# rsutormin/KmerGutsJava

Measured on AMD Instinct MI355X. Metric: amino-acid residues/sec scanned (and hits/sec) on 1 Gbp synthetic, 1/2/4/8 MI355X, higher is better.
Workload: dtype int64; 1 GPU; 1 Gbp contig mix (0.5 kbp..1.024 Mbp, uniform ACGT) on 1 GPU, 6-frame translate + 8-mer lookup vs 1400303159-slot signature table (33.6 GB, load 0.50), -m 5 -g 200; total_bp_rank0=1000000000, contigs_rank0=6351, total_bp_all_ranks=1000000000, num_sigs=1400303159, residues_rank0=1999974596, residues_all_ranks=1999974596, hits_rank0=36744843, hits_all_ranks=36744843, calls_rank0=4, parallelism=contig shards x1, table replicated

## Files before the change

### kmergutsjava_amd/csrc/kg_aggregate.hpp

```cpp
#pragma once

#include <hip/hip_runtime.h>
#include <stdint.h>

#include "../../include/kmerguts_hip.h"

namespace kg {

struct AggParams { int32_t min_hits, min_weighted_hits, max_gap, order_constraint; };

struct AggState {
    uint32_t lo, last, prev;
    int32_t last_pos, last_fI, last_avg, prev_fI;
    int32_t cnt;
    int32_t currentFI;
    uint32_t ncalls;
};

__device__ __forceinline__ int32_t rl(int32_t v, int k) { return __builtin_amdgcn_readlane(v, k); }
__device__ __forceinline__ int32_t uni(int32_t v) { return __builtin_amdgcn_readfirstlane(v); }

struct ChunkRegs {
    uint32_t base;
    uint64_t mask;
    int32_t fI, pos;
    float wt;
};

__device__ __forceinline__ uint32_t process_set(const kg_hit *__restrict__ h, const uint8_t *__restrict__ acc, uint8_t *__restrict__ vote,
                                            uint32_t begin, const AggParams &p, AggState &s, const ChunkRegs &cur, const ChunkRegs &prv,
                                            bool &cur_vote, uint32_t container, kg_call *calls, bool allow_carry)
{
    const int lane = threadIdx.x & 63;
    int32_t fICount = 0;
    float weighted = 0.f;
    uint32_t lastHit = s.lo;
    const uint32_t c0 = begin + ((s.lo - begin) & ~63u);
    for (uint32_t b = c0; b <= s.last; b += 64) {
        const uint32_t i = b + lane;
        const bool in = i >= s.lo && i <= s.last;
        int32_t fI = 0;
        float wt = 0.f;
        bool mem = false;
        if (b == cur.base) {
            fI = cur.fI;
            wt = cur.wt;
            mem = in && ((cur.mask >> lane) & 1ull) != 0;
        } else if (b == prv.base) {
            fI = prv.fI;
            wt = prv.wt;
            mem = in && ((prv.mask >> lane) & 1ull) != 0;
        } else if (in) {
            fI = h[i].fI;
            wt = h[i].functionWt;
            mem = (acc[i] & KG_EV_ACCEPTED) != 0;
        }
        uint64_t m = __ballot(in && mem && fI == s.currentFI);
        if (m) {
            fICount += (int32_t)__popcll(m);
            lastHit = b + 63u - (uint32_t)__builtin_clzll(m);
            const int32_t wbits = __float_as_int(wt);
            while (m) {
                const int k = __builtin_ctzll(m);
                m &= m - 1;
                weighted += __int_as_float(rl(wbits, k));
            }
        }
    }
    uint32_t what = 0;
    if (fICount >= p.min_hits && weighted >= (float)p.min_weighted_hits) {
        what = 1;
        auto pos_of = [&](uint32_t i) -> int32_t {
            if (i - cur.base < 64u) return rl(cur.pos, (int)(i - cur.base));
            if (i - prv.base < 64u) return rl(prv.pos, (int)(i - prv.base));
            return h[i].from0InProt;
        };
        const int32_t pos_lo = pos_of(s.lo), pos_last = pos_of(lastHit);
        if (lane == 0) {
            kg_call c;
            c.container = container;
            c.start = pos_lo;
            c.end = pos_last + (KG_K - 1);
            c.count = fICount; c.fI = s.currentFI; c.weightedHits = weighted;
            calls[s.ncalls] = c;
        }
        s.ncalls++;
        for (uint32_t b = c0; b <= s.last; b += 64) {
            const uint32_t i = b + lane;
            const bool in = i >= s.lo && i <= s.last;
            if (b == cur.base) {
                cur_vote = cur_vote || (in && ((cur.mask >> lane) & 1ull) != 0 && cur.fI == s.currentFI);
            } else if (b == prv.base) {
                if (in && ((prv.mask >> lane) & 1ull) != 0 && prv.fI == s.currentFI) vote[i] = 1;
            } else if (in && (acc[i] & KG_EV_ACCEPTED) != 0 && h[i].fI == s.currentFI) {
                vote[i] = 1;
            }
        }
    }
    if (allow_carry && s.cnt >= 2 && s.prev_fI != s.currentFI && s.prev_fI == s.last_fI) {
        s.currentFI = s.last_fI;
        s.lo = s.prev;
        s.cnt = 2;
        what |= 2;
    } else {
        s.cnt = 0;
    }
    return what;
}

struct EvBits {
    uint32_t e;
    __device__ __forceinline__ void before(int k, uint32_t what)
    {
        const uint32_t bits = KG_EV_RESET_BEFORE | ((what & 1u) ? KG_EV_CALL_BEFORE : 0u) | ((what & 2u) ? KG_EV_KEEP2_BEFORE : 0u);
        if ((int)(threadIdx.x & 63) == k) e |= bits;
    }
    __device__ __forceinline__ void after(int k, uint32_t what)
    {
        const uint32_t bits = KG_EV_RESET_AFTER | ((what & 1u) ? KG_EV_CALL_AFTER : 0u) | ((what & 2u) ? KG_EV_KEEP2_AFTER : 0u);
        if ((int)(threadIdx.x & 63) == k) e |= bits;
    }
};

constexpr uint32_t kNoPiece = 0xFFFFFFFFu;

constexpr uint32_t kPairWindow = 256;
constexpr uint32_t kPairMaxContainer = 39000;

__global__ __launch_bounds__(256) void piece_starts_kernel(const kg_hit *__restrict__ hits, const int64_t *__restrict__ chs,
                                                           uint32_t n_hits, uint32_t pshift, int32_t max_gap,
                                                           uint32_t *__restrict__ piece_start, uint8_t *__restrict__ piece_pair ,
                                                           uint32_t n_blocks, uint32_t pairs_ok)
{
    const int lane = threadIdx.x & 63;
    const uint32_t u = (uint32_t)uni((int32_t)(blockIdx.x * 4 + (threadIdx.x >> 6)));
    if (u >= n_blocks) return;
    uint32_t found = kNoPiece;
    const uint32_t blk = 1u << pshift, i0 = u << pshift;
    if (u > 0 && i0 < n_hits) {
        const uint32_t c0 = hits[i0].container;
        const uint32_t lo0 = (uint32_t)chs[c0], hi0 = (uint32_t)chs[c0 + 1];
        const bool long_enough = hi0 - lo0 >= 2u * blk || hi0 < i0 + blk;
        for (uint32_t j = 0; j < 256u && j < blk && found == kNoPiece && long_enough; j += 64) {
            const uint32_t i = i0 + j + (uint32_t)lane;
            bool gap = false;
            if (i < n_hits && j + (uint32_t)lane < blk) {
                const kg_hit a = hits[i - 1], b = hits[i];
                gap = a.container == b.container && (int32_t)((uint32_t)a.from0InProt + (uint32_t)max_gap) < b.from0InProt;
            }
            const uint64_t m = __ballot(gap);
            if (m) found = i0 + j + (uint32_t)__builtin_ctzll(m);
        }
    }
    if (found != kNoPiece) {
        const uint32_t c = hits[found].container;
        const uint32_t lo = (uint32_t)chs[c], hi = (uint32_t)chs[c + 1];
        if (found - lo < blk / 2 || hi - found < blk / 2) found = kNoPiece;
    }
    uint32_t pair = 0;
    if (found == kNoPiece && pairs_ok && u > 0 && i0 < n_hits) {
        const uint32_t c0 = hits[i0].container;
        const uint32_t lo0 = (uint32_t)chs[c0], hi0 = (uint32_t)chs[c0 + 1];
        if (hi0 - lo0 >= 2u * blk && hi0 - lo0 < kPairMaxContainer) {
            const uint32_t w0 = i0 - lo0 > kPairWindow ? i0 - kPairWindow : lo0;
            const uint32_t span = min(256u, blk);
            const uint32_t wend = min(min(i0 + span + 1u, hi0), n_hits);
            int32_t afi = 0;
            bool have = false, carry_eq = false, carry_start = false;
            for (uint32_t b = w0; b < wend && found == kNoPiece; b += 64) {
                const uint32_t i = b + (uint32_t)lane;
                const bool in = i < wend;
                int32_t fI = 0;
                bool cstart = false, gapf = false, eqf = false;
                if (in) {
                    const kg_hit cur = hits[i];
                    fI = cur.fI;
                    cstart = i == lo0;
                    if (!cstart) {
                        const kg_hit prv = hits[i - 1];
                        gapf = (int32_t)((uint32_t)prv.from0InProt + (uint32_t)max_gap) < cur.from0InProt;
                        eqf = !gapf && prv.fI == cur.fI;
                    }
                }
                const uint64_t am = __ballot(in && (cstart || gapf || eqf)), eqm = __ballot(eqf), stm = __ballot(cstart || gapf);
                const uint64_t below = am & ((1ull << lane) - 1ull);
                const int al = below ? 63 - __builtin_clzll(below) : 0;
                const int32_t lfi = __shfl(fI, al);
                const bool phave = below ? true : have;
                const int32_t pfi = below ? lfi : afi;
                const bool prev_eq = lane ? ((eqm >> (lane - 1)) & 1ull) != 0 : carry_eq;
                const bool prev_start = lane ? ((stm >> (lane - 1)) & 1ull) != 0 : carry_start;
                const bool cand = eqf && !prev_eq && !prev_start && phave && pfi != fI && i >= i0 + 1u && i - 1u < i0 + span &&
                                  i - 1u - lo0 >= blk / 2 && hi0 - (i - 1u) >= blk / 2;
                const uint64_t cm = __ballot(cand);
                if (cm) { found = b + (uint32_t)__builtin_ctzll(cm) - 1u; pair = 1; }
                if (am) { const int last = 63 - __builtin_clzll(am); afi = rl(fI, last); have = true; }
                carry_eq = (eqm >> 63) & 1ull;
                carry_start = (stm >> 63) & 1ull;
            }
        }
    }
    if (lane == 0) { piece_start[u] = found; piece_pair[u] = (uint8_t)pair; }
}

__global__ void merge_before_kernel(const uint32_t *__restrict__ piece_start, const uint8_t *__restrict__ piece_pair,
                                    const uint8_t *__restrict__ before_ev, uint32_t n_blocks, uint8_t *ev, unsigned long long *n_pieces)
{
    const uint32_t u = blockIdx.x * blockDim.x + threadIdx.x;
    const uint32_t ps = u < n_blocks ? piece_start[u] : kNoPiece;
    if (ps != kNoPiece && before_ev[u]) ev[ps + (piece_pair[u] ? 1u : 0u)] |= before_ev[u];
    const unsigned long long m = __ballot(ps != kNoPiece);
    if (m && (threadIdx.x & 63) == 0) atomicAdd(n_pieces, (unsigned long long)__popcll(m));
}

struct CallsCold {
    kg_call *staged;
    uint8_t *tail_ev;
    uint32_t *call_cnt, *first_cnt, *piece_cnt;
    uint8_t *before_ev;
    const uint8_t *piece_pair;
};

__device__ __forceinline__ uint32_t walk_unit(const kg_hit *__restrict__ hits, const AggParams &p, uint8_t *acc, uint8_t *vote,
                                              const uint32_t begin, const uint32_t end, const uint32_t c, kg_call *calls,
                                              const uint32_t *__restrict__ piece_start, const uint32_t pshift,
                                              const CallsCold *__restrict__ cold, uint32_t *tail_out, bool *reached_end)
{
    const int lane = threadIdx.x & 63;
    uint32_t stopped_at = kNoPiece;
    AggState s;
    s.lo = s.last = s.prev = begin;
    s.last_pos = s.last_fI = s.last_avg = s.prev_fI = 0;
    s.cnt = 0; s.currentFI = 0; s.ncalls = 0;
    int32_t carry_pos = 0, carry_fI = 0;
    ChunkRegs pv, ppv;
    pv.base = ppv.base = 0xFFFFFF00u; pv.mask = ppv.mask = 0; pv.fI = ppv.fI = pv.pos = ppv.pos = 0; pv.wt = ppv.wt = 0.f;

    int32_t n_pos = 0, n_fI = 0, n_avg = 0, m_pos = 0, m_fI = 0, m_avg = 0;
    float n_wt = 0.f, m_wt = 0.f;
    if (begin + (uint32_t)lane < end) {
        const kg_hit &h0 = hits[begin + lane];
        n_pos = h0.from0InProt; n_fI = h0.fI; n_avg = h0.avgOffFromEnd; n_wt = h0.functionWt;
    }
    if (begin + 64u + (uint32_t)lane < end) {
        const kg_hit &h1 = hits[begin + 64u + lane];
        m_pos = h1.from0InProt; m_fI = h1.fI; m_avg = h1.avgOffFromEnd; m_wt = h1.functionWt;
    }
    for (uint32_t base = begin; base < end; base += 64) {
        int n = (int)min(64u, end - base);
        if (piece_start) {
            const uint32_t u1 = base >> pshift, u2 = (base + (uint32_t)n - 1u) >> pshift;
            const uint32_t s1 = piece_start[u1];
            if (s1 > begin && s1 >= base && s1 < base + (uint32_t)n) stopped_at = s1;
            if (u2 != u1) {
                const uint32_t s2 = piece_start[u2];
                if (s2 > begin && s2 < base + (uint32_t)n && s2 < stopped_at) stopped_at = s2;
            }
            if (stopped_at != kNoPiece) n = (int)(stopped_at - base);
            if (n == 0) break;
        }
        const uint32_t i = base + lane;
        int32_t pos = n_pos, fI = n_fI, avg = n_avg;
        float wt = n_wt;
        if (lane >= n) { pos = 0; fI = 0; avg = 0; wt = 0.f; }
        n_pos = m_pos; n_fI = m_fI; n_avg = m_avg; n_wt = m_wt;
        m_pos = 0; m_fI = 0; m_avg = 0; m_wt = 0.f;
        if (base + 128u + (uint32_t)lane < end) {
            const kg_hit &h2 = hits[base + 128u + lane];
            m_pos = h2.from0InProt; m_fI = h2.fI; m_avg = h2.avgOffFromEnd; m_wt = h2.functionWt;
        }
        uint64_t accmask;
        bool votes = false;
        EvBits em = {0};
        ChunkRegs cu;
        cu.base = base; cu.mask = 0; cu.fI = fI; cu.pos = pos; cu.wt = wt;

        const bool fast = !p.order_constraint && s.cnt + n < KG_MAX_HITS_PER_SEQ - 2 &&
                          (s.cnt == 0 || s.last + 1 == base);
        if (fast) {
            accmask = n == 64 ? ~0ull : ((1ull << n) - 1ull);
            int32_t ppos = __shfl_up(pos, 1), pfI = __shfl_up(fI, 1);
            if (lane == 0) { ppos = carry_pos; pfI = carry_fI; }
            const bool first = i == begin;
            const bool gapf = !first && (int32_t)((uint32_t)ppos + (uint32_t)p.max_gap) < pos;
            const bool eqf = !first && fI == pfI;
            const uint64_t gapm = __ballot(gapf), eqm = __ballot(eqf);
            const uint64_t inm = n == 64 ? ~0ull : ((1ull << n) - 1ull);
            int k0 = 0;
            for (;;) {
                if (k0 >= n) break;
                const int32_t cfi = s.cnt > 0 ? s.currentFI : rl(fI, k0);
                const uint64_t neqm = __ballot(fI != cfi);
                const uint64_t ev = (gapm | (eqm & neqm)) & inm & ~((1ull << k0) - 1ull);
                if (!ev) break;
                const int k = __builtin_ctzll(ev);
                if (k > k0) {
                    if (s.cnt == 0) { s.currentFI = rl(fI, k0); s.lo = base + k0; }
                    s.cnt += k - k0;
                }
                const int32_t fk = rl(fI, k);
                const uint32_t ik = base + (uint32_t)k;
                if (s.cnt > 0 && ((gapm >> k) & 1)) {
                    uint32_t what = 0;
                    if (s.cnt >= p.min_hits) {
                        s.last = ik - 1;
                        what = (cu.mask = accmask, process_set(hits, acc, vote, begin, p, s, cu, pv, votes, c, calls, false));
                    } else {
                        s.cnt = 0;
                    }
                    em.before(k, what);
                }
                if (s.cnt == 0) { s.currentFI = fk; s.lo = ik; }
                s.cnt++;
                if (s.cnt > 1 && s.currentFI != fk && ((eqm >> k) & 1)) {
                    s.last = ik; s.prev = ik - 1; s.last_fI = fk; s.prev_fI = fk;
                    em.after(k, (cu.mask = accmask, process_set(hits, acc, vote, begin, p, s, cu, pv, votes, c, calls, true)));
                }
                k0 = k + 1;
            }
            if (n > k0) {
                if (s.cnt == 0) { s.currentFI = rl(fI, k0); s.lo = base + k0; }
                s.cnt += n - k0;
            }
            if (s.cnt > 0) {
                s.last = base + n - 1;
                s.last_pos = rl(pos, n - 1); s.last_fI = rl(fI, n - 1); s.last_avg = rl(avg, n - 1);
                if (s.cnt > 1) { s.prev = s.last - 1; s.prev_fI = n >= 2 ? rl(fI, n - 2) : carry_fI; }
            }
        } else {
            accmask = 0;
            for (int k = 0; k < n; k++) {
                const int32_t pk = rl(pos, k), fk = rl(fI, k), ak = rl(avg, k);
                const uint32_t ik = base + (uint32_t)k;
                if (s.cnt > 0 && (int32_t)((uint32_t)s.last_pos + (uint32_t)p.max_gap) < pk) {
                    uint32_t what = 0;
                    if (s.cnt >= p.min_hits)
                        what = (cu.mask = accmask, process_set(hits, acc, vote, begin, p, s, cu, pv, votes, c, calls, true));
                    else
                        s.cnt = 0;
                    em.before(k, what);
                }
                if (s.cnt == 0) s.currentFI = fk;
                bool ok = !p.order_constraint || s.cnt == 0;
                if (!ok) {
                    const int32_t d = (int32_t)((uint32_t)(pk - s.last_pos) - (uint32_t)(s.last_avg - ak));
                    const int32_t ad = d < 0 ? (int32_t)(0u - (uint32_t)d) : d;
                    ok = fk == s.last_fI && ad <= 20;
                }
                if (ok) {
                    if (s.cnt < KG_MAX_HITS_PER_SEQ - 2) {
                        if (s.cnt == 0) { s.lo = ik; s.prev = ik; s.prev_fI = fk; }
                        else { s.prev = s.last; s.prev_fI = s.last_fI; }
                        s.last = ik; s.last_pos = pk; s.last_fI = fk; s.last_avg = ak;
                        s.cnt++;
                        accmask |= 1ull << k;
                    }
                    if (s.cnt > 1 && s.currentFI != fk && s.prev_fI == s.last_fI)
                        em.after(k, (cu.mask = accmask, process_set(hits, acc, vote, begin, p, s, cu, pv, votes, c, calls, true)));
                }
            }
        }
        if (lane < n) {
            acc[i] = (uint8_t)(em.e | (uint32_t)((accmask >> lane) & 1ull) * KG_EV_ACCEPTED);
            vote[i] = votes ? 1 : 0;
        }
        carry_pos = rl(pos, n - 1);
        carry_fI = rl(fI, n - 1);
        ppv = pv;
        cu.mask = accmask;
        pv = cu;
        if (stopped_at != kNoPiece) break;
    }
    uint32_t tail = 0;
    if (stopped_at != kNoPiece && cold->piece_pair[stopped_at >> pshift]) {
        uint32_t bits = 0;
        if (s.cnt > 0) {
            bits = KG_EV_RESET_AFTER | KG_EV_KEEP2_AFTER;
            bool tail_votes = false;
            if (process_set(hits, acc, vote, begin, p, s, pv, ppv, tail_votes, c, calls, false) & 1u) bits |= KG_EV_CALL_AFTER;
            if (tail_votes) vote[pv.base + lane] = 1;
        }
        if (lane == 0) cold->before_ev[stopped_at >> pshift] = (uint8_t)bits;
    } else if (stopped_at != kNoPiece) {
        uint32_t bits = 0;
        if (s.cnt > 0) {
            bits = KG_EV_RESET_BEFORE;
            if (s.cnt >= p.min_hits) {
                bool tail_votes = false;
                if (process_set(hits, acc, vote, begin, p, s, pv, ppv, tail_votes, c, calls, false) & 1u) bits |= KG_EV_CALL_BEFORE;
                if (tail_votes) vote[pv.base + lane] = 1;
            }
        }
        if (lane == 0) cold->before_ev[stopped_at >> pshift] = (uint8_t)bits;
    } else if (s.cnt >= p.min_hits) {
        bool tail_votes = false;
        tail = process_set(hits, acc, vote, begin, p, s, pv, ppv, tail_votes, c, calls, true) & 1u;
        if (tail_votes) vote[pv.base + lane] = 1;
    }
    *tail_out = tail;
    *reached_end = stopped_at == kNoPiece;
    return s.ncalls;
}

__global__ __launch_bounds__(256) void calls_wave_kernel(const kg_hit *__restrict__ hits, const int64_t *__restrict__ chs,
                                                         uint32_t n_cont, AggParams p, uint8_t *acc, uint8_t *vote,
                                                         uint32_t per_wave, uint32_t n_cwaves,
                                                         const uint32_t *__restrict__ piece_start, uint32_t pshift, uint32_t n_pblocks,
                                                         const CallsCold *__restrict__ cold)
{
    const int lane = threadIdx.x & 63;
    const uint32_t w = (uint32_t)uni((int32_t)(blockIdx.x * 4 + (threadIdx.x >> 6)));
    if (w >= n_cwaves) {
        const uint32_t u = w - n_cwaves;
        if (u >= n_pblocks) return;
        const uint32_t begin = piece_start[u];
        if (begin == kNoPiece) return;
        const uint32_t c = hits[begin].container;
        const uint32_t end = (uint32_t)chs[c + 1];
        uint32_t tail;
        bool reached_end;
        const uint32_t ncalls = walk_unit(hits, p, acc, vote, begin, end, c, cold->staged + begin / (uint32_t)p.min_hits, piece_start, pshift,
                                          cold, &tail, &reached_end);
        if (lane == 0) {
            cold->piece_cnt[u] = ncalls;
            if (ncalls) atomicAdd(&cold->call_cnt[c], ncalls);
            if (reached_end) cold->tail_ev[c] = (uint8_t)tail;
        }
        return;
    }
    const uint32_t c_first = w * per_wave;
    uint32_t my_begin = 0, my_end = 0;
    const bool mine = (uint32_t)lane < per_wave && c_first + (uint32_t)lane < n_cont;
    if (mine) { my_begin = (uint32_t)chs[c_first + lane]; my_end = (uint32_t)chs[c_first + lane + 1]; }
    if (mine && my_end - my_begin < 2) {
        cold->first_cnt[c_first + lane] = 0;
        cold->tail_ev[c_first + lane] = 0;
        if (my_end != my_begin) { acc[my_begin] = (uint8_t)KG_EV_ACCEPTED; vote[my_begin] = 0; }
    }
    uint64_t todo = __ballot(mine && my_end - my_begin >= 2);
    while (todo) {
        const int ci = __builtin_ctzll(todo);
        todo &= todo - 1;
        const uint32_t c = c_first + (uint32_t)ci;
        const uint32_t begin = (uint32_t)rl((int32_t)my_begin, ci), end = (uint32_t)rl((int32_t)my_end, ci);
        uint32_t tail;
        bool reached_end;
        const uint32_t ncalls = walk_unit(hits, p, acc, vote, begin, end, c, cold->staged + begin / (uint32_t)p.min_hits, piece_start, pshift,
                                          cold, &tail, &reached_end);
        if (lane == 0) {
            cold->first_cnt[c] = ncalls;
            if (ncalls) atomicAdd(&cold->call_cnt[c], ncalls);
            if (reached_end) cold->tail_ev[c] = (uint8_t)tail;
        }
    }
}

template <int W>
__global__ __launch_bounds__(256) void compact_calls_kernel(const kg_call *__restrict__ staged, const int64_t *__restrict__ chs,
                                                            const uint32_t *__restrict__ first_cnt, const uint32_t *__restrict__ call_off,
                                                            uint32_t n_cont, uint32_t min_hits, kg_call *__restrict__ calls,
                                                            const uint32_t *__restrict__ piece_start, const uint32_t *__restrict__ piece_cnt,
                                                            uint32_t pshift)
{
    const uint64_t t = (uint64_t)blockIdx.x * blockDim.x + threadIdx.x;
    const uint64_t c = t / W;
    if (c >= n_cont) return;
    const uint32_t begin = (uint32_t)chs[c], end = (uint32_t)chs[c + 1];
    kg_call *dst = calls + call_off[c];
    {
        const uint32_t n = first_cnt[c];
        const kg_call *src = staged + begin / min_hits;
        for (uint32_t k = (uint32_t)(t % W); k < n; k += W) dst[k] = src[k];
        dst += n;
    }
    if (piece_start && end > begin) {
        if (W == 64) {
            const int lane = threadIdx.x & 63;
            const uint32_t last = (end - 1u) >> pshift;
            for (uint32_t u0 = begin >> pshift; u0 <= last; u0 += 64) {
                const uint32_t u = u0 + (uint32_t)lane;
                const uint32_t ps = u <= last ? piece_start[u] : kNoPiece;
                const bool mine = ps > begin && ps < end;
                const uint32_t n = mine ? piece_cnt[u] : 0u;
                uint32_t incl = n;
#pragma unroll
                for (int off = 1; off < 64; off <<= 1) {
                    const uint32_t v = (uint32_t)__shfl_up((int)incl, off);
                    if (lane >= off) incl += v;
                }
                const kg_call *src = staged + (mine ? ps / min_hits : 0u);
                for (uint32_t k = 0; k < n; k++) dst[incl - n + k] = src[k];
                dst += (uint32_t)__shfl((int)incl, 63);
            }
        } else {
            for (uint32_t u = begin >> pshift; u <= (end - 1u) >> pshift; u++) {
                const uint32_t ps = piece_start[u];
                if (ps <= begin || ps >= end) continue;
                const uint32_t n = piece_cnt[u];
                const kg_call *src = staged + ps / min_hits;
                for (uint32_t k = (uint32_t)(t % W); k < n; k += W) dst[k] = src[k];
                dst += n;
            }
        }
    }
}

__global__ void call_starts_kernel(const uint32_t *call_off, uint64_t n_cont, const uint64_t *total, int64_t *ccs)
{
    uint64_t c = (uint64_t)blockIdx.x * blockDim.x + threadIdx.x;
    if (c > n_cont) return;
    ccs[c] = c == n_cont ? (int64_t)*total : (int64_t)call_off[c];
}

__global__ __launch_bounds__(256) void voter_count_kernel(const uint8_t *__restrict__ vote, uint32_t n_hits, uint32_t *__restrict__ cnt)
{
    const uint32_t i = blockIdx.x * blockDim.x + threadIdx.x;
    const uint64_t m = __ballot(i < n_hits && vote[i] != 0);
    if ((threadIdx.x & 63) == 0 && (i & ~63u) < n_hits) cnt[i >> 6] = (uint32_t)__popcll(m);
    if (i == 0) cnt[(n_hits + 63u) >> 6] = 0;
}

__global__ __launch_bounds__(256) void voter_scatter_kernel(const kg_hit *__restrict__ hits, const uint8_t *__restrict__ vote,
                                                            uint32_t n_hits, const uint32_t *__restrict__ voff, int32_t *__restrict__ vlist)
{
    const uint32_t i = blockIdx.x * blockDim.x + threadIdx.x;
    const int lane = threadIdx.x & 63;
    const bool v = i < n_hits && vote[i] != 0;
    const uint64_t m = __ballot(v);
    if (v) vlist[voff[i >> 6] + (uint32_t)__popcll(m & ((1ull << lane) - 1ull))] = hits[i].oI;
}

__global__ __launch_bounds__(256) void otu_wave_kernel(const int32_t *__restrict__ vlist, const uint32_t *__restrict__ voff,
                                                       const uint8_t *__restrict__ vote, const int64_t *__restrict__ chs,
                                                       uint32_t n_hits, uint32_t n_seqs, uint32_t per, kg_otu *otu, uint32_t per_wave,
                                                       const kg_otu *__restrict__ otu_init)
{
    const int lane = threadIdx.x & 63;
    const uint32_t s_first = (uint32_t)uni((int32_t)(blockIdx.x * 4 + (threadIdx.x >> 6))) * per_wave;
    auto voter_index = [&](uint32_t i) -> uint32_t {
        const uint32_t c0 = i & ~63u;
        const uint64_t m = __ballot(c0 + (uint32_t)lane < n_hits && c0 + (uint32_t)lane < i && vote[c0 + lane] != 0);
        return (c0 < n_hits ? voff[c0 >> 6] : voff[(n_hits + 63u) >> 6]) + (uint32_t)__popcll(m);
    };
    for (uint32_t s = s_first; s < s_first + per_wave && s < n_seqs; s++) {
        int32_t n = 0;
        uint32_t nmask = 0;
        int32_t cnt = 0, oi = 0;
        if (otu_init) {
            const kg_otu *r0 = otu_init + s;
            n = uni(min(max(r0->n, 0), KG_OI_BUFSZ));
            nmask = (1u << n) - 1u;
            if (lane < KG_OI_BUFSZ) { cnt = r0->count[lane]; oi = r0->oI[lane]; }
        }
        const uint32_t vb = voter_index((uint32_t)chs[(uint64_t)s * per]), ve = voter_index((uint32_t)chs[(uint64_t)(s + 1) * per]);
        int32_t n_o = vb + (uint32_t)lane < ve ? vlist[vb + lane] : 0;
        for (uint32_t b = vb; b < ve; b += 64) {
            const int32_t o = n_o;
            n_o = b + 64u + (uint32_t)lane < ve ? vlist[b + 64u + lane] : 0;
            const int nv = (int)min(64u, ve - b);
            const int32_t before = __shfl_up(o, 1);
            uint64_t heads = __ballot(lane < nv && (lane == 0 || o != before));
            const uint64_t above = lane < 63 ? heads >> (lane + 1) : 0ull;
            const int32_t rlen = above ? __builtin_ctzll(above) + 1 : nv - lane;
            while (heads) {
                const int k = __builtin_ctzll(heads);
                heads &= heads - 1;
                const int32_t ok = rl(o, k), r = rl(rlen, k);
                const uint64_t at = __ballot(oi == ok) & nmask;
                int j;
                if (at) {
                    j = __builtin_ctzll(at);
                    cnt += lane == j ? r : 0;
                } else {
                    if (n == KG_OI_BUFSZ) j = KG_OI_BUFSZ - 1; else { j = n++; nmask = nmask * 2u + 1u; }
                    if (lane == j) { oi = ok; cnt = r; }
                }
                if (j == 0) continue;
                const int32_t cj = rl(cnt, j);
                const uint32_t more = (uint32_t)__ballot(cnt > cj);
                if ((more >> (j - 1)) & 1u) continue;
                const uint32_t gt = more & ((1u << j) - 1u);
                const int p = gt ? 32 - __builtin_clz(gt) : 0;
                const int32_t oj = rl(oi, j);
                const int32_t pc = __builtin_amdgcn_update_dpp(0, cnt, 0x111, 0xF, 0xF, false);
                const int32_t po = __builtin_amdgcn_update_dpp(0, oi, 0x111, 0xF, 0xF, false);
                if (lane > p && lane <= j) { cnt = pc; oi = po; }
                else if (lane == p) { cnt = cj; oi = oj; }
            }
        }
        if (lane < KG_OI_BUFSZ) {
            otu[s].count[lane] = lane < n ? cnt : 0;
            otu[s].oI[lane] = lane < n ? oi : 0;
        }
        if (lane == 0) otu[s].n = n;
    }
}

__global__ void process_set_single_kernel(const kg_hit *__restrict__ hits, int32_t n, int32_t current_fi, AggParams p,
                                          kg_otu *otu, kg_call *call, int32_t *out)
{
    if (threadIdx.x != 0 || blockIdx.x != 0) return;
    int32_t count = 0, last = 0;
    float wt = 0.f;
    for (int32_t i = 0; i < n; i++)
        if (hits[i].fI == current_fi) { last = i; count++; wt += hits[i].functionWt; }
    int32_t called = 0;
    kg_otu o = *otu;
    if (count >= p.min_hits && wt >= (float)p.min_weighted_hits) {
        called = 1;
        kg_call c;
        c.container = hits[0].container; c.start = hits[0].from0InProt; c.end = hits[last].from0InProt + (KG_K - 1);
        c.count = count; c.fI = current_fi; c.weightedHits = wt;
        *call = c;
        for (int32_t i = 0; i <= last; i++) {
            if (hits[i].fI != current_fi) continue;
            int32_t j = 0;
            while (j < o.n && o.oI[j] != hits[i].oI) j++;
            if (j == o.n) {
                if (o.n == KG_OI_BUFSZ) j--; else o.n++;
                o.oI[j] = hits[i].oI; o.count[j] = 1;
            } else o.count[j]++;
            while (j > 0 && o.count[j - 1] <= o.count[j]) {
                const int32_t tc = o.count[j - 1], to = o.oI[j - 1];
                o.count[j - 1] = o.count[j]; o.oI[j - 1] = o.oI[j];
                o.count[j] = tc; o.oI[j] = to;
                j--;
            }
        }
    }
    *otu = o;
    const bool keep2 = hits[n - 2].fI != current_fi && hits[n - 2].fI == hits[n - 1].fI;
    out[0] = called; out[1] = keep2 ? hits[n - 1].fI : current_fi; out[2] = keep2 ? 1 : 0;
}

}
```

### kmergutsjava_amd/csrc/kg_device.hpp

```cpp
#pragma once

#include <hip/hip_runtime.h>
#include <stdint.h>

#include "../../include/kmerguts_hip.h"

namespace kg {

constexpr int kWave = 64;
constexpr int kWavesPerWG = 4;
constexpr int kDnaPosPerBlock = 192;
constexpr int kAaWinPerBlock = 64;
constexpr uint32_t kInvalid = 0xFFFFFFFFu;
constexpr uint32_t kTagEmpty = 0xFFu;
constexpr uint64_t kNotFound = ~0ull;
constexpr int kTagPad = 64;

struct BlockDesc {
    uint64_t soff;
    uint32_t len;
    uint32_t j;
    uint32_t nk;
    uint32_t ibase;
    uint32_t seq;
// ... 623 lines not shown
            }
#pragma unroll
            for (int q = 0; q < N; q++) {
                if (r == q) {
                    cand[q] = s;
                    if (done) {
                        if (COUNTERS) stop[q] = s;
                        if (hit) { ent[q].oI = e.oI; ent[q].avg = e.avg; ent[q].fI = e.fI; ent[q].wt = e.wt; foundm |= 1u << q; }
                    }
                }
            }
            if (done) pend &= pend - 1;
        }
    }
    if (COUNTERS) {
#pragma unroll
        for (int q = 0; q < N; q++) {
            if (valid[q]) {
                uint64_t last = stop[q] < tab.limit ? stop[q] + 1 : tab.limit;
                ctr_slots += last - home[q];
                if (prog) progress_note_walk(prog, home[q], stop[q], tab.limit);
                if (found_slot) found_slot[q] = (uint32_t)stop[q];
            }
        }
    }
    return foundm;
}

__device__ __forceinline__ void flush_ran_off(bool ran_off, unsigned long long *ctr, int lane)
{
    if (__ballot(ran_off) && lane == 0) atomicOr(&ctr[3], 1ull);
}

__device__ __forceinline__ void flush_counters(unsigned long long ctr_valid, unsigned long long ctr_slots,
                                               unsigned long long *ctr, int lane)
{
    for (int off = 32; off > 0; off >>= 1) {
        ctr_valid += __shfl_down(ctr_valid, off);
        ctr_slots += __shfl_down(ctr_slots, off);
    }
    if (lane == 0) {
        atomicAdd(&ctr[0], ctr_valid);
        atomicAdd(&ctr[1], ctr_slots);
    }
}

template <bool AA, bool COUNTERS, int RPG>
__global__ __launch_bounds__(kWave *kWavesPerWG) void scan_kernel(
    const uint8_t *__restrict__ entries, const uint8_t *__restrict__ tags, uint64_t limit, uint64_t num_sigs, uint64_t magic,
    uint32_t m35, const uint8_t *__restrict__ seq, const BlockDesc *__restrict__ blocks, uint32_t n_blocks,
    uint32_t *__restrict__ counts,
    uint32_t *__restrict__ block_stage_base, kg_hit *__restrict__ stage, unsigned long long *cursor, uint64_t stage_cap,
    uint32_t stage_chunk, unsigned long long *ctr,
    Progress *prog , uint32_t *__restrict__ stage_slot ,
    const uint32_t *__restrict__ hbits , uint64_t tail_start)
{
    constexpr int ROWS = AA ? 1 : 6;
    constexpr int NG = ROWS / RPG;
    static_assert(ROWS % RPG == 0, "RPG must divide the row count");
    __shared__ typename WaveLds<AA>::type lds[kWavesPerWG];
    __shared__ typename WaveLds<AA>::tables enc_tables;
    const int lane = threadIdx.x & 63;
    const int wave = threadIdx.x >> 6;
    const uint32_t wave_global = __builtin_amdgcn_readfirstlane(blockIdx.x * kWavesPerWG + wave);
    const uint32_t n_waves = gridDim.x * kWavesPerWG;
    TableView tab;
    tab.entries = entries; tab.tags = tags; tab.limit = limit; tab.num_sigs = num_sigs; tab.magic = magic; tab.m35 = m35;

    typename WaveLds<AA>::type &l = lds[wave];
    encode_init<AA>(enc_tables, threadIdx.x, blockDim.x);
    __syncthreads();

    unsigned long long ctr_valid = 0, ctr_slots = 0;
    bool ran_off = false;
    unsigned long long res_at = 0, res_end = 0;

    for (uint32_t it_v = wave_global; it_v < n_blocks; it_v += n_waves) {
        const uint32_t it = __builtin_amdgcn_readfirstlane(it_v);
        const BlockDesc bd = blocks[it];
        encode_block<AA>(l, enc_tables, seq, bd, lane);

        for (int g = 0; g < NG; g++) {
            uint64_t val[RPG], home[RPG];
            uint32_t fp[RPG];
            bool valid[RPG];
#pragma unroll
            for (int q = 0; q < RPG; q++) {
                uint32_t hi, lo;
                uint64_t quo;
                valid[q] = row_halves<AA>(l, g * RPG + q, lane, bd, &hi, &lo);
                home[q] = split_halves(hi, lo, tab, &quo);
                fp[q] = tag_qs(quo, home[q]);
                val[q] = (uint64_t)hi * 160000ull + lo;
            }

            if (!COUNTERS && hbits) {
                uint32_t w[RPG];
#pragma unroll
                for (int q = 0; q < RPG; q++) w[q] = valid[q] && home[q] < limit ? hbits[home[q] >> 5] : ~0u;
#pragma unroll
                for (int q = 0; q < RPG; q++)
                    if (valid[q] && home[q] < limit && !((w[q] >> ((uint32_t)home[q] & 31u)) & 1u)) {
                        valid[q] = false;
                        if (home[q] >= tail_start) ran_off = true;
                    }
            }
            Payload ent[RPG];
            uint32_t fslot[RPG];
#pragma unroll
            for (int q = 0; q < RPG; q++) fslot[q] = 0;
            const uint32_t foundm = probe_n<RPG, COUNTERS>(tab, val, home, fp, valid, ent, ctr_valid, ctr_slots, ran_off,
                                                           COUNTERS ? prog : nullptr, COUNTERS && stage_slot ? fslot : nullptr);

            uint32_t cnt[RPG], rank[RPG];
            uint32_t total = 0;
#pragma unroll
            for (int q = 0; q < RPG; q++) {
                const int r = g * RPG + q;
                unsigned long long m = __ballot((foundm >> q) & 1u);
                cnt[q] = (uint32_t)__popcll(m);
                unsigned long long below = m & ((1ull << lane) - 1ull);
                unsigned long long above = lane == 63 ? 0ull : (m >> (lane + 1));
                rank[q] = (!AA && r >= 3) ? (uint32_t)__popcll(above) : (uint32_t)__popcll(below);
                total += cnt[q];
                if (lane == 0) counts[row_index<AA>(bd, it, r)] = cnt[q];
            }
            if (total > res_end - res_at) {
                unsigned long long chunk = total > stage_chunk ? total : stage_chunk;
                unsigned long long b = 0;
                if (lane == 0) b = atomicAdd(cursor, chunk);
                b = ((unsigned long long)__builtin_amdgcn_readfirstlane((uint32_t)(b >> 32)) << 32) |
                    (unsigned long long)__builtin_amdgcn_readfirstlane((uint32_t)b);
                res_at = b; res_end = b + chunk;
            }
            const unsigned long long base = res_at;
            res_at += total;
            if (lane == 0) block_stage_base[(uint64_t)it * NG + g] = (uint32_t)base;
            if (total && base + total <= stage_cap) {
                uint32_t rowbase = 0;
#pragma unroll
                for (int q = 0; q < RPG; q++) {
                    if ((foundm >> q) & 1u) {
                        kg_hit h;
                        row_record_key<AA>(bd, g * RPG + q, lane, &h.container, &h.from0InProt);
                        h.oI = ent[q].oI; h.avgOffFromEnd = ent[q].avg; h.fI = ent[q].fI; h.functionWt = ent[q].wt;
                        stage[base + rowbase + rank[q]] = h;
                        if (COUNTERS && stage_slot) stage_slot[base + rowbase + rank[q]] = fslot[q];
                    }
                    rowbase += cnt[q];
                }
            }
        }
        wave_sync();
    }

    if (COUNTERS) flush_counters(ctr_valid, ctr_slots, ctr, lane);
    flush_ran_off(ran_off, ctr, lane);
}

__global__ void build_blocks_kernel(const int64_t *seq_off, const uint32_t *ibase, uint32_t n_seqs,
                                    uint32_t n_blocks, BlockDesc *out)
{
    uint32_t i = blockIdx.x * blockDim.x + threadIdx.x;
    if (i >= n_blocks) return;
    uint32_t lo = 0, hi = n_seqs;
    while (hi - lo > 1) {
        uint32_t mid = lo + (hi - lo) / 2;
        if (ibase[mid] <= i) lo = mid; else hi = mid;
    }
    BlockDesc d;
    d.soff = (uint64_t)seq_off[lo];
    d.len = (uint32_t)(seq_off[lo + 1] - seq_off[lo]);
    d.j = i - ibase[lo];
    d.nk = ibase[lo + 1] - ibase[lo];
    d.ibase = ibase[lo];
    d.seq = lo;
    d.pad = 0;
    out[i] = d;
}

constexpr int kScanThreads = 256;
constexpr int kScanPerThread = 8;
constexpr int kScanChunk = kScanThreads * kScanPerThread;

__device__ __forceinline__ uint32_t wg_exclusive_scan(uint32_t x, uint32_t *total, uint32_t *lds )
{
    const int lane = threadIdx.x & 63, wave = threadIdx.x >> 6;
    uint32_t incl = x;
    for (int off = 1; off < 64; off <<= 1) {
        uint32_t y = __shfl_up(incl, off);
        if (lane >= off) incl += y;
    }
    if (lane == 63) lds[wave] = incl;
    __syncthreads();
    uint32_t wbase = 0, all = 0;
    for (int w = 0; w < kScanThreads / 64; w++) {
        uint32_t s = lds[w];
        if (w < wave) wbase += s;
        all += s;
    }
    __syncthreads();
    *total = all;
    return wbase + incl - x;
}

__global__ __launch_bounds__(kScanThreads) void scan_partials_kernel(const uint32_t *in, uint64_t n, uint64_t *partial)
{
    __shared__ uint64_t wsum[kScanThreads / 64];
    uint64_t base = (uint64_t)blockIdx.x * kScanChunk + (uint64_t)threadIdx.x * kScanPerThread;
    uint64_t s = 0;
    for (int k = 0; k < kScanPerThread; k++)
        if (base + k < n) s += in[base + k];
    for (int d = 32; d > 0; d >>= 1) s += __shfl_xor(s, d);
    if ((threadIdx.x & 63) == 0) wsum[threadIdx.x >> 6] = s;
    __syncthreads();
    if (threadIdx.x == 0) {
        uint64_t all = 0;
        for (int w = 0; w < kScanThreads / 64; w++) all += wsum[w];
        partial[blockIdx.x] = all;
    }
}

__global__ __launch_bounds__(kScanThreads) void scan_top_kernel(uint64_t *partial, uint32_t n_partials, uint64_t *total_out)
{
    __shared__ uint64_t carry;
    __shared__ uint64_t wsum[kScanThreads / 64];
    if (threadIdx.x == 0) carry = 0;
    __syncthreads();
    const int lane = threadIdx.x & 63, wave = threadIdx.x >> 6;
    for (uint32_t b = 0; b < n_partials; b += kScanThreads) {
        uint32_t i = b + threadIdx.x;
        uint64_t x = i < n_partials ? partial[i] : 0;
        uint64_t incl = x;
        for (int off = 1; off < 64; off <<= 1) {
            uint64_t y = __shfl_up(incl, off);
            if (lane >= off) incl += y;
        }
        if (lane == 63) wsum[wave] = incl;
        __syncthreads();
        uint64_t wbase = 0, all = 0;
        for (int w = 0; w < kScanThreads / 64; w++) {
            uint64_t s = wsum[w];
            if (w < wave) wbase += s;
            all += s;
        }
        uint64_t c = carry;
        if (i < n_partials) partial[i] = c + wbase + incl - x;
        __syncthreads();
        if (threadIdx.x == 0) carry = c + all;
        __syncthreads();
    }
    if (threadIdx.x == 0) *total_out = carry;
}

__global__ __launch_bounds__(kScanThreads) void scan_final_kernel(const uint32_t *in, uint64_t n, const uint64_t *partial,
                                                                  uint32_t *out)
{
    __shared__ uint32_t lds[8];
    uint64_t base = (uint64_t)blockIdx.x * kScanChunk + (uint64_t)threadIdx.x * kScanPerThread;
    uint32_t v[kScanPerThread];
    uint32_t s = 0;
    for (int k = 0; k < kScanPerThread; k++) {
        v[k] = base + k < n ? in[base + k] : 0;
        s += v[k];
    }
    uint32_t total;
    uint32_t excl = wg_exclusive_scan(s, &total, lds);
    uint32_t run = (uint32_t)partial[blockIdx.x] + excl;
    for (int k = 0; k < kScanPerThread; k++) {
        if (base + k < n) out[base + k] = run;
        run += v[k];
    }
}

template <bool AA>
__global__ __launch_bounds__(kWave *kWavesPerWG) void place_kernel(const BlockDesc *__restrict__ blocks, uint32_t n_blocks,
                                                                  const uint32_t *__restrict__ counts,
                                                                  const uint32_t *__restrict__ offs,
                                                                  const uint32_t *__restrict__ block_stage_base, uint32_t rpg,
                                                                  const kg_hit *__restrict__ stage, kg_hit *__restrict__ hits,
                                                                  const uint32_t *__restrict__ stage_slot, uint32_t *__restrict__ hit_slots)
{
    constexpr int ROWS = AA ? 1 : 6;
    const int lane = threadIdx.x & 63;
    const uint32_t it = __builtin_amdgcn_readfirstlane(blockIdx.x * kWavesPerWG + (threadIdx.x >> 6));
    if (it >= n_blocks) return;
    const BlockDesc bd = blocks[it];
    const uint32_t ng = (uint32_t)ROWS / rpg;
    uint32_t src = 0;
#pragma unroll
    for (int r = 0; r < ROWS; r++) {
        if ((uint32_t)r % rpg == 0) src = block_stage_base[(uint64_t)it * ng + (uint32_t)r / rpg];
        const uint32_t vrow = row_index<AA>(bd, it, r);
        uint32_t n = counts[vrow];
        if ((uint32_t)lane < n) {
            hits[(uint64_t)offs[vrow] + lane] = stage[(uint64_t)src + lane];
            if (hit_slots) hit_slots[(uint64_t)offs[vrow] + lane] = stage_slot[(uint64_t)src + lane];
        }
        src += n;
    }
}

template <bool AA>
__global__ void container_starts_kernel(const uint32_t *ibase, uint32_t n_seqs, const uint32_t *offs, uint64_t n_rows,
                                        const uint64_t *total, int64_t *chs)
{
    constexpr uint32_t PER = AA ? 1 : 6;
    uint64_t c = (uint64_t)blockIdx.x * blockDim.x + threadIdx.x;
    uint64_t n_cont = (uint64_t)n_seqs * PER;
    if (c > n_cont) return;
    if (c == n_cont) { chs[c] = (int64_t)*total; return; }
    uint32_t k = (uint32_t)(c / PER), cc = (uint32_t)(c % PER);
    uint32_t nk = ibase[k + 1] - ibase[k];
    uint64_t row = (uint64_t)PER * ibase[k] + (uint64_t)cc * nk;
    chs[c] = row < n_rows ? (int64_t)offs[row] : (int64_t)*total;
}

struct ClearList { uint32_t *p[8]; uint64_t words[8]; int n; };

__global__ __launch_bounds__(256) void clear_many_kernel(ClearList l)
{
    const uint64_t tid = (uint64_t)blockIdx.x * blockDim.x + threadIdx.x, stride = (uint64_t)gridDim.x * blockDim.x;
    for (int k = 0; k < l.n; k++) {
        uint32_t *p = l.p[k];
        const uint64_t w = l.words[k];
        const uint64_t head = min(w, (uint64_t)((16u - ((uintptr_t)p & 15u)) & 15u) / 4u);
        const uint64_t quads = (w - head) / 4;
        uint4 *q = reinterpret_cast<uint4 *>(p + head);
        for (uint64_t i = tid; i < quads; i += stride) q[i] = make_uint4(0, 0, 0, 0);
        for (uint64_t i = tid; i < head; i += stride) p[i] = 0;
        for (uint64_t i = head + quads * 4 + tid; i < w; i += stride) p[i] = 0;
    }
}

__global__ void build_tags_kernel(const uint8_t *entries, uint64_t limit, uint64_t n_tags, uint64_t num_sigs, uint64_t magic,
                                  uint8_t *tags, unsigned long long *occupied)
{
    TableView tab;
    tab.entries = entries; tab.tags = tags; tab.limit = limit; tab.num_sigs = num_sigs; tab.magic = magic; tab.m35 = 0;
    uint64_t i = (uint64_t)blockIdx.x * blockDim.x + threadIdx.x;
    uint64_t stride = (uint64_t)gridDim.x * blockDim.x;
    unsigned long long occ = 0, tail = 0;
    for (; i < n_tags; i += stride) {
        uint32_t t = kTagEmpty;
        if (i < limit) {
            const uint2 *p = reinterpret_cast<const uint2 *>(entries + i * 24);
            uint2 a = p[0];
            int64_t key = (int64_t)(((uint64_t)a.y << 32) | a.x);
            if (key <= KG_MAX_ENCODED) {
                uint64_t q;
                const uint64_t slot = split_value((uint64_t)key, tab, &q);
                t = tag_qs(q, slot);
                occ++;
            }
        }
        tags[i] = (uint8_t)t;
        if (t == kTagEmpty && i < limit) tail = i + 1;
    }
    for (int off = 32; off > 0; off >>= 1) {
        occ += __shfl_down(occ, off);
        const unsigned long long o = __shfl_down(tail, off);
        tail = o > tail ? o : tail;
    }
    if ((threadIdx.x & 63) == 0) {
        if (occ) atomicAdd(occupied, occ);
        if (tail) atomicMax(occupied + 1, tail);
    }
}

constexpr uint32_t kHomeWalkMax = 1024;
constexpr uint32_t kBidxClasses = 19, kBidxPair0 = 20, kBidxHash0 = 191, kBidxMore = 255;
constexpr uint32_t kBidxInexact = 0x80000000u;

__host__ __device__ constexpr uint32_t bidx_pair_code(uint32_t c1, uint32_t c2)
{
    return kBidxPair0 + c1 * 19u - c1 * (c1 + 1u) / 2u + (c2 - c1 - 1u);
}
static_assert(bidx_pair_code(0, 1) == 20 && bidx_pair_code(0, 18) == 37 && bidx_pair_code(1, 2) == 38 && bidx_pair_code(17, 18) == 190,
              "pair codes must fill 20..190");

__device__ __forceinline__ uint32_t bidx_decode(uint32_t code)
{
    if (code == 0) return 0u;
    if (code < kBidxPair0) return 1u << (code - 1u);
    if (code < kBidxHash0) {
        uint32_t c1 = 0;
        while (code >= bidx_pair_code(c1, c1 + 1u) + (18u - c1)) c1++;
        const uint32_t c2 = c1 + 1u + (code - bidx_pair_code(c1, c1 + 1u));
        return (1u << c1) | (1u << c2);
    }
    if (code == kBidxMore) return 0x7FFFFu | kBidxInexact;
    const uint32_t m6 = code - kBidxHash0;
    uint32_t m = 0;
    for (uint32_t c = 0; c < kBidxClasses; c++) m |= ((m6 >> (c % 6u)) & 1u) << c;
    return m | kBidxInexact;
}

__device__ __forceinline__ uint32_t bidx_encode(uint32_t class_mask, bool complete)
{
    if (!complete) return kBidxMore;
    const uint32_t n = (uint32_t)__popc(class_mask);
    if (n == 0) return 0u;
    const uint32_t c1 = (uint32_t)__builtin_ctz(class_mask);
    if (n == 1) return 1u + c1;
    if (n == 2) return bidx_pair_code(c1, 31u - (uint32_t)__builtin_clz(class_mask));
    const uint32_t m6 = (class_mask | (class_mask >> 6) | (class_mask >> 12) | (class_mask >> 18)) & 63u;
    return kBidxHash0 + m6;
}

__global__ void build_bidx_kernel(const uint8_t *entries, const uint8_t *tags, uint64_t limit, uint64_t n_idx, uint64_t num_sigs,
                                  uint64_t magic, uint8_t *idx)
{
    TableView tab;
    tab.entries = entries; tab.tags = tags; tab.limit = limit; tab.num_sigs = num_sigs; tab.magic = magic; tab.m35 = 0;
    const uint64_t stride = (uint64_t)gridDim.x * blockDim.x;
    for (uint64_t h = (uint64_t)blockIdx.x * blockDim.x + threadIdx.x; h < n_idx; h += stride) {
        uint32_t mask = 0;
        bool complete = true;
        if (h < limit && tags[h] != kTagEmpty) {
            uint64_t j = h;
            for (; j < limit && j - h < kHomeWalkMax; j++) {
                if (tags[j] == kTagEmpty) break;
                const uint2 a = *reinterpret_cast<const uint2 *>(entries + j * 24);
                const int64_t key = (int64_t)(((uint64_t)a.y << 32) | a.x);
                if (key < 0) continue;
                uint64_t q;
                if (split_value((uint64_t)key, tab, &q) != h) continue;
                mask |= 1u << (uint32_t)(q % kBidxClasses);
            }
            if (j < limit && j - h >= kHomeWalkMax) complete = false;
        }
        idx[h] = (uint8_t)bidx_encode(mask, complete);
    }
}

__global__ void build_hbits_kernel(const uint8_t *__restrict__ idx, uint64_t n_idx, uint32_t *__restrict__ bits, uint64_t n_words)
{
    const uint64_t stride = (uint64_t)gridDim.x * blockDim.x;
    for (uint64_t w = (uint64_t)blockIdx.x * blockDim.x + threadIdx.x; w < n_words; w += stride) {
        uint32_t out = 0;
        const uint64_t s0 = w * 32;
        if (s0 + 32 <= n_idx) {
            const uint4 a = *reinterpret_cast<const uint4 *>(idx + s0), b = *reinterpret_cast<const uint4 *>(idx + s0 + 16);
            const uint32_t v[8] = {a.x, a.y, a.z, a.w, b.x, b.y, b.z, b.w};
#pragma unroll
            for (int k = 0; k < 8; k++)
#pragma unroll
                for (int j = 0; j < 4; j++) out |= (((v[k] >> (8 * j)) & 0xFFu) != 0u ? 1u : 0u) << (4 * k + j);
        } else {
            for (uint32_t j = 0; j < 32 && s0 + j < n_idx; j++) out |= (idx[s0 + j] != 0 ? 1u : 0u) << j;
        }
        bits[w] = out;
    }
}

}
```

### kmergutsjava_amd/csrc/kg_host.hpp

```cpp
#pragma once

#include <algorithm>
#include <atomic>
#include <cstdio>
#include <cstdlib>
#include <cstring>
#include <map>
#include <memory>
#include <mutex>
#include <new>
#include <string>
#include <thread>
#include <unordered_map>
#include <vector>

namespace {

thread_local std::string g_err;

int fail(int code, const std::string &msg)
{
    g_err = msg;
    return code;
}

#define HIP_TRY(expr)                                                                              \
    do {                                                                                           \
        hipError_t e_ = (expr);                                                                    \
        if (e_ != hipSuccess)                                                                      \
            return fail(KG_ERR_DEVICE, std::string(#expr) + ": " + hipGetErrorString(e_));         \
    } while (0)

struct DevCache {
    std::mutex mu;
    std::multimap<size_t, void *> free_;
    std::unordered_map<void *, size_t> live;

    static size_t round_up(size_t b)
    {
        if (b < 256) return 256;
        size_t g = b >= (8u << 20) ? (2u << 20) : 256;
        return (b + g - 1) / g * g;
    }
    hipError_t get(void **p, size_t bytes)
    {
        bytes = round_up(bytes);
        std::lock_guard<std::mutex> lk(mu);
        auto it = free_.lower_bound(bytes);
        if (it != free_.end() && it->first <= bytes + bytes / 2 + (1u << 20)) {
            *p = it->second;
            live[*p] = it->first;
            free_.erase(it);
            return hipSuccess;
        }
        hipError_t e = hipMalloc(p, bytes);
        if (e != hipSuccess) {
            for (auto &kv : free_) (void)hipFree(kv.second);
            free_.clear();
            e = hipMalloc(p, bytes);
            if (e != hipSuccess) return e;
        }
        live[*p] = bytes;
        return hipSuccess;
    }
    void put(void *p)
    {
        std::lock_guard<std::mutex> lk(mu);
        auto it = live.find(p);
        if (it == live.end()) return;
        free_.emplace(it->second, p);
        live.erase(it);
    }
    void detach(void *p)
    {
        std::lock_guard<std::mutex> lk(mu);
        live.erase(p);
    }
    size_t live_bytes()
    {
        std::lock_guard<std::mutex> lk(mu);
        size_t n = 0;
        for (auto &kv : live) n += kv.second;
        return n;
    }
    void release_all()
    {
        std::lock_guard<std::mutex> lk(mu);
        for (auto &kv : free_) (void)hipFree(kv.second);
        for (auto &kv : live) (void)hipFree(kv.first);
        free_.clear();
        live.clear();
    }
    void release_free()
    {
        std::lock_guard<std::mutex> lk(mu);
        for (auto &kv : free_) (void)hipFree(kv.second);
        free_.clear();
    }
};

struct PinCache {
    std::mutex mu;
    std::multimap<size_t, void *> free_;
    std::unordered_map<void *, size_t> live;
    size_t kept = 0;
    static constexpr size_t kKeepTotal = 6ull << 30;

    hipError_t get(void **p, size_t bytes)
    {
        bytes = bytes < 4096 ? 4096 : (bytes + 4095) / 4096 * 4096;
        {
            std::lock_guard<std::mutex> lk(mu);
            auto it = free_.lower_bound(bytes);
            if (it != free_.end() && it->first <= 2 * bytes + (1u << 16)) {
                *p = it->second;
                live[*p] = it->first;
                kept -= it->first;
                free_.erase(it);
                return hipSuccess;
            }
        }
        hipError_t e = hipHostMalloc(p, bytes);
        if (e != hipSuccess) return e;
        std::lock_guard<std::mutex> lk(mu);
        live[*p] = bytes;
        return hipSuccess;
    }
    void put(void *p)
    {
        std::vector<void *> drop;
        {
            std::lock_guard<std::mutex> lk(mu);
            auto it = live.find(p);
            if (it == live.end()) return;
            const size_t bytes = it->second;
            live.erase(it);
            free_.emplace(bytes, p);
            kept += bytes;
            while (kept > kKeepTotal && !free_.empty()) {
                auto big = std::prev(free_.end());
                kept -= big->first;
                drop.push_back(big->second);
                free_.erase(big);
            }
        }
        for (void *d : drop) (void)hipHostFree(d);
    }
    void release_all()
    {
        std::lock_guard<std::mutex> lk(mu);
        for (auto &kv : free_) (void)hipHostFree(kv.second);
        for (auto &kv : live) (void)hipHostFree(kv.first);
        free_.clear();
        live.clear();
        kept = 0;
    }
};

}

constexpr uint64_t kHbitsMaxSlots = 1ull << 26;

constexpr uint32_t kMaxChunks = 8;
constexpr uint32_t kMaxOrderStreams = 4;
enum : int {
    kPevChunk = 0,
    kPevFork = 16,
    kPevJoin2 = 17, kPevJoin3 = 18,
    kPevTotals = 19,
    kPevVerified = 20,
    kPevBase = 32,
    kPevOrdered = 40,
    kPevCount = 48
};
static_assert(kPevChunk + 2 * kMaxChunks <= kPevFork && kPevVerified + kMaxChunks <= kPevBase && kPevBase + kMaxChunks <= kPevOrdered &&
              kPevOrdered + kMaxOrderStreams <= kPevCount, "event slots overlap");
enum : int { kEvBegin = 0, kEvScanBegin = 1, kEvScanEnd = 2, kEvOrderEnd = 3, kEvAggEnd = 4, kEvScattered = 5 , kEvSpare = 6,
             kEvJoined = 7 , kEvCount = 8, kEvStageBegin = kEvBegin, kEvStageEnd = kEvScanBegin };
enum : int { kTotHits = 0, kTotCursor = 1 , kTotValid = 2, kTotSlots = 3 ,
             kTotCalls = 4, kTotRanOff = 5 , kTotPieces = 6, kTotVoters = 7, kTotWords = 8,
             kTotSent = 6  };
enum : int { kPcUcur = 0 , kPcCcur = 8 , kPcBase = 16 ,
             kPcCtot = 32 , kPcWords = 48 };
static_assert(kPcUcur + kMaxChunks <= kPcCcur && kPcCcur + kMaxChunks <= kPcBase && kPcBase + kMaxChunks + 1 <= kPcCtot &&
              kPcCtot + kMaxChunks <= kPcWords, "per-chunk words overlap");
enum : int { kOvfGroups = 0 , kOvfLowc = 1 , kOvfGuard = 2 ,
             kOvfWords = 8 };
enum : int { kPinPc = 0 , kPinOvf = 48 , kPinTotals = 80 , kPinCalls = 88 ,
             kPinPieces = 89, kPinWords = 96,
             kPinStage = 80, kPinStageWords = kPinWords - kPinStage,
             kPinAssign = 90  };
static_assert(kPinPc + kPcWords <= kPinOvf && kOvfWords * kMaxChunks * 4 <= (kPinTotals - kPinOvf) * 8 && kPinTotals + kTotSent <= kPinCalls,
              "counters must fit their pinned words");
static_assert(kPinAssign >= kPinStage && kPinAssign + 2 + 3 <= kPinWords, "stage words must fit their pinned words");

struct kg_table {
    int device = 0;
    hipStream_t stream = nullptr;
    hipStream_t stream2 = nullptr;
    hipStream_t stream3 = nullptr;
    hipStream_t ostream[kMaxOrderStreams] = {};
    hipEvent_t pev[kPevCount] = {};
    bool own_entries = false;
    uint8_t *d_entries = nullptr;
    uint8_t *d_tags = nullptr;
    uint8_t *d_bidx = nullptr;
    bool bidx_exact = false;
    uint32_t *d_hbits = nullptr;
    uint64_t tail_start = 0;
    int64_t num_sigs = 0, entry_size = 0, version = 0;
    uint64_t limit = 0;
    uint64_t magic = 0;
    uint32_t m35 = 0;
    uint64_t occupied = 0;
    double stage_ratio = 1.0 / 16;
    size_t scatter_lds[2][3] = {};
    kg::ScatterCold *d_cold = nullptr;
    kg::ScatterCold h_cold[kMaxChunks] = {};
    kg::CallsCold *d_calls_cold = nullptr;
    kg::CallsCold h_calls_cold = {};
    size_t hist_lds = 48 * 1024;
    size_t place_lds[2] = {48 * 1024, 48 * 1024};
    hipEvent_t ev[kEvCount] = {};
    uint64_t *h_pin = nullptr;
    std::atomic<int> busy{0};
    uint32_t fail_alloc_at = 0, alloc_count = 0;
    DevCache cache;
    PinCache pins;
};

struct kg_result {
    kg_table *tab = nullptr;
    bool own_tab = false;
    kg_stats st = {};
    uint32_t per = 6;
    kg_hit *d_hits = nullptr;
    int64_t *d_chs = nullptr;
    kg_call *d_calls = nullptr;
    int64_t *d_ccs = nullptr;
    kg_otu *d_otu = nullptr;
    uint8_t *d_ev = nullptr, *d_tail_ev = nullptr;
    uint32_t *d_hit_slots = nullptr;
    bool has_progress = false;
    kg_progress progress = {};
    void *h_hits = nullptr, *h_chs = nullptr, *h_ccs = nullptr, *h_calls = nullptr, *h_otu = nullptr, *h_ev = nullptr,
         *h_tail_ev = nullptr, *h_hit_slots = nullptr;
};

namespace {

uint32_t env_u32(const char *name, uint32_t dflt)
{
    const char *v = getenv(name);
    if (!v || !*v) return dflt;
    char *end = nullptr;
    long x = strtol(v, &end, 10);
    return (end != v && x >= 0) ? (uint32_t)x : dflt;
}

constexpr uint32_t kMaxGrid = 256u * 32u;

uint32_t env_knob(const char *name, uint32_t dflt, uint32_t lo, uint32_t hi, uint32_t mult = 1)
{
    uint32_t x = dflt;
    if (const char *v = getenv(name); v && *v) {
        char *end = nullptr;
        const long long y = strtoll(v, &end, 10);
        if (end != v && y >= 0) x = y > (long long)hi ? hi : (uint32_t)y;
    }
    x = std::min(hi, std::max(lo, x));
    return (x + mult - 1) / mult * mult;
}

uint32_t test_hook(const char *name)
{
    static const bool enabled = env_u32("KG_ENABLE_TEST_HOOKS", 0u) != 0;
    return enabled ? env_u32(name, 0u) : 0u;
}

int dalloc(kg_table *t, void **p, size_t bytes)
{
    if (t->fail_alloc_at && ++t->alloc_count == t->fail_alloc_at)
        return fail(KG_ERR_NOMEM, "device allocation failed: KG_TEST_FAIL_ALLOC test hook");
    hipError_t e = t->cache.get(p, bytes);
    if (e != hipSuccess) return fail(KG_ERR_NOMEM, std::string("device allocation failed: ") + hipGetErrorString(e));
    return KG_OK;
}

void dfree(kg_table *t, void *p)
{
    if (p) t->cache.put(p);
}

int dalloc_detached(kg_table *t, uint8_t **p, size_t bytes)
{
    const int rc = dalloc(t, (void **)p, bytes);
    if (rc == KG_OK) t->cache.detach(*p);
    return rc;
}

int table_new(int device, kg_table **out);

struct CallScope {
    kg_table *t = nullptr;
    const bool owned;
    int rc;
    CallScope(kg_table *tab, const char *busy_text) : owned(false), rc(tab->busy.exchange(1) != 0 ? fail(KG_ERR_BUSY, busy_text) : KG_OK)
    {
        if (rc == KG_OK) { t = tab; rc = arm(true); }
    }
    explicit CallScope(int device, bool hook = true) : owned(true), rc(table_new(device, &t))
    {
        if (rc == KG_OK) arm(hook);
    }
    ~CallScope()
    {
        if (!t) return;
        t->fail_alloc_at = 0;
        if (owned) kg_table_close(t);
        else t->busy.store(0);
    }
    int arm(bool hook)
    {
        t->fail_alloc_at = hook ? test_hook("KG_TEST_FAIL_ALLOC") : 0u;
        t->alloc_count = 0;
        if (!owned) HIP_TRY(hipSetDevice(t->device));
        return KG_OK;
    }
    kg_table *disown() { kg_table *out = t; t = nullptr; out->fail_alloc_at = 0; return out; }
};

int prefix_sum(kg_table *t, const uint32_t *d_in, uint64_t n, uint32_t *d_out, uint64_t *d_partial, uint64_t *d_total,
               hipStream_t stream = nullptr)
{
    if (!stream) stream = t->stream;
    uint32_t nb = (uint32_t)((n + kg::kScanChunk - 1) / kg::kScanChunk);
    if (nb == 0) nb = 1;
    hipLaunchKernelGGL(kg::scan_partials_kernel, dim3(nb), dim3(kg::kScanThreads), 0, stream, d_in, n, d_partial);
    hipLaunchKernelGGL(kg::scan_top_kernel, dim3(1), dim3(kg::kScanThreads), 0, stream, d_partial, nb, d_total);
    hipLaunchKernelGGL(kg::scan_final_kernel, dim3(nb), dim3(kg::kScanThreads), 0, stream, d_in, n, d_partial, d_out);
    HIP_TRY(hipGetLastError());
    return KG_OK;
}

struct ClearItem { void *p; uint64_t words; };

template <typename G>
int clear_words(hipStream_t stream, G grid, std::initializer_list<ClearItem> items)
{
    kg::ClearList cl = {};
    uint64_t most = 0;
    for (const ClearItem &it : items) {
        if (!it.words) continue;
        if (cl.n == (int)std::size(cl.p)) return fail(KG_ERR_DEVICE, "more than eight arrays in one clear (internal error)");
        cl.p[cl.n] = (uint32_t *)it.p; cl.words[cl.n++] = it.words;
        most = std::max(most, it.words);
    }
    if (cl.n) hipLaunchKernelGGL(kg::clear_many_kernel, dim3(grid(most)), dim3(256), 0, stream, cl);
    return KG_OK;
}

struct Scratch {
    kg_table *t;
    std::vector<void *> ptrs;
    explicit Scratch(kg_table *tt) : t(tt) {}
    ~Scratch()
    {
        (void)hipStreamSynchronize(t->stream);
        if (t->stream2) (void)hipStreamSynchronize(t->stream2);
        if (t->stream3) (void)hipStreamSynchronize(t->stream3);
        for (auto &os : t->ostream) if (os) (void)hipStreamSynchronize(os);
        for (void *p : ptrs) dfree(t, p);
    }
    void adopt(void *p) { ptrs.push_back(p); }
    void release(void *p) { ptrs.erase(std::find(ptrs.begin(), ptrs.end(), p)); }
    template <typename T> int get(T **p, size_t count)
    {
        void *v = nullptr;
        int rc = dalloc(t, &v, count * sizeof(T));
        if (rc) return rc;
        ptrs.push_back(v);
        *p = (T *)v;
        return KG_OK;
    }
};

struct SetBase {
    kg_table *tab = nullptr;
    bool own_tab = false;
    std::vector<void *> blocks;
    SetBase() = default;
    SetBase(const SetBase &) = delete;
    SetBase &operator=(const SetBase &) = delete;
    ~SetBase()
    {
        if (!tab) return;
        (void)hipSetDevice(tab->device);
        for (void *p : blocks) dfree(tab, p);
        if (own_tab) kg_table_close(tab);
    }
    template <typename T> T *keep(Scratch &sc, T *p)
    {
        if (p) { blocks.push_back(p); sc.release(p); }
        return p;
    }
};

template <typename S>
int make_set(const CallScope &cs, std::unique_ptr<S> &set)
{
    set.reset(new (std::nothrow) S());
    if (!set) return fail(KG_ERR_NOMEM, "out of host memory");
    set->tab = cs.t;
    return KG_OK;
}

template <typename S>
int hand_out(CallScope &cs, std::unique_ptr<S> &set, S **out)
{
    if (cs.owned) {
        cs.t->cache.release_free();
        set->own_tab = true;
        cs.disown();
    }
    *out = set.release();
    return KG_OK;
}

int device_of(const SetBase *s) { return s ? s->tab->device : 0; }

template <typename T>
int copy_records(const void *s, int device, const T *src, size_t per, int64_t have, int64_t first, int64_t count, T *dst, const char *what,
                 const char *of = "the set")
{
    if (!s || (count > 0 && !dst)) return fail(KG_ERR_ARG, "null argument");
    if (first < 0 || count < 0 || first + count > have) return fail(KG_ERR_ARG, std::string(what) + ": range outside " + of);
    if (count == 0) return KG_OK;
    HIP_TRY(hipSetDevice(device));
    HIP_TRY(hipMemcpy(dst, src + (size_t)first * per, (size_t)count * per * sizeof(T), hipMemcpyDefault));
    return KG_OK;
}

int copy_starts(const void *s, int device, const int64_t *src, int64_t n, int64_t *dst)
{
    if (!s || !dst) return fail(KG_ERR_ARG, "null argument");
    HIP_TRY(hipSetDevice(device));
    HIP_TRY(hipMemcpy(dst, src, ((size_t)n + 1) * 8, hipMemcpyDefault));
    return KG_OK;
}

template <typename St>
int copy_stats(const void *s, const St *st, St *out)
{
    if (!s || !out) return fail(KG_ERR_ARG, "null argument");
    *out = *st;
    return KG_OK;
}

uint32_t grid_of(uint64_t n, uint32_t threads = 256)
{
    return (uint32_t)std::max<uint64_t>(1, (n + threads - 1) / threads);
}

uint64_t magic_of(uint64_t d)
{
    return d == 1 ? ~0ull : (uint64_t)(((unsigned __int128)1 << 64) / d);
}

std::string kmer_text(int64_t v)
{
    char b[32];
    snprintf(b, sizeof b, "%lld", (long long)v);
    return b;
}

int fail_and_free(kg_result *r, int rc) { std::string keep = g_err; kg_result_free(r); g_err = keep; return rc; }

uint32_t bit_width(uint64_t v) { return v ? 64u - (uint32_t)__builtin_clzll(v) : 0u; }

uint32_t bits_for(uint64_t n) { return n > 1 ? bit_width(n - 1) : 0; }

template <int N>
struct Events {
    hipEvent_t e[N] = {};
    ~Events() { for (auto x : e) if (x) (void)hipEventDestroy(x); }
    int create() { for (auto &x : e) HIP_TRY(hipEventCreate(&x)); return KG_OK; }
    hipEvent_t operator[](int i) const { return e[i]; }
    float ms(int i, int j) const { float m = 0; (void)hipEventElapsedTime(&m, e[i], e[j]); return m; }
};

struct ErrWord { int word, code; const char *prefix, *suffix; };
constexpr uint64_t kNoErr = 0x7F7F7F7F7F7F7F7Full;
static_assert(kNoErr == kg::kAssignNoErr && kNoErr == kg::kRegionNoErr, "the stages' kernels share the error words' \"none\"");

int read_error_words(kg_table *t, const void *d_words, size_t n_words, int pin, std::initializer_list<ErrWord> table)
{
    HIP_TRY(hipMemcpyAsync(t->h_pin + pin, d_words, n_words * 8, hipMemcpyDeviceToHost, t->stream));
    HIP_TRY(hipStreamSynchronize(t->stream));
    for (const ErrWord &w : table)
        if (const uint64_t at = t->h_pin[pin + w.word]; at != kNoErr) return fail(w.code, w.prefix + kmer_text((int64_t)at) + w.suffix);
    return KG_OK;
}

int read_record_errors(kg_table *t, const void *d_words, size_t n_words, int n_err, const char *const *what)
{
    int rc;
    if ((rc = read_error_words(t, d_words, n_words, kPinStage, {}))) return rc;
    const uint64_t *h = t->h_pin + kPinStage;
    const int first = (int)(std::min_element(h, h + n_err) - h);
    if (h[first] != kNoErr) return fail(KG_ERR_ARG, "record " + kmer_text((int64_t)h[first]) + what[first]);
    return KG_OK;
}

int upload_pinned(kg_table *t, const uint8_t *src, size_t bytes, uint8_t *d_dst)
{
    const size_t CH = 32u << 20;
    const size_t n_pieces = (bytes + CH - 1) / CH;
    const unsigned hw = std::thread::hardware_concurrency();
    const size_t n_thr = std::max<size_t>(1, std::min<size_t>({(size_t)8, (size_t)(hw ? hw : 4), n_pieces}));
    std::atomic<size_t> next{0};
    std::atomic<bool> ok{true};
    auto worker = [&]() {
        if (hipSetDevice(t->device) != hipSuccess) { ok = false; return; }
        hipStream_t s = nullptr;
        uint8_t *pin[2] = {nullptr, nullptr};
        hipEvent_t done[2] = {nullptr, nullptr};
        bool good = hipStreamCreateWithFlags(&s, hipStreamNonBlocking) == hipSuccess &&
                    hipHostMalloc((void **)&pin[0], CH) == hipSuccess && hipHostMalloc((void **)&pin[1], CH) == hipSuccess &&
                    hipEventCreate(&done[0]) == hipSuccess && hipEventCreate(&done[1]) == hipSuccess;
        bool used[2] = {false, false};
        int which = 0;
        while (good && ok.load()) {
            const size_t k = next.fetch_add(1);
            if (k >= n_pieces) break;
            const size_t at = k * CH, n = std::min(CH, bytes - at);
            if (used[which]) good = hipEventSynchronize(done[which]) == hipSuccess;
            if (!good) break;
            memcpy(pin[which], src + at, n);
            good = hipMemcpyAsync(d_dst + at, pin[which], n, hipMemcpyHostToDevice, s) == hipSuccess &&
                   hipEventRecord(done[which], s) == hipSuccess;
            used[which] = true;
            which ^= 1;
        }
        if (s && hipStreamSynchronize(s) != hipSuccess) good = false;
        if (!good) ok = false;
        for (int i = 0; i < 2; i++) { if (pin[i]) (void)hipHostFree(pin[i]); if (done[i]) (void)hipEventDestroy(done[i]); }
        if (s) (void)hipStreamDestroy(s);
    };
    {
        std::vector<std::thread> pool;
        for (size_t i = 1; i < n_thr; i++) pool.emplace_back(worker);
        worker();
        for (auto &th : pool) th.join();
    }
    return ok.load() ? KG_OK : fail(KG_ERR_DEVICE, "uploading to the device failed (pinned staging or host-to-device copy)");
}

struct SortPairs {
    uint64_t *k[2] = {nullptr, nullptr};
    uint32_t *v[2] = {nullptr, nullptr};
    int cur = 0;
    int alloc(Scratch &sc, uint64_t n) { int rc = sc.get(&k[0], n); return rc ? rc : sc.get(&v[0], n); }
    uint64_t *keys() const { return k[cur]; }
    uint32_t *vals() const { return v[cur]; }
    SortPairs next() const { SortPairs s; s.k[0] = k[cur ^ 1]; s.v[0] = v[cur]; return s; }
    int sort(kg_table *t, Scratch &sc, uint64_t n, uint32_t key_bits);
};

int SortPairs::sort(kg_table *t, Scratch &sc, uint64_t n, uint32_t key_bits)
{
    if (n <= 1 || key_bits == 0) return KG_OK;
    const uint32_t n_tiles = (uint32_t)((n + kg::kBuildTile - 1) / kg::kBuildTile);
    const uint32_t passes = (key_bits + 7) / 8, bits = passes ? (key_bits + passes - 1) / passes : 1, radix = 1u << bits;
    const uint64_t n_hist = (uint64_t)radix * n_tiles;
    const uint64_t nb = (n_hist + kg::kScanChunk - 1) / kg::kScanChunk;
    uint32_t *hist = nullptr, *offs = nullptr;
    uint64_t *partial = nullptr;
    int rc;
    if ((rc = sc.get(&k[cur ^ 1], n)) || (rc = sc.get(&v[cur ^ 1], n)) || (rc = sc.get(&hist, n_hist)) ||
        (rc = sc.get(&offs, n_hist)) || (rc = sc.get(&partial, nb + 2)))
        return rc;
    for (uint32_t p = 0; p < passes; p++) {
        const uint32_t shift = p * bits;
        hipLaunchKernelGGL(kg::build_hist_kernel, dim3(n_tiles), dim3(kg::kBuildThreads), 0, t->stream, k[cur], n, shift, radix,
                           n_tiles, hist);
        HIP_TRY(hipGetLastError());
        if ((rc = prefix_sum(t, hist, n_hist, offs, partial, partial + nb + 1))) return rc;
        hipLaunchKernelGGL(kg::build_scatter_kernel, dim3(n_tiles), dim3(kg::kBuildThreads), 0, t->stream, k[cur], v[cur], n,
                           shift, bits, n_tiles, offs, k[cur ^ 1], v[cur ^ 1]);
        HIP_TRY(hipGetLastError());
        cur ^= 1;
    }
    return KG_OK;
}

}
```

### kmergutsjava_amd/csrc/kg_host_aggregate.hpp

```cpp
#pragma once

namespace {

int aggregate_stage(kg_table *t, const kg_params *p, kg_result *res, Scratch &sc, int64_t n_seqs, uint64_t n_cont, uint64_t n_hits,
                    uint32_t PER, uint64_t *d_partial, uint64_t *d_totals, const kg_otu *d_otu_init, bool allow_pieces, const AggPlan &ag)
{
    int rc;
    kg::AggParams ap;
    ap.min_hits = p->min_hits; ap.min_weighted_hits = p->min_weighted_hits;
    ap.max_gap = p->max_gap; ap.order_constraint = p->order_constraint ? 1 : 0;
    uint32_t *d_ccnt = nullptr, *d_coff = nullptr, *d_first = nullptr;
    kg_call *d_staged = nullptr;
    uint8_t *d_vote = nullptr;
    if ((rc = dalloc(t, (void **)&res->d_ev, n_hits))) return rc;
    if ((rc = dalloc(t, (void **)&res->d_tail_ev, n_cont))) return rc;
    uint8_t *d_acc = res->d_ev;
    if ((rc = sc.get(&d_ccnt, n_cont))) return rc;
    if ((rc = sc.get(&d_first, n_cont))) return rc;
    if ((rc = sc.get(&d_coff, n_cont))) return rc;
    if ((rc = sc.get(&d_vote, n_hits))) return rc;
    if ((rc = sc.get(&d_staged, (size_t)(n_hits / (uint64_t)p->min_hits + 1)))) return rc;
    if ((rc = dalloc(t, (void **)&res->d_ccs, (n_cont + 1) * 8))) return rc;
    if ((rc = dalloc(t, (void **)&res->d_otu, (size_t)(n_seqs ? n_seqs : 1) * sizeof(kg_otu)))) return rc;
    const bool pieces = allow_pieces && !p->order_constraint && p->max_gap >= 0 && p->max_gap < (1 << 30) && n_cont &&
                        n_hits > (2ull << ag.pshift) && ag.pieces_on;
    const uint32_t n_pblocks = pieces ? (uint32_t)((n_hits + (1ull << ag.pshift) - 1) >> ag.pshift) : 0u;
    uint32_t *d_pstart = nullptr, *d_pcnt = nullptr;
    uint8_t *d_before = nullptr, *d_ppair = nullptr;
    t->h_pin[kPinCalls] = 0;
    t->h_pin[kPinPieces] = 0;
    if (pieces) {
        if ((rc = sc.get(&d_pstart, (size_t)n_pblocks + 1))) return rc;
        if ((rc = sc.get(&d_pcnt, (size_t)n_pblocks + 1))) return rc;
        if ((rc = sc.get(&d_before, ((size_t)n_pblocks + 4) & ~(size_t)3))) return rc;
        if ((rc = sc.get(&d_ppair, ((size_t)n_pblocks + 4) & ~(size_t)3))) return rc;
    }
    if ((rc = clear_words(t->stream, [](uint64_t most) { return (uint32_t)std::min<uint64_t>(1024, most / 1024 + 1); },
                          {{d_ccnt, n_cont}, {d_pcnt, pieces ? (uint64_t)n_pblocks + 1 : 0}, {d_before, pieces ? ((uint64_t)n_pblocks + 4) / 4 : 0}})))
        return rc;
    if (pieces)
        hipLaunchKernelGGL(kg::piece_starts_kernel, dim3((n_pblocks + 3) / 4), dim3(256), 0, t->stream, res->d_hits, res->d_chs,
                           (uint32_t)n_hits, ag.pshift, ap.max_gap, d_pstart, d_ppair, n_pblocks, ag.agg_pairs);
    const uint32_t cpw = (uint32_t)std::min<uint64_t>(16, std::max<uint64_t>(1, n_cont / (1u << 17)));
    const uint32_t n_cwaves = (uint32_t)((n_cont + cpw - 1) / cpw);
    if (n_cont) {
        const kg::CallsCold cold = {d_staged, res->d_tail_ev, d_ccnt, d_first, d_pcnt, d_before, d_ppair};
        if (!t->d_calls_cold || memcmp(&cold, &t->h_calls_cold, sizeof cold)) {
            if (!t->d_calls_cold) HIP_TRY(hipMalloc((void **)&t->d_calls_cold, sizeof cold));
            t->h_calls_cold = cold;
            HIP_TRY(hipMemcpyAsync(t->d_calls_cold, &t->h_calls_cold, sizeof cold, hipMemcpyHostToDevice, t->stream));
        }
        hipLaunchKernelGGL(kg::calls_wave_kernel, dim3((n_cwaves + n_pblocks + 3) / 4), dim3(256), 0, t->stream, res->d_hits, res->d_chs,
                           (uint32_t)n_cont, ap, d_acc, d_vote, cpw, n_cwaves, d_pstart, ag.pshift, n_pblocks, t->d_calls_cold);
        if (pieces)
            hipLaunchKernelGGL(kg::merge_before_kernel, dim3((n_pblocks + 255) / 256), dim3(256), 0, t->stream, d_pstart, d_ppair, d_before,
                               n_pblocks, res->d_ev, (unsigned long long *)(d_totals + kTotPieces));
        HIP_TRY(hipGetLastError());
    }
    if ((rc = prefix_sum(t, d_ccnt, n_cont, d_coff, d_partial, d_totals + kTotCalls))) return rc;
    if (n_cont) HIP_TRY(hipMemcpyAsync(t->h_pin + kPinCalls, d_totals + kTotCalls, 8, hipMemcpyDeviceToHost, t->stream));
    if (pieces) HIP_TRY(hipMemcpyAsync(t->h_pin + kPinPieces, d_totals + kTotPieces, 8, hipMemcpyDeviceToHost, t->stream));
    if (n_seqs) {
        const uint32_t n_vchunks = (uint32_t)((n_hits + 63) / 64);
        uint32_t *d_vcnt = nullptr, *d_voff = nullptr;
        int32_t *d_vlist = nullptr;
        uint64_t *d_vpartial = nullptr;
        if ((rc = sc.get(&d_vcnt, (size_t)n_vchunks + 1))) return rc;
        if ((rc = sc.get(&d_voff, (size_t)n_vchunks + 1))) return rc;
        if ((rc = sc.get(&d_vlist, (size_t)n_hits + 1))) return rc;
        if ((rc = sc.get(&d_vpartial, (size_t)((n_vchunks + 1) / kg::kScanChunk + 2)))) return rc;
        if (n_hits) {
            const uint32_t vgrid = (uint32_t)((n_hits + 255) / 256);
            hipLaunchKernelGGL(kg::voter_count_kernel, dim3(vgrid), dim3(256), 0, t->stream, d_vote, (uint32_t)n_hits, d_vcnt);
            if ((rc = prefix_sum(t, d_vcnt, (uint64_t)n_vchunks + 1, d_voff, d_vpartial, d_totals + kTotVoters))) return rc;
            hipLaunchKernelGGL(kg::voter_scatter_kernel, dim3(vgrid), dim3(256), 0, t->stream, res->d_hits, d_vote, (uint32_t)n_hits, d_voff,
                               d_vlist);
        } else {
            HIP_TRY(hipMemsetAsync(d_voff, 0, 4, t->stream));
        }
        const uint32_t spw = (uint32_t)std::min<uint64_t>(16, std::max<uint64_t>(1, (uint64_t)n_seqs / (1u << 17)));
        hipLaunchKernelGGL(kg::otu_wave_kernel, dim3((uint32_t)((((uint64_t)n_seqs + spw - 1) / spw + 3) / 4)), dim3(256), 0, t->stream,
                           d_vlist, d_voff, d_vote, res->d_chs, (uint32_t)n_hits, (uint32_t)n_seqs, PER, res->d_otu, spw, d_otu_init);
    }
    hipLaunchKernelGGL(kg::call_starts_kernel, dim3((uint32_t)((n_cont + 1 + 255) / 256)), dim3(256), 0, t->stream, d_coff,
                       n_cont, d_totals + kTotCalls, res->d_ccs);
    if ((rc = dalloc(t, (void **)&res->d_calls, (size_t)(n_hits / (uint64_t)p->min_hits + 1) * sizeof(kg_call)))) return rc;
    if (n_cont) {
        if (n_cont < (1u << 17))
            hipLaunchKernelGGL((kg::compact_calls_kernel<64>), dim3((uint32_t)((n_cont * 64 + 255) / 256)), dim3(256), 0, t->stream,
                               d_staged, res->d_chs, d_first, d_coff, (uint32_t)n_cont, (uint32_t)p->min_hits, res->d_calls,
                               d_pstart, d_pcnt, ag.pshift);
        else
            hipLaunchKernelGGL((kg::compact_calls_kernel<1>), dim3((uint32_t)((n_cont + 255) / 256)), dim3(256), 0, t->stream,
                               d_staged, res->d_chs, d_first, d_coff, (uint32_t)n_cont, (uint32_t)p->min_hits, res->d_calls,
                               d_pstart, d_pcnt, ag.pshift);
    }
    HIP_TRY(hipGetLastError());
    return KG_OK;
}

int aggregate_records(kg_table *t, const kg_params *p, const kg_hit *hits, const int64_t *container_hit_start, int64_t n_seqs,
                      const kg_otu *otu_init, kg_result *r)
{
    const uint64_t n_cont = (uint64_t)n_seqs * r->per, n_hits = (uint64_t)container_hit_start[n_cont];
    Scratch sc(t);
    int rc;
    uint64_t *d_partial = nullptr, *d_totals = nullptr;
    kg_otu *d_init = nullptr;
    if ((rc = dalloc(t, (void **)&r->d_hits, (n_hits ? n_hits : 1) * sizeof(kg_hit)))) return rc;
    if ((rc = dalloc(t, (void **)&r->d_chs, (n_cont + 1) * 8))) return rc;
    if ((rc = sc.get(&d_partial, (size_t)(n_cont / kg::kScanChunk + 2)))) return rc;
    if ((rc = sc.get(&d_totals, 8))) return rc;
    if (otu_init && n_seqs && (rc = sc.get(&d_init, (size_t)n_seqs))) return rc;
    HIP_TRY(hipMemsetAsync(d_totals, 0, 64, t->stream));
    if (n_hits) HIP_TRY(hipMemcpyAsync(r->d_hits, hits, n_hits * sizeof(kg_hit), hipMemcpyHostToDevice, t->stream));
    HIP_TRY(hipMemcpyAsync(r->d_chs, container_hit_start, (n_cont + 1) * 8, hipMemcpyHostToDevice, t->stream));
    if (d_init) HIP_TRY(hipMemcpyAsync(d_init, otu_init, (size_t)n_seqs * sizeof(kg_otu), hipMemcpyHostToDevice, t->stream));
    if ((rc = aggregate_stage(t, p, r, sc, n_seqs, n_cont, n_hits, r->per, d_partial, d_totals, d_init, false, plan_aggregate()))) return rc;
    HIP_TRY(hipStreamSynchronize(t->stream));
    r->st.n_seqs = n_seqs; r->st.n_containers = (int64_t)n_cont; r->st.n_hits = (int64_t)n_hits;
    r->st.n_calls = (int64_t)t->h_pin[kPinCalls];
    r->st.windows_valid = -1; r->st.slots_inspected = -1;
    return KG_OK;
}

}

extern "C" {

int kg_aggregate_hits(int device, const kg_params *p, const kg_hit *hits, const int64_t *container_hit_start, int64_t n_seqs,
                      const kg_otu *otu_init, kg_result **out)
{
    if (!p || !container_hit_start || !out || n_seqs < 0) return fail(KG_ERR_ARG, "null or negative argument");
    if (n_seqs > 0x7FFFFFF0ll / 6) return fail(KG_ERR_LIMIT, "too many sequences in one batch");
    if (p->min_hits < 2)
        return fail(KG_ERR_UNSUPPORTED, "minHits < 2: the reference throws in processSetOfHits (KGJ:442); refusing");
    const uint32_t PER = p->aa ? 1u : 6u;
    const uint64_t n_cont = (uint64_t)n_seqs * PER;
    if (container_hit_start[0] != 0) return fail(KG_ERR_ARG, "container_hit_start[0] must be 0");
    for (uint64_t c = 0; c < n_cont; c++)
        if (container_hit_start[c + 1] < container_hit_start[c]) return fail(KG_ERR_ARG, "container_hit_start must be non-decreasing");
    const uint64_t n_hits = (uint64_t)container_hit_start[n_cont];
    if (n_hits && !hits) return fail(KG_ERR_ARG, "null hit records");
    if (n_hits > 0xFFFFFF00ull) return fail(KG_ERR_LIMIT, "more than 2^32-256 hit records");
    CallScope cs(device,  false);
    if (cs.rc) return cs.rc;
    kg_result *r = new (std::nothrow) kg_result();
    if (!r) return fail(KG_ERR_NOMEM, "out of host memory");
    r->tab = cs.t; r->per = PER;
    if (const int rc = aggregate_records(cs.t, p, hits, container_hit_start, n_seqs, otu_init, r)) return fail_and_free(r, rc);
    r->own_tab = true;
    cs.disown();
    *out = r;
    return KG_OK;
}

int kg_process_set_of_hits(int device, const kg_params *p, const kg_hit *hits, int32_t n_hits, int32_t current_fi, kg_otu *otu,
                           kg_call *call, int32_t *called, int32_t *new_current_fi, int32_t *keeps_last_two)
{
    if (!p || !hits || !otu || !call || !called || !new_current_fi || !keeps_last_two) return fail(KG_ERR_ARG, "null argument");
    if (n_hits < 2)
        return fail(KG_ERR_UNSUPPORTED, "processSetOfHits on fewer than two hits: the reference throws (hits.get(numHits-2), KGJ:442); refusing");
    if (otu->n < 0 || otu->n > KG_OI_BUFSZ) return fail(KG_ERR_ARG, "oICounts holds more than OI_BUFSZ entries");
    int ndev = 0;
    if (hipGetDeviceCount(&ndev) != hipSuccess || ndev <= 0)
        return fail(KG_ERR_DEVICE, "no HIP device: libkmerguts_hip needs an MI355X (gfx950) GPU; there is no CPU path");
    if (device < 0 || device >= ndev) return fail(KG_ERR_ARG, "device index out of range");
    HIP_TRY(hipSetDevice(device));
    kg_hit *d_hits = nullptr;
    uint8_t *d_small = nullptr;
    const size_t small = sizeof(kg_otu) + sizeof(kg_call) + 16;
    HIP_TRY(hipMalloc((void **)&d_hits, (size_t)n_hits * sizeof(kg_hit)));
    hipError_t e = hipMalloc((void **)&d_small, small);
    if (e == hipSuccess) e = hipMemcpy(d_hits, hits, (size_t)n_hits * sizeof(kg_hit), hipMemcpyHostToDevice);
    if (e == hipSuccess) e = hipMemset(d_small, 0, small);
    if (e == hipSuccess) e = hipMemcpy(d_small, otu, sizeof(kg_otu), hipMemcpyHostToDevice);
    uint8_t h_small[sizeof(kg_otu) + sizeof(kg_call) + 16];
    if (e == hipSuccess) {
        kg::AggParams ap;
        ap.min_hits = p->min_hits; ap.min_weighted_hits = p->min_weighted_hits;
        ap.max_gap = p->max_gap; ap.order_constraint = p->order_constraint ? 1 : 0;
        hipLaunchKernelGGL(kg::process_set_single_kernel, dim3(1), dim3(64), 0, nullptr, d_hits, n_hits, current_fi, ap,
                           (kg_otu *)d_small, (kg_call *)(d_small + sizeof(kg_otu)), (int32_t *)(d_small + sizeof(kg_otu) + sizeof(kg_call)));
        e = hipGetLastError();
        if (e == hipSuccess) e = hipMemcpy(h_small, d_small, small, hipMemcpyDeviceToHost);
    }
    (void)hipFree(d_hits);
    if (d_small) (void)hipFree(d_small);
    if (e != hipSuccess) return fail(KG_ERR_DEVICE, std::string("processSetOfHits on the device failed: ") + hipGetErrorString(e));
    memcpy(otu, h_small, sizeof(kg_otu));
    memcpy(call, h_small + sizeof(kg_otu), sizeof(kg_call));
    int32_t o3[4];
    memcpy(o3, h_small + sizeof(kg_otu) + sizeof(kg_call), 16);
    *called = o3[0]; *new_current_fi = o3[1]; *keeps_last_two = o3[2];
    return KG_OK;
}

}
```

### kmergutsjava_amd/csrc/kg_host_plan.hpp

```cpp
#pragma once

namespace {


template <typename T, T V, T... Vs, typename F>
void dispatch(T x, F &&f)
{
    if constexpr (sizeof...(Vs) == 0) f(std::integral_constant<T, V>{});
    else if (x == V) f(std::integral_constant<T, V>{});
    else dispatch<T, Vs...>(x, f);
}

struct BatchPlan {
    std::vector<uint32_t> ibase;
    uint64_t nblocks = 0, windows = 0, residues = 0;
    uint64_t n_rows = 0, n_cont = 0;
    int64_t longest = 0;
};

template <bool AA>
int plan_batch(const int64_t *offsets, int64_t n_seqs, BatchPlan &b)
{
    constexpr uint32_t PER = AA ? 1 : 6;
    b.ibase.resize((size_t)n_seqs + 1);
    for (int64_t k = 0; k < n_seqs; k++) {
        int64_t L = offsets[k + 1] - offsets[k];
        if (L < 0) return fail(KG_ERR_ARG, "offsets must be non-decreasing");
        b.longest = std::max(b.longest, L);
        if (L > 0xFFFFFFF0ll) return fail(KG_ERR_LIMIT, "a single sequence longer than 2^32-16 characters");
        b.ibase[(size_t)k] = (uint32_t)b.nblocks;
        uint64_t nb;
        if (AA) {
            uint64_t nwin = L >= 9 ? (uint64_t)L - 8 : 0;
            b.windows += nwin;
            b.residues += (uint64_t)L;
            nb = (nwin + kg::kAaWinPerBlock - 1) / kg::kAaWinPerBlock;
        } else {
            uint64_t npos = L >= 24 ? (uint64_t)L - 23 : 0;
            b.windows += 2 * npos;
            for (int f = 0; f < 3; f++)
                if (L - f >= 3) b.residues += 2 * (uint64_t)((L - f) / 3);
            nb = (npos + kg::kDnaPosPerBlock - 1) / kg::kDnaPosPerBlock;
        }
        b.nblocks += nb;
        if (b.nblocks > 0x7FFFFFFFull / PER) return fail(KG_ERR_LIMIT, "batch too large: more than 2^31-1 window rows; split the batch");
    }
    b.ibase[(size_t)n_seqs] = (uint32_t)b.nblocks;
    if (b.windows > 0xFFFFFF00ull) return fail(KG_ERR_LIMIT, "batch too large: more than 2^32-256 windows; split the batch");
    b.n_rows = b.nblocks * PER;
    b.n_cont = (uint64_t)n_seqs * PER;
    return KG_OK;
}

uint64_t bucket_count(uint64_t limit, uint32_t shift) { return (limit + (1ull << shift) - 1) >> shift; }

struct PartPlan {
    bool applicable = false;
    uint32_t shift = 0, buckets = 0;
    uint32_t n_chunks = 0;
    std::vector<uint64_t> clo;
    std::vector<int64_t> cseq;
    uint64_t max_chunk = 0;
    uint32_t n_wg = 0, cap = 0;
    uint64_t n_regions = 0;
    uint32_t ovf_cap = 0;
    uint32_t gshift = 10, groups_stride = 0;
    size_t next_stride = 0;
    size_t scatter_lds = 0;
    bool use_bidx = false, part_counters = false, prog_index = false;
    uint32_t probe_grid = 0, index_grid = 0, verify_grid = 0, lowc_grid = 0, ovf_grid = 0, order_grid = 0;
    uint32_t scatter_prio = 0, index_prio = 0, verify_prio = 0, index_r = 1, probe_grab = 0;
    uint32_t flush_list = 0;
    uint64_t list_slack = 0, ucap = 0, ccap = 0;
    uint32_t n_os = 0;
    bool early_totals = false, place_staged = false, debug = false;
};

template <bool AA>
int plan_partition(const kg_table *t, const BatchPlan &b, bool progress, bool counters_req, PartPlan &pl)
{
    constexpr uint32_t PER = AA ? 1 : 6;
    const uint64_t nblocks = b.nblocks;
    uint32_t shift = env_knob("KG_PART_SHIFT", 21u, 4u, 31u);
    const uint64_t qmax = (uint64_t)KG_MAX_ENCODED / (uint64_t)t->num_sigs + 1;
    while (shift > 4 && qmax >= (1ull << (32 - shift))) shift--;
    while (bucket_count(t->limit, shift) > (uint64_t)kg::kMaxBuckets) shift++;
    while (kg::scatter_lds_bytes<AA>((uint32_t)bucket_count(t->limit, shift)) > 160u * 1024) shift++;
    const bool fits = shift < 32 && qmax < (1ull << (32 - shift)) && nblocks <= (1ull << 23) && t->m35 != 0 &&
                      t->limit < (1ull << 32) - 64;
    const uint32_t mode = env_u32("KG_PARTITION", 2u);
    const bool worth = t->limit >= (64ull << 20) && b.windows >= (1ull << 27);
    if (!(fits && nblocks > 0 && (mode == 1 || (mode == 2 && worth)))) return KG_OK;
    pl.shift = shift;
    pl.buckets = (uint32_t)bucket_count(t->limit, shift);

    constexpr uint32_t WIN = AA ? 64u : 384u;
    uint32_t want = env_u32("KG_PART_CHUNKS", 4u);
    if (want < 1) want = 1;
    if (want > kMaxChunks) want = kMaxChunks;
    if (getenv("KG_PART_MIN_CHUNK_BLOCKS")) {
        const uint64_t min_chunk = std::max(1u, env_u32("KG_PART_MIN_CHUNK_BLOCKS", 600000u));
        while (want > 1 && nblocks / want < min_chunk) want--;
    } else {
        const uint32_t by_size = nblocks < 450000 ? 1u : std::max(2u, (uint32_t)std::lround(std::sqrt((double)nblocks / 325000.0)));
        want = std::min(want, std::max(1u, by_size));
    }
    pl.clo.push_back(0); pl.cseq.push_back(0);
    std::vector<double> cum;
    if (const char *tp = getenv("KG_PART_TAPER")) {
        double acc = 0;
        for (const char *q = tp; *q;) {
            char *endp = nullptr;
            const double v = strtod(q, &endp);
            if (endp == q) break;
            acc += v; cum.push_back(acc);
            q = *endp == ',' ? endp + 1 : endp;
        }
        if (cum.size() >= 2 && cum.size() <= kMaxChunks && acc > 0) { for (auto &x : cum) x /= acc; want = (uint32_t)cum.size(); }
        else cum.clear();
    }
    for (uint32_t c = 1; c < want; c++) {
        const uint64_t target = cum.empty() ? nblocks * c / want : (uint64_t)((double)nblocks * cum[c - 1]);
        const auto it = std::lower_bound(b.ibase.begin(), b.ibase.end(), (uint32_t)target);
        const uint64_t cut = *it;
        if (cut > pl.clo.back() && cut < nblocks) { pl.clo.push_back(cut); pl.cseq.push_back((int64_t)(it - b.ibase.begin())); }
    }
    pl.clo.push_back(nblocks); pl.cseq.push_back((int64_t)b.ibase.size() - 1);
    pl.n_chunks = (uint32_t)pl.clo.size() - 1;
    for (uint32_t c = 0; c < pl.n_chunks; c++) pl.max_chunk = std::max(pl.max_chunk, pl.clo[c + 1] - pl.clo[c]);
    const uint64_t max_chunk = pl.max_chunk;
    const uint64_t chunk_blocks = (max_chunk + kg::kScatterWaves - 1) / kg::kScatterWaves * kg::kScatterWaves;
    const double max_frac = (double)max_chunk / (double)nblocks;
    uint32_t n_wg = env_knob("KG_PART_WGS", 256u, 1u, kMaxGrid);
    if ((uint64_t)n_wg * kg::kScatterWaves > chunk_blocks) n_wg = (uint32_t)((chunk_blocks + kg::kScatterWaves - 1) / kg::kScatterWaves);
    const uint64_t blocks_per_wg = ((chunk_blocks + (uint64_t)n_wg * kg::kScatterWaves - 1) / ((uint64_t)n_wg * kg::kScatterWaves)) * kg::kScatterWaves;
    const double mean = (double)blocks_per_wg * WIN / (double)pl.buckets * (env_u32("KG_PART_SLACK", 100u) / 100.0);
    const uint64_t cap64 = ((uint64_t)(mean + 6.0 * std::sqrt(mean) + 32.0) + 15) / 16 * 16;
    if (cap64 >= (1ull << 24) || (uint64_t)pl.buckets * n_wg >= (1ull << 24)) return KG_OK;
    pl.n_wg = n_wg;
    pl.cap = (uint32_t)cap64;
    pl.n_regions = (uint64_t)pl.buckets * n_wg;
    pl.ovf_cap = env_u32("KG_PART_OVF_GROUPS", (uint32_t)std::min<uint64_t>(1u << 23, std::max<uint64_t>(65536, pl.n_regions * pl.cap / 16 / 8)));
    while (pl.gshift < 12 && ((max_chunk * PER) >> pl.gshift) + 2 > 8192) pl.gshift++;
    pl.groups_stride = (uint32_t)(((max_chunk * PER) >> pl.gshift) + 2);
    if (pl.groups_stride > kg::kMaxGroups) return fail(KG_ERR_LIMIT, "a chunk of the batch holds more than 2^26 window rows");
    pl.next_stride = std::max<size_t>((size_t)pl.buckets + 8, 256);
    pl.use_bidx = t->d_bidx != nullptr && !counters_req && env_u32("KG_BIDX", 1u) != 0;
    pl.part_counters = (counters_req || progress) && !pl.use_bidx;
    pl.prog_index = progress && pl.use_bidx;
    pl.scatter_lds = kg::scatter_lds_bytes<AA>(pl.buckets);
    pl.flush_list = env_knob("KG_SCATTER_FLUSH_LIST", kg::scatter_flush_list_max<AA>(), 1u, kg::scatter_flush_list_max<AA>());
    pl.probe_grid = env_knob("KG_PROBE_GRID", 256u * 8u, 8u, kMaxGrid, 8u);
    pl.index_grid = env_knob("KG_INDEX_GRID", 256u * 4u, 8u, kMaxGrid, 8u);
    pl.scatter_prio = std::min(3u, env_u32("KG_SCATTER_PRIO", 1u));
    pl.index_prio = std::min(3u, env_u32("KG_INDEX_PRIO", 2u));
    pl.verify_prio = std::min(3u, env_u32("KG_VERIFY_PRIO", pl.n_chunks == 1 ? 2u : 0u));
    uint32_t index_r = env_u32("KG_INDEX_R", 0u);
    if (index_r == 0) index_r = mean * 0.7 >= 640.0 ? 1u : mean * 0.7 >= 320.0 ? 2u : 4u;
    if (index_r != 1 && index_r != 2) index_r = 4;
    while (index_r > 1 && (n_wg % index_r != 0 || kg::kIndexN % index_r != 0)) index_r /= 2;
    pl.index_r = index_r;
    pl.verify_grid = env_knob("KG_VERIFY_GRID", 256u * 2u, 1u, kMaxGrid);
    pl.lowc_grid = env_knob("KG_LOWC_GRID", 256u, 1u, kMaxGrid);
    pl.ovf_grid = env_knob("KG_OVF_GRID", 256u, 1u, kMaxGrid);
    pl.list_slack = (uint64_t)(std::max(std::max(pl.probe_grid, pl.index_grid), pl.verify_grid) + 64) * 4 * kg::kUChunk + 4096;
    pl.ucap = ((uint64_t)((double)b.windows * t->stage_ratio * max_frac) + pl.list_slack + kg::kUChunk - 1) / kg::kUChunk * kg::kUChunk;
    pl.ccap = ((uint64_t)((double)b.windows * (t->stage_ratio * 1.25 + 0.03) * max_frac) + pl.list_slack + kg::kUChunk - 1) /
              kg::kUChunk * kg::kUChunk;
    if (test_hook("KG_TEST_TINY_LISTS")) pl.ucap = pl.ccap = kg::kUChunk;
    const uint32_t grab_unit = 256u * (uint32_t)std::max(kg::kProbeN, kg::kIndexN);
    pl.probe_grab = env_knob("KG_PROBE_GRAB", pl.cap, grab_unit, 1u << 24, grab_unit);
    pl.n_os = pl.n_chunks < 2 ? 0u : std::min(env_u32("KG_ORDER_STREAMS", 0u), kMaxOrderStreams);
    pl.early_totals = pl.n_os == 0 && env_u32("KG_EARLY_TOTALS", 1u) != 0;
    pl.order_grid = env_knob("KG_ORDER_GRID", 256u * 3u, 1u, kMaxGrid);
    pl.place_staged = pl.gshift == 10 && env_u32("KG_PLACE_STAGED", 1u) != 0;
    pl.debug = getenv("KG_DEBUG") != nullptr;
    pl.applicable = true;
    return KG_OK;
}

struct DirectPlan {
    uint32_t scan_grid, stage_chunk;
    const uint32_t *d_hbits;
    uint32_t rpg;
    uint64_t stage_cap;
};

template <bool AA>
DirectPlan plan_direct(const kg_table *t, const BatchPlan &b, bool counters)
{
    DirectPlan pl;
    pl.scan_grid = env_knob("KG_SCAN_GRID", 256u * 8u, 1u, kMaxGrid);
    pl.stage_chunk = env_knob("KG_STAGE_CHUNK", 256u, 1u, 1u << 12);
    const uint32_t filter_mode = env_u32("KG_DIRECT_FILTER", 1u);
    pl.d_hbits = (counters || filter_mode == 0 || (filter_mode == 1 && t->limit <= (4ull << 20))) ? nullptr : t->d_hbits;
    pl.rpg = AA ? 1u : env_u32("KG_SCAN_RPG", pl.d_hbits ? 6u : 3u);
    if (pl.rpg != 1 && pl.rpg != 2 && pl.rpg != 3 && pl.rpg != 6) pl.rpg = 3;
    pl.stage_cap = (uint64_t)((double)b.windows * t->stage_ratio) + 4096 + (uint64_t)pl.scan_grid * kg::kWavesPerWG * pl.stage_chunk;
    if (pl.stage_cap > 0xFFFFFF00ull) pl.stage_cap = 0xFFFFFF00ull;
    if (test_hook("KG_TEST_TINY_LISTS")) pl.stage_cap = 256;
    return pl;
}

struct AggPlan {
    uint32_t pshift;
    bool pieces_on;
    uint32_t agg_pairs;
};

AggPlan plan_aggregate()
{
    AggPlan pl;
    pl.pshift = std::min(20u, std::max(6u, env_u32("KG_AGG_BLOCK_SHIFT", 9u)));
    pl.pieces_on = env_u32("KG_AGG_PIECES", 1u) != 0;
    pl.agg_pairs = env_u32("KG_AGG_PAIRS", 1u);
    return pl;
}

}
```

### kmergutsjava_amd/csrc/kg_host_scan.hpp

```cpp
#pragma once

namespace {

struct ScanCtx {
    kg_table *t;
    kg_result *res;
    Scratch &sc;
    const BatchPlan &b;
    const uint8_t *d_seq, *h_seq;
    const int64_t *offsets;
    int64_t n_seqs;
    bool progress, counters;
    bool seq_uploaded;
    uint64_t n_hits = 0;
    int64_t *d_off = nullptr;
    uint32_t *d_ibase = nullptr;
    kg::BlockDesc *d_blocks = nullptr;
    uint32_t *d_counts = nullptr, *d_offs = nullptr, *d_bsb = nullptr;
    uint64_t *d_partial = nullptr, *d_totals = nullptr;
    kg::Progress *d_prog = nullptr;
};

int upload_seq(const ScanCtx &cx, int64_t a, int64_t b)
{
    if (cx.h_seq && b > a)
        HIP_TRY(hipMemcpyAsync(const_cast<uint8_t *>(cx.d_seq) + a, cx.h_seq + a, (size_t)(b - a), hipMemcpyHostToDevice, cx.t->stream));
    return KG_OK;
}

template <int N>
struct BlockGuard {
    Scratch &sc;
    void **slot[N];
    void release() { for (void **q : slot) { dfree(sc.t, *q); *q = nullptr; } }
    ~BlockGuard() { for (void **q : slot) if (*q) { sc.adopt(*q); *q = nullptr; } }
};

void drop_hits(kg_table *t, kg_result *res)
{
    dfree(t, res->d_hits); dfree(t, res->d_hit_slots);
    res->d_hits = nullptr; res->d_hit_slots = nullptr;
}

int send_counters(kg_table *t, const uint64_t *d_pc, const uint32_t *d_ovfc, const uint64_t *d_totals, hipStream_t s)
{
    if (d_pc) {
        HIP_TRY(hipMemcpyAsync(t->h_pin + kPinPc, d_pc, kPcWords * 8, hipMemcpyDeviceToHost, s));
        HIP_TRY(hipMemcpyAsync(t->h_pin + kPinOvf, d_ovfc, kOvfWords * kMaxChunks * 4, hipMemcpyDeviceToHost, s));
    }
    HIP_TRY(hipMemcpyAsync(t->h_pin + kPinTotals, d_totals, kTotSent * 8, hipMemcpyDeviceToHost, s));
    return KG_OK;
}

void note_totals(ScanCtx &cx, uint64_t n_hits, bool counted)
{
    kg_table *t = cx.t;
    kg_stats &st = cx.res->st;
    const uint64_t *h_tot = t->h_pin + kPinTotals;
    st.windows_valid = counted ? (int64_t)h_tot[kTotValid] : -1;
    st.slots_inspected = counted ? (int64_t)h_tot[kTotSlots] : -1;
    st.lookup_ran_off = h_tot[kTotRanOff] ? 1 : 0;
    if (cx.b.windows) {
        double ratio = (double)n_hits / (double)cx.b.windows * 1.1 + 1e-3;
        if (ratio > t->stage_ratio) t->stage_ratio = ratio > 1.0 ? 1.0 : ratio;
    }
    cx.n_hits = n_hits;
    st.n_hits = (int64_t)n_hits;
}

int progress_begin(ScanCtx &cx)
{
    kg_table *t = cx.t;
    int rc;
    if (t->limit > 0xFFFFFFFFull) return fail(KG_ERR_UNSUPPORTED, "KG_F_PROGRESS: table streams of 2^32 records or more");
    if ((rc = cx.sc.get(&cx.d_prog, 1))) return rc;
    kg::Progress h;
    for (auto &x : h.first) x = ~0ull;
    h.last_plus1 = 0; h.first_beyond = ~0ull; h.walk_ran_off = 0;
    for (auto &x : h.found_upto) x = 0;
    h.kmers_found = 0;
    for (auto &x : h.miss_max1) x = 0;
    const double n = (double)t->num_sigs;
    auto tenth = [&](uint64_t s) { return (int)(10.0 * ((double)(s + 1) / n)); };
    for (int f = 0; f <= 10; f++) {
        const unsigned __int128 num = (unsigned __int128)(uint64_t)t->num_sigs * (unsigned)f;
        uint64_t s = (uint64_t)((num + 9) / 10);
        s = s > 3 ? s - 3 : 0;
        while (tenth(s) < f) s++;
        h.lo[f] = s;
    }
    HIP_TRY(hipMemcpyAsync(cx.d_prog, &h, sizeof h, hipMemcpyHostToDevice, t->stream));
    HIP_TRY(hipStreamSynchronize(t->stream));
    return KG_OK;
}

int progress_finish(ScanCtx &cx, bool index_walks)
{
    kg_table *t = cx.t;
    int rc;
    if (index_walks)
        hipLaunchKernelGGL(kg::progress_finish_kernel, dim3(1), dim3(256), 0, t->stream, cx.d_prog, t->d_tags, t->limit);
    uint32_t *d_bitmap = nullptr;
    const uint64_t n_words = (t->limit + 31) / 32 + 1;
    if ((rc = cx.sc.get(&d_bitmap, (size_t)n_words))) return rc;
    HIP_TRY(hipMemsetAsync(d_bitmap, 0, n_words * 4, t->stream));
    if (cx.n_hits)
        hipLaunchKernelGGL(kg::mark_found_kernel, dim3((uint32_t)std::min<uint64_t>(2048, (cx.n_hits + 255) / 256)), dim3(256), 0, t->stream,
                           cx.res->d_hit_slots, cx.n_hits, d_bitmap);
    hipLaunchKernelGGL(kg::count_found_kernel, dim3((uint32_t)std::min<uint64_t>(2048, (n_words + 255) / 256)), dim3(256), 0, t->stream,
                       d_bitmap, n_words, cx.d_prog);
    return KG_OK;
}

int progress_fetch(ScanCtx &cx)
{
    kg::Progress h;
    HIP_TRY(hipMemcpy(&h, cx.d_prog, sizeof h, hipMemcpyDeviceToHost));
    kg_progress &g = cx.res->progress;
    for (int f = 0; f <= 10; f++) g.first_visited[f] = h.first[f] == ~0ull ? -1 : (int64_t)h.first[f];
    g.last_visited = (int64_t)h.last_plus1 - 1;
    g.first_beyond = h.first_beyond == ~0ull ? -1 : (int64_t)h.first_beyond;
    g.walk_ran_off = h.walk_ran_off ? 1 : 0;
    g.stream_slots = (int64_t)cx.t->limit;
    for (int f = 0; f <= 10; f++) g.found_upto[f] = g.first_visited[f] < 0 ? 0 : (int64_t)h.found_upto[f];
    g.kmers_found = (int64_t)h.kmers_found;
    cx.res->has_progress = true;
    return KG_OK;
}

struct PartBuffers {
    uint64_t *d_ent = nullptr, *d_ovf_ent = nullptr;
    uint32_t *d_fill = nullptr, *d_ovf_bucket = nullptr, *d_next = nullptr;
    uint32_t *d_ovfc = nullptr;
    uint32_t *d_lowc = nullptr;
    kg::RowGeo *d_geo = nullptr;
    uint64_t *d_pc = nullptr;
    uint32_t *d_ghist = nullptr, *d_gbase = nullptr, *d_gcur1 = nullptr, *d_gcur2 = nullptr, *d_gtile = nullptr;
    uint64_t ucap = 0, ccap = 0;
    size_t cused_stride = 0, candused_stride = 0;
    kg_hit *d_ulist = nullptr, *d_sortA = nullptr, *d_sortB = nullptr;
    uint32_t *d_cused = nullptr, *d_candused = nullptr;
    kg::CandRec *d_cand = nullptr;
};

struct ChunkView {
    uint32_t c, lo, nb;
    uint64_t *ent, *ovf_ent;
    uint32_t *fill, *next, *ovfc, *ovf_bucket;
    kg_hit *ulist, *sortA, *sortB;
    uint32_t *cused, *candused;
    kg::CandRec *cand;
    unsigned long long *ucur, *ccur;
    uint64_t *base, *ctot;
    uint32_t *ghist, *gbase, *gcur1, *gcur2, *gtile;
};

ChunkView chunk_view(const PartPlan &pl, const PartBuffers &pb, uint32_t c)
{
    ChunkView v;
    v.c = c; v.lo = (uint32_t)pl.clo[c]; v.nb = (uint32_t)(pl.clo[c + 1] - pl.clo[c]);
    v.ent = pb.d_ent + (uint64_t)c * pl.n_regions * pl.cap;
    v.fill = pb.d_fill + (uint64_t)c * pl.n_regions;
    v.next = pb.d_next + (size_t)c * pl.next_stride;
    v.ovfc = pb.d_ovfc + kOvfWords * c; v.ovf_bucket = pb.d_ovf_bucket + (size_t)c * pl.ovf_cap;
    v.ovf_ent = pb.d_ovf_ent + (size_t)c * pl.ovf_cap * kg::kGroup;
    v.ulist = pb.d_ulist + (uint64_t)c * pb.ucap;
    v.cused = pb.d_cused + c * pb.cused_stride; v.candused = pb.d_candused + c * pb.candused_stride;
    v.cand = pb.d_cand + (uint64_t)c * pb.ccap;
    v.ucur = (unsigned long long *)(pb.d_pc + kPcUcur + c); v.ccur = (unsigned long long *)(pb.d_pc + kPcCcur + c);
    v.base = pb.d_pc + kPcBase + c; v.ctot = pb.d_pc + kPcCtot + c;
    v.ghist = pb.d_ghist + (size_t)c * pl.groups_stride; v.gbase = pb.d_gbase + (size_t)c * (pl.groups_stride + 1);
    v.gcur1 = pb.d_gcur1 + (size_t)c * (kg::kHDigits + 1); v.gcur2 = pb.d_gcur2 + (size_t)c * pl.groups_stride;
    v.gtile = pb.d_gtile + (size_t)c * (kg::kHDigits + 1);
    v.sortA = pb.d_sortA + (uint64_t)c * pb.ucap; v.sortB = pb.d_sortB + (uint64_t)c * pb.ucap;
    return v;
}

int scatter_variant_of(const ScanCtx &cx)
{
    return cx.t->limit >= (uint64_t)cx.t->num_sigs ? 0 : cx.d_prog ? 2 : 1;
}
template <typename F>
void scatter_variant(int variant, F &&f)
{
    if (variant == 0) f(std::false_type{}, std::false_type{});
    else if (variant == 1) f(std::true_type{}, std::false_type{});
    else f(std::true_type{}, std::true_type{});
}

int upload_scatter_cold(const ScanCtx &cx, const PartPlan &pl, const PartBuffers &pb)
{
    kg_table *t = cx.t;
    kg::ScatterCold h[kMaxChunks] = {};
    for (uint32_t c = 0; c < pl.n_chunks; c++) {
        uint32_t *ovfc = pb.d_ovfc + kOvfWords * c;
        h[c].ovf_cursor = ovfc; h[c].ovf_bucket = pb.d_ovf_bucket + (size_t)c * pl.ovf_cap;
        h[c].ovf_ent = pb.d_ovf_ent + (size_t)c * pl.ovf_cap * kg::kGroup;
        h[c].lowc_cursor = ovfc + kOvfLowc; h[c].lowc_blocks = pb.d_lowc + pl.clo[c];
        h[c].ctr = (unsigned long long *)(cx.d_totals + kTotValid); h[c].prog = cx.d_prog;
        h[c].ovf_cap = pl.ovf_cap;
    }
    if (!t->d_cold) HIP_TRY(hipMalloc((void **)&t->d_cold, sizeof h));
    else if (!memcmp(h, t->h_cold, sizeof h)) return KG_OK;
    memcpy(t->h_cold, h, sizeof h);
    HIP_TRY(hipMemcpyAsync(t->d_cold, t->h_cold, sizeof h, hipMemcpyHostToDevice, t->stream));
    return KG_OK;
}

template <bool AA>
int chunk_passes(const ScanCtx &cx, const PartPlan &pl, const PartBuffers &pb, const ChunkView &v)
{
    kg_table *t = cx.t;
    kg::Progress *d_prog = cx.d_prog;
    unsigned long long *d_ctr = (unsigned long long *)(cx.d_totals + kTotValid);
    const hipStream_t s2 = t->stream2, s3 = t->stream3;
    uint32_t *lowc_cursor = v.ovfc + kOvfLowc, *lowc = pb.d_lowc + v.lo;
    const uint32_t limit32 = (uint32_t)std::min<uint64_t>(t->limit, 0xFFFFFFFFull);
    scatter_variant(scatter_variant_of(cx), [&](auto is_short, auto prog) {
        constexpr bool SHORT = decltype(is_short)::value, PROG = decltype(prog)::value;
        hipLaunchKernelGGL((kg::part_scatter_kernel<AA, SHORT, PROG>), dim3(pl.n_wg), dim3(kg::kWave * kg::kScatterWaves), pl.scatter_lds,
                           t->stream, cx.d_seq, cx.d_blocks, v.lo, v.nb, limit32, (uint32_t)t->num_sigs, t->m35, pl.shift, pl.buckets, pl.cap,
                           v.ent, v.fill, t->d_cold + v.c, pl.scatter_prio, pl.flush_list);
    });
    HIP_TRY(hipEventRecord(t->pev[kPevChunk + 2 * v.c], t->stream));
    HIP_TRY(hipStreamWaitEvent(s2, t->pev[kPevChunk + 2 * v.c], 0));
    hipLaunchKernelGGL((kg::lowc_blocks_kernel<AA>), dim3(pl.lowc_grid), dim3(64 * kg::kLowcWaves), 0, s2, cx.d_seq, cx.d_blocks, lowc_cursor, lowc,
                       t->limit, (uint32_t)t->num_sigs, t->m35, pl.shift, pl.n_wg, pl.cap, v.ent, v.fill, v.ovfc, pl.ovf_cap,
                       v.ovf_bucket, v.ovf_ent, d_ctr, d_prog);
    if (pl.use_bidx) {
        const uint32_t tail_start = (uint32_t)std::min<uint64_t>(t->tail_start, 0xFFFFFFFFull);
        dispatch<int, 1, 2, 4>((int)pl.index_r, [&](auto r) {
            dispatch<bool, true, false>(t->bidx_exact, [&](auto exact) {
                dispatch<bool, true, false>(pl.prog_index, [&](auto prog) {
                    constexpr int R = decltype(r)::value;
                    constexpr bool EXACT = decltype(exact)::value, PROG = decltype(prog)::value;
                    hipLaunchKernelGGL((kg::bucket_index_kernel<kg::kIndexN, R, EXACT, PROG>), dim3(pl.index_grid), dim3(256), 0, s2,
                                       t->d_bidx, tail_start, v.ent, v.fill, pl.n_wg, pl.cap, pl.buckets, pl.shift, pl.probe_grab, v.next,
                                       v.cand, v.candused, v.ccur, pb.ccap, d_ctr, pl.index_prio, PROG ? d_prog : (kg::Progress *)nullptr);
                });
            });
        });
    } else {
        dispatch<bool, true, false>(pl.part_counters, [&](auto counters) {
            constexpr bool COUNTERS = decltype(counters)::value;
            hipLaunchKernelGGL((kg::bucket_tag_kernel<COUNTERS>), dim3(pl.probe_grid), dim3(256), 0, s2, t->d_tags, t->limit,
                               (uint64_t)t->num_sigs, v.ent, v.fill, pl.n_wg, pl.cap, pl.buckets, pl.shift, pl.probe_grab, v.next, v.cand,
                               v.candused, v.ccur, pb.ccap, d_ctr, COUNTERS ? d_prog : (kg::Progress *)nullptr);
        });
    }
    HIP_TRY(hipEventRecord(t->pev[kPevChunk + 2 * v.c + 1], s2));
    HIP_TRY(hipStreamWaitEvent(s3, t->pev[kPevChunk + 2 * v.c + 1], 0));
    dispatch<int, 1, 2, 0>(pl.part_counters ? 1 : pl.prog_index ? 2 : 0, [&](auto walks) {
        constexpr bool COUNTERS = decltype(walks)::value == 1, PROG = decltype(walks)::value == 2;
        hipLaunchKernelGGL((kg::verify_kernel<AA, COUNTERS, PROG>), dim3(pl.verify_grid), dim3(256), 0, s3, t->d_entries, t->d_tags, t->limit,
                           (uint64_t)t->num_sigs, t->magic, v.cand, v.candused, v.ccur, pb.ccap, v.ulist, v.cused, v.ucur, pb.ucap, d_ctr,
                           d_prog, pl.verify_prio);
        hipLaunchKernelGGL((kg::overflow_probe_kernel<AA, COUNTERS, PROG>), dim3(pl.ovf_grid), dim3(256), 0, s3, t->d_entries, t->d_tags,
                           t->limit, (uint64_t)t->num_sigs, t->magic, v.ovf_bucket, v.ovf_ent, v.ovfc, pl.ovf_cap, pl.shift, v.ulist,
                           v.cused, v.ucur, pb.ucap, d_ctr, d_prog);
    });
    HIP_TRY(hipEventRecord(t->pev[kPevVerified + v.c], s3));
    HIP_TRY(hipGetLastError());
    return KG_OK;
}

template <bool AA>
int chunk_order(const ScanCtx &cx, const PartPlan &pl, const PartBuffers &pb, const ChunkView &v, uint64_t hits_cap)
{
    constexpr uint32_t PER = AA ? 1 : 6;
    kg_table *t = cx.t;
    kg_result *res = cx.res;
    const uint32_t c = v.c, gshift = pl.gshift;
    const bool last = c + 1 == pl.n_chunks;
    hipStream_t s = t->stream;
    if (pl.n_os) {
        s = t->ostream[c % pl.n_os];
        HIP_TRY(hipStreamWaitEvent(s, t->ev[kEvScattered], 0));
    }
    HIP_TRY(hipStreamWaitEvent(s, t->pev[kPevVerified + c], 0));
    const uint64_t row_lo = (uint64_t)v.lo * PER, row_hi = row_lo + (uint64_t)v.nb * PER;
    const uint32_t g0 = (uint32_t)(row_lo >> gshift);
    const uint32_t n_groups = v.nb ? (uint32_t)(((row_hi - 1) >> gshift) - g0 + 1) : 1u;
    hipLaunchKernelGGL(kg::hit_hist_kernel, dim3(pl.order_grid), dim3(kg::kHThreads), (size_t)n_groups * 4, s, v.ulist, v.cused, v.ucur, pb.ucap,
                       g0, 6u + gshift, n_groups, v.ghist);
    hipLaunchKernelGGL(kg::group_scan_kernel, dim3(1), dim3(kg::kGsThreads), 0, s, v.ghist, n_groups, v.gbase, v.gcur1, v.gcur2, v.ctot, v.gtile);
    if (pl.n_os && c) HIP_TRY(hipStreamWaitEvent(s, t->pev[kPevBase + c - 1], 0));
    hipLaunchKernelGGL(kg::chunk_base_kernel, dim3(1), dim3(1), 0, s, v.ctot, v.base, last ? cx.d_totals : (uint64_t *)nullptr);
    if (pl.n_os) HIP_TRY(hipEventRecord(t->pev[kPevBase + c], s));
    if (pl.early_totals && last) {
        int rc;
        if ((rc = send_counters(t, pb.d_pc, pb.d_ovfc, cx.d_totals, s))) return rc;
        HIP_TRY(hipEventRecord(t->pev[kPevTotals], s));
    }
    hipLaunchKernelGGL((kg::hit_partition_kernel<true>), dim3(pl.order_grid), dim3(kg::kHThreads), 0, s, v.ulist, v.cused, v.ucur, pb.ucap,
                       v.gbase, n_groups, g0, 6u + gshift, v.gcur1, v.sortA, pb.ucap, v.gtile);
    hipLaunchKernelGGL((kg::hit_partition_kernel<false>), dim3(pl.order_grid), dim3(kg::kHThreads), 0, s, v.sortA, v.cused, v.ucur, pb.ucap,
                       v.gbase, n_groups, g0, 6u + gshift, v.gcur2, v.sortB, pb.ucap, v.gtile);
    hipLaunchKernelGGL((kg::group_place_kernel<AA>), dim3(std::min(n_groups, 256u * 8u)), dim3(kg::kHThreads),
                       kg::group_place_lds(gshift, pl.place_staged), s,
                       v.sortB, v.gbase, n_groups, g0, gshift, (uint32_t)row_lo, (uint32_t)row_hi, pb.d_geo, (uint64_t)cx.b.n_rows,
                       pl.place_staged ? 1u : 0u, v.base, res->d_hits, hits_cap, cx.d_offs, res->d_hit_slots);
    HIP_TRY(hipGetLastError());
    return KG_OK;
}

template <bool AA>
int part_allocate(ScanCtx &cx, const PartPlan &pl, PartBuffers &pb)
{
    kg_table *t = cx.t;
    Scratch &sc = cx.sc;
    const uint32_t n_chunks = pl.n_chunks, groups_stride = pl.groups_stride;
    int rc;
    if ((rc = sc.get(&pb.d_ent, (size_t)(pl.n_regions * pl.cap * n_chunks)))) return rc;
    if ((rc = sc.get(&pb.d_fill, (size_t)pl.n_regions * n_chunks))) return rc;
    if ((rc = sc.get(&pb.d_ovf_ent, (size_t)pl.ovf_cap * kg::kGroup * n_chunks))) return rc;
    if ((rc = sc.get(&pb.d_ovf_bucket, (size_t)pl.ovf_cap * n_chunks))) return rc;
    if ((rc = sc.get(&pb.d_next, pl.next_stride * n_chunks))) return rc;
    if ((rc = sc.get(&pb.d_ovfc, kOvfWords * kMaxChunks))) return rc;
    if ((rc = sc.get(&pb.d_lowc, (size_t)cx.b.nblocks + 1))) return rc;
    if ((rc = sc.get(&pb.d_geo, (size_t)cx.b.n_rows))) return rc;
    if ((rc = sc.get(&pb.d_ghist, (size_t)groups_stride * n_chunks))) return rc;
    if ((rc = sc.get(&pb.d_gbase, (size_t)(groups_stride + 1) * n_chunks))) return rc;
    if ((rc = sc.get(&pb.d_gcur1, (size_t)(kg::kHDigits + 1) * n_chunks))) return rc;
    if ((rc = sc.get(&pb.d_gcur2, (size_t)groups_stride * n_chunks))) return rc;
    if ((rc = sc.get(&pb.d_gtile, (size_t)(kg::kHDigits + 1) * n_chunks))) return rc;
    if (kg::group_place_lds(pl.gshift, pl.gshift == 10) > t->place_lds[AA ? 1 : 0]) {
        const size_t want_lds = kg::group_place_lds(pl.gshift, pl.gshift == 10);
        HIP_TRY(hipFuncSetAttribute((const void *)kg::group_place_kernel<AA>, hipFuncAttributeMaxDynamicSharedMemorySize, (int)want_lds));
        t->place_lds[AA ? 1 : 0] = want_lds;
    }
    if (groups_stride * 4u > t->hist_lds) {
        HIP_TRY(hipFuncSetAttribute((const void *)kg::hit_hist_kernel, hipFuncAttributeMaxDynamicSharedMemorySize, (int)(groups_stride * 4u)));
        t->hist_lds = groups_stride * 4u;
    }
    if ((rc = sc.get(&pb.d_pc, kPcWords))) return rc;
    const int sv = scatter_variant_of(cx);
    if (t->scatter_lds[AA ? 1 : 0][sv] < pl.scatter_lds) {
        hipError_t e = hipSuccess;
        scatter_variant(sv, [&](auto is_short, auto prog) {
            e = hipFuncSetAttribute((const void *)kg::part_scatter_kernel<AA, decltype(is_short)::value, decltype(prog)::value>,
                                    hipFuncAttributeMaxDynamicSharedMemorySize, (int)pl.scatter_lds);
        });
        HIP_TRY(e);
        t->scatter_lds[AA ? 1 : 0][sv] = pl.scatter_lds;
    }
    return KG_OK;
}

template <bool AA>
int scan_partitioned(ScanCtx &cx, const PartPlan &pl, bool &done)
{
    constexpr uint32_t PER = AA ? 1 : 6;
    kg_table *t = cx.t;
    kg_result *res = cx.res;
    kg_stats &st = res->st;
    const uint32_t n_chunks = pl.n_chunks;
    const uint64_t nblocks = cx.b.nblocks;
    int rc;
    PartBuffers pb;
    if ((rc = part_allocate<AA>(cx, pl, pb))) return rc;
    BlockGuard<6> lists{cx.sc, {(void **)&pb.d_ulist, (void **)&pb.d_cused, (void **)&pb.d_cand, (void **)&pb.d_candused,
                                (void **)&pb.d_sortA, (void **)&pb.d_sortB}};
    pb.ucap = pl.ucap; pb.ccap = pl.ccap;
    HIP_TRY(hipEventRecord(t->ev[kEvScanBegin], t->stream));
    for (int attempt = 0; attempt < 3; attempt++) {
        const uint64_t ucap = pb.ucap, ccap = pb.ccap;
        const uint64_t hits_cap = ucap * n_chunks;
        pb.cused_stride = (size_t)(ucap / kg::kUChunk + 1); pb.candused_stride = (size_t)(ccap / kg::kUChunk + 1);
        if ((rc = dalloc(t, (void **)&res->d_hits, hits_cap * sizeof(kg_hit)))) return rc;
        if (cx.progress && (rc = dalloc(t, (void **)&res->d_hit_slots, hits_cap * 4))) return rc;
        if ((rc = dalloc(t, (void **)&pb.d_ulist, ucap * n_chunks * sizeof(kg_hit)))) return rc;
        if ((rc = dalloc(t, (void **)&pb.d_cused, pb.cused_stride * n_chunks * 4))) return rc;
        if ((rc = dalloc(t, (void **)&pb.d_cand, ccap * n_chunks * sizeof(kg::CandRec)))) return rc;
        if ((rc = dalloc(t, (void **)&pb.d_candused, pb.candused_stride * n_chunks * 4))) return rc;
        if ((rc = dalloc(t, (void **)&pb.d_sortA, ucap * n_chunks * sizeof(kg_hit)))) return rc;
        if ((rc = dalloc(t, (void **)&pb.d_sortB, ucap * n_chunks * sizeof(kg_hit)))) return rc;
        if ((rc = clear_words(t->stream, [](uint64_t most) { return (uint32_t)std::min<uint64_t>(4096, (most / 4 + 255) / 256 + 1); },
                              {{pb.d_cused, (uint64_t)pb.cused_stride * n_chunks},
                               {pb.d_candused, (uint64_t)pb.candused_stride * n_chunks},
                               {pb.d_pc, kPcWords * 2},
                               {cx.d_totals, kTotWords * 2},
                               {pb.d_ovfc, kOvfWords * kMaxChunks},
                               {pb.d_next, (uint64_t)pl.next_stride * n_chunks},
                               {pb.d_ghist, (uint64_t)pl.groups_stride * n_chunks}})))
            return rc;
        if ((rc = upload_scatter_cold(cx, pl, pb))) return rc;
        HIP_TRY(hipEventRecord(t->pev[kPevFork], t->stream));
        HIP_TRY(hipStreamWaitEvent(t->stream2, t->pev[kPevFork], 0));
        HIP_TRY(hipStreamWaitEvent(t->stream3, t->pev[kPevFork], 0));
        hipLaunchKernelGGL((kg::row_geo_kernel<AA>), dim3((uint32_t)((nblocks * PER + 255) / 256)), dim3(256), 0, t->stream3, cx.d_blocks,
                           (uint32_t)nblocks, pb.d_geo);
        for (uint32_t c = 0; c < n_chunks; c++) {
            if (!cx.seq_uploaded && (rc = upload_seq(cx, cx.offsets[pl.cseq[c]], cx.offsets[pl.cseq[c + 1]]))) return rc;
            if ((rc = chunk_passes<AA>(cx, pl, pb, chunk_view(pl, pb, c)))) return rc;
        }
        HIP_TRY(hipEventRecord(t->ev[kEvScattered], t->stream));
        cx.seq_uploaded = true;
        for (uint32_t k = 0; k < pl.n_os; k++)
            if (!t->ostream[k]) {
                int pr_least = 0, pr_greatest = 0;
                HIP_TRY(hipDeviceGetStreamPriorityRange(&pr_least, &pr_greatest));
                HIP_TRY(hipStreamCreateWithPriority(&t->ostream[k], hipStreamNonBlocking, pr_least));
            }
        for (uint32_t c = 0; c < n_chunks; c++)
            if ((rc = chunk_order<AA>(cx, pl, pb, chunk_view(pl, pb, c), hits_cap))) return rc;

        for (uint32_t k = 0; k < pl.n_os; k++) {
            HIP_TRY(hipEventRecord(t->pev[kPevOrdered + k], t->ostream[k]));
            HIP_TRY(hipStreamWaitEvent(t->stream, t->pev[kPevOrdered + k], 0));
        }
        HIP_TRY(hipEventRecord(t->pev[kPevJoin2], t->stream2));
        HIP_TRY(hipStreamWaitEvent(t->stream, t->pev[kPevJoin2], 0));
        HIP_TRY(hipEventRecord(t->pev[kPevJoin3], t->stream3));
        HIP_TRY(hipStreamWaitEvent(t->stream, t->pev[kPevJoin3], 0));
        HIP_TRY(hipEventRecord(t->ev[kEvJoined], t->stream));
        st.scan_launches++;
        HIP_TRY(hipEventRecord(t->ev[kEvScanEnd], t->stream));
        if (pl.early_totals) {
            HIP_TRY(hipEventSynchronize(t->pev[kPevTotals]));
        } else {
            if ((rc = send_counters(t, pb.d_pc, pb.d_ovfc, cx.d_totals, t->stream))) return rc;
            HIP_TRY(hipStreamSynchronize(t->stream));
        }
        const uint64_t *h_pc = t->h_pin + kPinPc;
        const uint32_t *h_ovf = reinterpret_cast<const uint32_t *>(t->h_pin + kPinOvf);
        uint64_t need_u = 0, need_c = 0;
        uint32_t max_ovf = 0, guard = 0;
        for (uint32_t c = 0; c < n_chunks; c++) {
            need_u = std::max(need_u, h_pc[kPcUcur + c]); need_c = std::max(need_c, h_pc[kPcCcur + c]);
            max_ovf = std::max(max_ovf, h_ovf[kOvfWords * c + kOvfGroups]);
            guard |= h_ovf[kOvfWords * c + kOvfGuard];
        }
        const uint64_t n_hits = h_pc[kPcBase + n_chunks];
        if (pl.debug)
            fprintf(stderr, "[kg] partition attempt %d: %u chunks (largest %llu of %llu blocks), overflow groups <= %u (cap %u), hit list <= %llu "
                            "(cap %llu), candidates <= %llu (cap %llu), regions/chunk %llu x %u entries, %u buckets, shift %u, %u scatter "
                            "workgroups, hits %llu, %s\n",
                    attempt, n_chunks, (unsigned long long)pl.max_chunk, (unsigned long long)nblocks, max_ovf, pl.ovf_cap,
                    (unsigned long long)need_u, (unsigned long long)ucap, (unsigned long long)need_c, (unsigned long long)ccap,
                    (unsigned long long)pl.n_regions, pl.cap, pl.buckets, pl.shift, pl.n_wg, (unsigned long long)n_hits, pl.use_bidx ? "byte home index" : "tags");
        const bool redo = guard || max_ovf > pl.ovf_cap || need_u > ucap || need_c > ccap;
        if (redo && pl.early_totals) HIP_TRY(hipStreamSynchronize(t->stream));
        if (guard || max_ovf > pl.ovf_cap) {
            st.fallback = guard ? 2 : 1;
            lists.release();
            drop_hits(t, res);
            return KG_OK;
        }
        if (!redo) {
            note_totals(cx, n_hits, pl.part_counters);
            st.partitioned = 1;
            st.part_chunks = (int32_t)n_chunks; st.part_buckets = (int32_t)pl.buckets; st.part_shift = (int32_t)pl.shift;
            st.part_levels = pl.use_bidx ? 4 : 1;
            done = true;
            return KG_OK;
        }
        lists.release();
        drop_hits(t, res);
        if (attempt == 2) break;
        if (need_c > ccap) { pb.ccap = (need_c + pl.list_slack + kg::kUChunk - 1) / kg::kUChunk * kg::kUChunk; pb.ucap = std::max(ucap, pb.ccap); }
        else pb.ucap = (need_u + pl.list_slack + kg::kUChunk - 1) / kg::kUChunk * kg::kUChunk;
    }
    return fail(KG_ERR_DEVICE, "hit list overflow after resize (internal error)");
}

template <bool AA>
int scan_direct(ScanCtx &cx, const DirectPlan &pl)
{
    kg_table *t = cx.t;
    kg_result *res = cx.res;
    kg_stats &st = res->st;
    const uint64_t nblocks = cx.b.nblocks, n_rows = cx.b.n_rows;
    int rc;
    st.scan_launches = 0;
    if (!cx.seq_uploaded) { if ((rc = upload_seq(cx, cx.offsets[0], cx.offsets[cx.n_seqs]))) return rc; cx.seq_uploaded = true; }
    uint64_t stage_cap = pl.stage_cap;
    kg_hit *d_stage = nullptr;
    uint32_t *d_stage_slot = nullptr;
    BlockGuard<2> stage{cx.sc, {(void **)&d_stage, (void **)&d_stage_slot}};
    unsigned long long *d_cursor = (unsigned long long *)(cx.d_totals + kTotCursor);
    unsigned long long *d_ctr = (unsigned long long *)(cx.d_totals + kTotValid);
    for (int attempt = 0;; attempt++) {
        if ((rc = dalloc(t, (void **)&d_stage, stage_cap * sizeof(kg_hit)))) return rc;
        if (cx.progress && (rc = dalloc(t, (void **)&d_stage_slot, stage_cap * 4))) return rc;
        HIP_TRY(hipMemsetAsync(cx.d_totals, 0, kTotWords * 8, t->stream));
        HIP_TRY(hipEventRecord(t->ev[kEvScanBegin], t->stream));
        if (nblocks) {
            const uint64_t wgs = (nblocks + kg::kWavesPerWG - 1) / kg::kWavesPerWG;
            const uint32_t grid = (uint32_t)(wgs < pl.scan_grid ? wgs : pl.scan_grid);
            dispatch<bool, true, false>(cx.counters, [&](auto counters) {
                dispatch<int, 1, 2, 3, 6>((int)pl.rpg, [&](auto rpg) {
                    constexpr bool COUNTERS = decltype(counters)::value;
                    constexpr int RPG = AA ? 1 : decltype(rpg)::value;
                    hipLaunchKernelGGL((kg::scan_kernel<AA, COUNTERS, RPG>), dim3(grid), dim3(kg::kWave * kg::kWavesPerWG), 0, t->stream,
                                       t->d_entries, t->d_tags, t->limit, (uint64_t)t->num_sigs, t->magic, t->m35, cx.d_seq, cx.d_blocks,
                                       (uint32_t)nblocks, cx.d_counts, cx.d_bsb, d_stage, d_cursor, stage_cap, pl.stage_chunk, d_ctr, cx.d_prog,
                                       d_stage_slot, pl.d_hbits, t->tail_start);
                });
            });
            HIP_TRY(hipGetLastError());
        }
        HIP_TRY(hipEventRecord(t->ev[kEvScanEnd], t->stream));
        st.scan_launches++;
        if ((rc = prefix_sum(t, cx.d_counts, n_rows, cx.d_offs, cx.d_partial, cx.d_totals + kTotHits))) return rc;
        if ((rc = send_counters(t, nullptr, nullptr, cx.d_totals, t->stream))) return rc;
        HIP_TRY(hipStreamSynchronize(t->stream));
        const uint64_t need = t->h_pin[kPinTotals + kTotCursor];
        if (need <= stage_cap) break;
        stage.release();
        if (attempt == 1) return fail(KG_ERR_DEVICE, "staging overflow after resize (internal error)");
        stage_cap = need;
    }
    const uint64_t n_hits = n_rows ? t->h_pin[kPinTotals + kTotHits] : 0;
    note_totals(cx, n_hits, cx.counters);

    if ((rc = dalloc(t, (void **)&res->d_hits, n_hits * sizeof(kg_hit)))) return rc;
    if (cx.progress && (rc = dalloc(t, (void **)&res->d_hit_slots, (n_hits ? n_hits : 1) * 4))) return rc;
    if (nblocks) {
        const uint32_t grid = (uint32_t)((nblocks + kg::kWavesPerWG - 1) / kg::kWavesPerWG);
        hipLaunchKernelGGL((kg::place_kernel<AA>), dim3(grid), dim3(kg::kWave * kg::kWavesPerWG), 0, t->stream, cx.d_blocks,
                           (uint32_t)nblocks, cx.d_counts, cx.d_offs, cx.d_bsb, pl.rpg, d_stage, res->d_hits, d_stage_slot, res->d_hit_slots);
    }
    return KG_OK;
}

template <bool AA>
int scan_impl(kg_table *t, const kg_params *p, const uint8_t *d_seq, const uint8_t *h_seq ,
              const int64_t *offsets, int64_t n_seqs, kg_result *res)
{
    constexpr uint32_t PER = AA ? 1 : 6;
    const bool progress = (p->flags & KG_F_PROGRESS) != 0;
    const bool counters_req = (p->flags & KG_F_COUNTERS) != 0;
    const bool aggregate = !(p->flags & KG_F_SKIP_AGGREGATE);
    kg_stats &st = res->st;
    res->per = PER;
    int rc;

    BatchPlan b;
    if ((rc = plan_batch<AA>(offsets, n_seqs, b))) return rc;
    const uint64_t nblocks = b.nblocks, n_rows = b.n_rows, n_cont = b.n_cont;
    st.n_seqs = n_seqs; st.n_containers = (int64_t)n_cont; st.n_blocks = (int64_t)nblocks;
    st.residues = (int64_t)b.residues; st.windows = (int64_t)b.windows;
    st.table_bytes = t->num_sigs * (int64_t)KG_TABLE_ENTRY_SIZE;

    Scratch sc(t);
    ScanCtx cx{t, res, sc, b, d_seq, h_seq, offsets, n_seqs, progress, counters_req || progress, h_seq == nullptr};
    if ((rc = sc.get(&cx.d_off, (size_t)n_seqs + 1))) return rc;
    if ((rc = sc.get(&cx.d_ibase, (size_t)n_seqs + 1))) return rc;
    HIP_TRY(hipMemcpyAsync(cx.d_off, offsets, ((size_t)n_seqs + 1) * 8, hipMemcpyHostToDevice, t->stream));
    HIP_TRY(hipMemcpyAsync(cx.d_ibase, b.ibase.data(), ((size_t)n_seqs + 1) * 4, hipMemcpyHostToDevice, t->stream));
    if ((rc = sc.get(&cx.d_blocks, nblocks))) return rc;
    if ((rc = sc.get(&cx.d_counts, n_rows))) return rc;
    if ((rc = sc.get(&cx.d_offs, n_rows))) return rc;
    if ((rc = sc.get(&cx.d_bsb, nblocks * 6))) return rc;
    if ((rc = sc.get(&cx.d_partial, (size_t)(std::max(n_rows, n_cont) / kg::kScanChunk + 2)))) return rc;
    if ((rc = sc.get(&cx.d_totals, kTotWords))) return rc;
    HIP_TRY(hipMemsetAsync(cx.d_totals, 0, kTotWords * 8, t->stream));
    if ((rc = dalloc(t, (void **)&res->d_chs, (n_cont + 1) * 8))) return rc;
    if (progress && (rc = progress_begin(cx))) return rc;
    HIP_TRY(hipEventRecord(t->ev[kEvBegin], t->stream));
    if (nblocks) {
        hipLaunchKernelGGL(kg::build_blocks_kernel, dim3((uint32_t)((nblocks + 255) / 256)), dim3(256), 0, t->stream,
                           cx.d_off, cx.d_ibase, (uint32_t)n_seqs, (uint32_t)nblocks, cx.d_blocks);
        HIP_TRY(hipGetLastError());
    }

    st.scan_launches = 0;
    PartPlan part;
    if ((rc = plan_partition<AA>(t, b, progress, counters_req, part))) return rc;
    bool part_done = false;
    if (part.applicable && (rc = scan_partitioned<AA>(cx, part, part_done))) return rc;
    if (!part_done && (rc = scan_direct<AA>(cx, plan_direct<AA>(t, b, cx.counters)))) return rc;

    if (progress && (rc = progress_finish(cx, part_done && part.prog_index))) return rc;
    hipLaunchKernelGGL((kg::container_starts_kernel<AA>), dim3((uint32_t)((n_cont + 1 + 255) / 256)), dim3(256), 0, t->stream,
                       cx.d_ibase, (uint32_t)n_seqs, cx.d_offs, n_rows, cx.d_totals, res->d_chs);
    HIP_TRY(hipGetLastError());
    HIP_TRY(hipEventRecord(t->ev[kEvOrderEnd], t->stream));

    if (aggregate && (rc = aggregate_stage(t, p, res, sc, n_seqs, n_cont, cx.n_hits, PER, cx.d_partial, cx.d_totals, nullptr, b.longest < (1ll << 30),
                                         plan_aggregate())))
        return rc;
    HIP_TRY(hipEventRecord(t->ev[kEvAggEnd], t->stream));
    HIP_TRY(hipStreamSynchronize(t->stream));
    st.n_calls = aggregate ? (int64_t)t->h_pin[kPinCalls] : 0;
    if (progress && (rc = progress_fetch(cx))) return rc;
    st.agg_pieces = aggregate ? (int32_t)std::min<uint64_t>(t->h_pin[kPinPieces], 0x7FFFFFFF) : 0;
    float ms = 0;
    HIP_TRY(hipEventElapsedTime(&ms, t->ev[kEvScanBegin], t->ev[kEvScanEnd])); st.ms_scan = ms;
    HIP_TRY(hipEventElapsedTime(&ms, t->ev[kEvScanEnd], t->ev[kEvOrderEnd])); st.ms_order = ms;
    HIP_TRY(hipEventElapsedTime(&ms, t->ev[kEvOrderEnd], t->ev[kEvAggEnd])); st.ms_aggregate = ms;
    HIP_TRY(hipEventElapsedTime(&ms, t->ev[kEvBegin], t->ev[kEvAggEnd])); st.ms_total = ms;
    if (st.partitioned) {
        HIP_TRY(hipEventElapsedTime(&ms, t->ev[kEvScanBegin], t->ev[kEvScattered])); st.ms_part_scatter = ms;
        st.ms_part_tag = 0;
        HIP_TRY(hipEventElapsedTime(&ms, t->ev[kEvScattered], t->ev[kEvJoined])); st.ms_part_verify = ms;
    }
    return KG_OK;
}

int scan_entry(kg_table *t, const kg_params *p, const uint8_t *seq, bool on_device, const int64_t *offsets, int64_t n_seqs,
               kg_result **out)
{
    if (!t || !p || !offsets || !out || n_seqs < 0) return fail(KG_ERR_ARG, "null or negative argument");
    if (n_seqs > 0x7FFFFFF0ll / 6) return fail(KG_ERR_LIMIT, "too many sequences in one batch");
    if (p->min_hits < 2)
        return fail(KG_ERR_UNSUPPORTED, "minHits < 2: the reference throws in processSetOfHits (KGJ:442); refusing");
    CallScope cs(t, "another kg_scan* is in flight on this kg_table (one scan at a time per table; open a second table "
                    "object for concurrent scans)");
    if (cs.rc) return cs.rc;
    int64_t total = offsets[n_seqs] - offsets[0];
    if (total < 0) return fail(KG_ERR_ARG, "offsets must be non-decreasing");
    if (!seq && total > 0) return fail(KG_ERR_ARG, "null sequence buffer");
    kg_result *r = new (std::nothrow) kg_result();
    if (!r) return fail(KG_ERR_NOMEM, "out of host memory");
    r->tab = t;
    uint8_t *d_seq = nullptr;
    int rc = KG_OK;
    if (!on_device) {
        size_t end = (size_t)offsets[n_seqs];
        rc = dalloc(t, (void **)&d_seq, end + 16);
    }
    if (rc == KG_OK) {
        const uint8_t *s = on_device ? seq : d_seq;
        const uint8_t *h = on_device ? nullptr : seq;
        rc = p->aa ? scan_impl<true>(t, p, s, h, offsets, n_seqs, r) : scan_impl<false>(t, p, s, h, offsets, n_seqs, r);
    }
    (void)hipStreamSynchronize(t->stream);
    if (d_seq) dfree(t, d_seq);
    if (rc != KG_OK) return fail_and_free(r, rc);
    *out = r;
    return KG_OK;
}

}

extern "C" {

int kg_scan(kg_table *t, const kg_params *p, const uint8_t *seq, const int64_t *offsets, int64_t n_seqs, kg_result **out)
{
    return scan_entry(t, p, seq, false, offsets, n_seqs, out);
}

int kg_scan_device(kg_table *t, const kg_params *p, const uint8_t *d_seq, const int64_t *offsets, int64_t n_seqs,
                   kg_result **out)
{
    return scan_entry(t, p, d_seq, true, offsets, n_seqs, out);
}

}
```

### kmergutsjava_amd/csrc/kg_host_table.hpp

```cpp
#pragma once

namespace {

int table_finish(kg_table *t)
{
    HIP_TRY(hipSetDevice(t->device));
    HIP_TRY(hipDeviceSynchronize());
    unsigned __int128 one = 1;
    if (t->num_sigs == 1) t->magic = ~0ull;
    else t->magic = (uint64_t)((one << 64) / (unsigned __int128)(uint64_t)t->num_sigs);
    t->m35 = (t->num_sigs >= 64 && t->num_sigs < (1ll << 31)) ? (uint32_t)((1ull << 35) / (uint64_t)t->num_sigs) : 0u;
    uint64_t n_tags = t->limit + kg::kTagPad;
    HIP_TRY(hipMalloc((void **)&t->d_tags, n_tags));
    unsigned long long *d_occ = nullptr;
    HIP_TRY(hipMalloc((void **)&d_occ, 16));
    HIP_TRY(hipMemsetAsync(d_occ, 0, 16, t->stream));
    uint64_t want = (n_tags + 255) / 256;
    uint32_t grid = (uint32_t)(want < 256ull * 16 ? (want ? want : 1) : 256ull * 16);
    hipLaunchKernelGGL(kg::build_tags_kernel, dim3(grid), dim3(256), 0, t->stream, t->d_entries, t->limit, n_tags,
                       (uint64_t)t->num_sigs, t->magic, t->d_tags, d_occ);
    HIP_TRY(hipGetLastError());
    t->bidx_exact = (uint64_t)KG_MAX_ENCODED / (uint64_t)t->num_sigs + 1 <= kg::kBidxClasses;
    if (t->m35 != 0 && t->limit > 0) {
        const uint64_t n_bidx = t->limit + kg::kTagPad;
// ... 4 lines not shown
        HIP_TRY(hipGetLastError());
        if (n_bidx <= kHbitsMaxSlots) {
            const uint64_t n_words = (n_bidx + 31) / 32;
            HIP_TRY(hipMalloc((void **)&t->d_hbits, n_words * 4));
            hipLaunchKernelGGL(kg::build_hbits_kernel, dim3((uint32_t)std::min<uint64_t>((n_words + 255) / 256, 256ull * 32)), dim3(256), 0, t->stream,
                               t->d_bidx, n_bidx, t->d_hbits, n_words);
            HIP_TRY(hipGetLastError());
        }
    }
    unsigned long long occ[2] = {0, 0};
    HIP_TRY(hipMemcpyAsync(occ, d_occ, 16, hipMemcpyDeviceToHost, t->stream));
    HIP_TRY(hipStreamSynchronize(t->stream));
    HIP_TRY(hipFree(d_occ));
    t->occupied = occ[0];
    t->tail_start = occ[1];
    for (auto &e : t->pev) HIP_TRY(hipEventCreateWithFlags(&e, hipEventDisableTiming));
    HIP_TRY(hipStreamCreateWithFlags(&t->stream2, hipStreamNonBlocking));
    HIP_TRY(hipStreamCreateWithFlags(&t->stream3, hipStreamNonBlocking));
    return KG_OK;
}

int table_new(int device, kg_table **out)
{
    int ndev = 0;
    if (hipGetDeviceCount(&ndev) != hipSuccess || ndev <= 0)
        return fail(KG_ERR_DEVICE, "no HIP device: libkmerguts_hip needs an MI355X (gfx950) GPU; there is no CPU path");
    if (device < 0 || device >= ndev) return fail(KG_ERR_ARG, "device index out of range");
    HIP_TRY(hipSetDevice(device));
    kg_table *t = new (std::nothrow) kg_table();
    if (!t) return fail(KG_ERR_NOMEM, "out of host memory");
    t->device = device;
    hipError_t e = hipStreamCreateWithFlags(&t->stream, hipStreamNonBlocking);
    if (e == hipSuccess) e = hipHostMalloc((void **)&t->h_pin, kPinWords * 8);
    for (auto &ev : t->ev)
        if (e == hipSuccess) e = hipEventCreate(&ev);
    if (e != hipSuccess) { kg_table_close(t); return fail(KG_ERR_DEVICE, std::string("hipStreamCreate / hipEventCreate: ") + hipGetErrorString(e)); }
    *out = t;
    return KG_OK;
}

int64_t rd_i64le(const uint8_t *b)
{
    uint64_t v = 0;
    for (int i = 7; i >= 0; i--) v = (v << 8) | b[i];
    return (int64_t)v;
}

int parse_header(const uint8_t *hdr, kg_table *t)
{
    t->num_sigs = rd_i64le(hdr);
    t->entry_size = rd_i64le(hdr + 8);
    t->version = rd_i64le(hdr + 16);
    if (t->num_sigs <= 0) return fail(KG_ERR_FORMAT, "kmer table header: numSigs <= 0");
    if (t->entry_size != KG_TABLE_ENTRY_SIZE)
        return fail(KG_ERR_FORMAT, "kmer table header: entrySize != 24 (the reference reads 24-byte records, KGJ:995-999)");
    return KG_OK;
}

bool write_all(int fd, gzFile g, const uint8_t *p, size_t n)
{
    while (n) {
        const size_t piece = std::min<size_t>(n, 1u << 30);
        long got;
        if (g) got = gzwrite(g, p, (unsigned)piece);
        else got = (long)write(fd, p, piece);
        if (got <= 0) {
            if (!g && got < 0 && errno == EINTR) continue;
            return false;
        }
        p += got;
        n -= (size_t)got;
    }
    return true;
}

}

extern "C" {

const char *kg_last_error(void) { return g_err.c_str(); }
const char *kg_version(void) { return "libkmerguts_hip 0.1.0 gfx950"; }

int kg_table_from_memory(const void *image, size_t nbytes, int device, kg_table **out)
{
    if (!image || !out) return fail(KG_ERR_ARG, "null argument");
    if (nbytes < 24) return fail(KG_ERR_FORMAT, "kmer table image shorter than its 24-byte header");
    kg_table *t = nullptr;
    int rc = table_new(device, &t);
    if (rc) return rc;
    rc = parse_header((const uint8_t *)image, t);
    if (rc) { kg_table_close(t); return rc; }
    t->limit = (nbytes - 24) / KG_TABLE_ENTRY_SIZE;
    size_t bytes = (size_t)t->limit * KG_TABLE_ENTRY_SIZE;
    t->own_entries = true;
    hipError_t e = hipMalloc((void **)&t->d_entries, bytes ? bytes : 256);
    if (e != hipSuccess) { kg_table_close(t); return fail(KG_ERR_NOMEM, std::string("hipMalloc(table): ") + hipGetErrorString(e)); }
    if (bytes) {
        e = hipMemcpy(t->d_entries, (const uint8_t *)image + 24, bytes, hipMemcpyHostToDevice);
        if (e != hipSuccess) { kg_table_close(t); return fail(KG_ERR_DEVICE, std::string("hipMemcpy(table): ") + hipGetErrorString(e)); }
    }
    rc = table_finish(t);
    if (rc) { kg_table_close(t); return rc; }
    *out = t;
    return KG_OK;
}

static int open_gz(const char *path, int device, kg_table **out)
{
    gzFile g = gzopen(path, "rb");
    if (!g) return fail(KG_ERR_IO, std::string("cannot open ") + path + ": " + strerror(errno));
    gzbuffer(g, 1u << 20);
    uint8_t hdr[24];
    if (gzread(g, hdr, 24) != 24) { gzclose(g); return fail(KG_ERR_FORMAT, "kmer table file shorter than its 24-byte header"); }
    kg_table *t = nullptr;
    int rc = table_new(device, &t);
    if (rc) { gzclose(g); return rc; }
    rc = parse_header(hdr, t);
    if (rc) { gzclose(g); kg_table_close(t); return rc; }
    size_t cap = (size_t)t->num_sigs * KG_TABLE_ENTRY_SIZE;
    if (cap < 256) cap = 256;
    t->own_entries = true;
    hipError_t e = hipMalloc((void **)&t->d_entries, cap);
    if (e != hipSuccess) { gzclose(g); kg_table_close(t); return fail(KG_ERR_NOMEM, std::string("hipMalloc(table): ") + hipGetErrorString(e)); }
    const size_t CH = 64u << 20;
    uint8_t *pin[2] = {nullptr, nullptr};
    hipEvent_t done[2];
    bool ok = hipHostMalloc((void **)&pin[0], CH) == hipSuccess && hipHostMalloc((void **)&pin[1], CH) == hipSuccess &&
              hipEventCreate(&done[0]) == hipSuccess && hipEventCreate(&done[1]) == hipSuccess;
    size_t at = 0;
    int which = 0;
    bool used[2] = {false, false};
    std::string why;
    while (ok) {
        if (used[which]) ok = hipEventSynchronize(done[which]) == hipSuccess;
        if (!ok) break;
        size_t n = 0;
        while (n < CH) {
            const int got = gzread(g, pin[which] + n, (unsigned)std::min<size_t>(CH - n, 1u << 30));
            if (got < 0) { int en = 0; why = gzerror(g, &en); ok = false; break; }
            if (got == 0) break;
            n += (size_t)got;
        }
        if (!ok || n == 0) break;
        if (at + n > cap) {
            size_t ncap = std::max(at + n, cap + cap / 2);
            uint8_t *bigger = nullptr;
            ok = hipStreamSynchronize(t->stream) == hipSuccess && hipMalloc((void **)&bigger, ncap) == hipSuccess &&
                 hipMemcpy(bigger, t->d_entries, at, hipMemcpyDeviceToDevice) == hipSuccess;
            if (!ok) { if (bigger) (void)hipFree(bigger); why = "out of device memory for a table longer than its header says"; break; }
            (void)hipFree(t->d_entries);
            t->d_entries = bigger; cap = ncap;
        }
        ok = hipMemcpyAsync(t->d_entries + at, pin[which], n, hipMemcpyHostToDevice, t->stream) == hipSuccess &&
             hipEventRecord(done[which], t->stream) == hipSuccess;
        used[which] = true;
        at += n;
        which ^= 1;
    }
    if (ok) ok = hipStreamSynchronize(t->stream) == hipSuccess;
    gzclose(g);
    if (pin[0]) (void)hipHostFree(pin[0]);
    if (pin[1]) (void)hipHostFree(pin[1]);
    (void)hipEventDestroy(done[0]);
    (void)hipEventDestroy(done[1]);
    if (!ok) { kg_table_close(t); return fail(KG_ERR_IO, "inflating/uploading the kmer table failed" + (why.empty() ? std::string() : ": " + why)); }
    t->limit = at / KG_TABLE_ENTRY_SIZE;
    rc = table_finish(t);
    if (rc) { kg_table_close(t); return rc; }
    *out = t;
    return KG_OK;
}

int kg_table_open(const char *path, int device, kg_table **out)
{
    if (!path || !out) return fail(KG_ERR_ARG, "null argument");
    FILE *f = fopen(path, "rb");
    if (!f) return fail(KG_ERR_IO, std::string("cannot open ") + path + ": " + strerror(errno));
    uint8_t hdr[24];
    const size_t got_hdr = fread(hdr, 1, 24, f);
    if (got_hdr >= 2 && hdr[0] == 0x1f && hdr[1] == 0x8b) {
        fclose(f);
        return open_gz(path, device, out);
    }
    if (got_hdr != 24) { fclose(f); return fail(KG_ERR_FORMAT, "kmer table file shorter than its 24-byte header"); }
    if (fseeko(f, 0, SEEK_END) != 0) { fclose(f); return fail(KG_ERR_IO, "fseek failed"); }
    off_t fsz = ftello(f);
    fclose(f);
    kg_table *t = nullptr;
    int rc = table_new(device, &t);
    if (rc) return rc;
    rc = parse_header(hdr, t);
    if (rc) { kg_table_close(t); return rc; }
    t->limit = (uint64_t)(fsz - 24) / KG_TABLE_ENTRY_SIZE;
    size_t bytes = (size_t)t->limit * KG_TABLE_ENTRY_SIZE;
    t->own_entries = true;
    hipError_t e = hipMalloc((void **)&t->d_entries, bytes ? bytes : 256);
    if (e != hipSuccess) { kg_table_close(t); return fail(KG_ERR_NOMEM, std::string("hipMalloc(table): ") + hipGetErrorString(e)); }
    const int fd = open(path, O_RDONLY);
    if (fd < 0) { kg_table_close(t); return fail(KG_ERR_IO, std::string("cannot open ") + path + ": " + strerror(errno)); }
    const size_t CH = 32u << 20;
    const size_t n_pieces = (bytes + CH - 1) / CH;
    const unsigned hw = std::thread::hardware_concurrency();
    const size_t n_thr = std::max<size_t>(1, std::min<size_t>({(size_t)8, (size_t)(hw ? hw : 4), n_pieces}));
    std::atomic<size_t> next{0};
    std::atomic<bool> ok{true};
    std::mutex err_mu;
    std::string why;
    auto worker = [&]() {
        if (hipSetDevice(device) != hipSuccess) { ok = false; return; }
        hipStream_t s = nullptr;
        uint8_t *pin[2] = {nullptr, nullptr};
        hipEvent_t done[2] = {nullptr, nullptr};
        bool good = hipStreamCreateWithFlags(&s, hipStreamNonBlocking) == hipSuccess &&
                    hipHostMalloc((void **)&pin[0], CH) == hipSuccess && hipHostMalloc((void **)&pin[1], CH) == hipSuccess &&
                    hipEventCreate(&done[0]) == hipSuccess && hipEventCreate(&done[1]) == hipSuccess;
        bool used[2] = {false, false};
        int which = 0;
        while (good && ok.load()) {
            const size_t k = next.fetch_add(1);
            if (k >= n_pieces) break;
            const size_t at = k * CH, n = std::min(CH, bytes - at);
            if (used[which]) good = hipEventSynchronize(done[which]) == hipSuccess;
            size_t got = 0;
            while (good && got < n) {
                const ssize_t r = pread(fd, pin[which] + got, n - got, (off_t)(24 + at + got));
                if (r <= 0) { std::lock_guard<std::mutex> lk(err_mu); why = "short read on kmer table file"; good = false; break; }
                got += (size_t)r;
            }
            if (!good) break;
            good = hipMemcpyAsync(t->d_entries + at, pin[which], n, hipMemcpyHostToDevice, s) == hipSuccess &&
                   hipEventRecord(done[which], s) == hipSuccess;
            used[which] = true;
            which ^= 1;
        }
        if (s) (void)hipStreamSynchronize(s);
        if (!good) ok = false;
        for (int i = 0; i < 2; i++) { if (pin[i]) (void)hipHostFree(pin[i]); if (done[i]) (void)hipEventDestroy(done[i]); }
        if (s) (void)hipStreamDestroy(s);
    };
    {
        std::vector<std::thread> pool;
        for (size_t i = 1; i < n_thr; i++) pool.emplace_back(worker);
        worker();
        for (auto &th : pool) th.join();
    }
    close(fd);
    if (!ok.load()) { kg_table_close(t); return fail(KG_ERR_IO, "reading/uploading the kmer table failed" + (why.empty() ? std::string() : ": " + why)); }
    rc = table_finish(t);
    if (rc) { kg_table_close(t); return rc; }
    *out = t;
    return KG_OK;
}

int kg_table_from_device(const void *d_entries, int64_t num_sigs, int device, kg_table **out)
{
    if (!d_entries || !out) return fail(KG_ERR_ARG, "null argument");
    if (num_sigs <= 0) return fail(KG_ERR_ARG, "num_sigs <= 0");
    kg_table *t = nullptr;
    int rc = table_new(device, &t);
    if (rc) return rc;
    t->num_sigs = num_sigs;
    t->entry_size = KG_TABLE_ENTRY_SIZE;
    t->version = 1;
    t->limit = (uint64_t)num_sigs;
    t->own_entries = false;
    t->d_entries = (uint8_t *)d_entries;
    rc = table_finish(t);
    if (rc) { kg_table_close(t); return rc; }
    *out = t;
    return KG_OK;
}

int kg_table_info(const kg_table *t, int64_t *num_sigs, int64_t *entry_size, int64_t *version, int64_t *occupied)
{
    if (!t) return fail(KG_ERR_ARG, "null table");
    if (num_sigs) *num_sigs = t->num_sigs;
    if (entry_size) *entry_size = t->entry_size;
    if (version) *version = t->version;
    if (occupied) *occupied = (int64_t)t->occupied;
    return KG_OK;
}

void kg_table_close(kg_table *t)
{
    if (!t) return;
    (void)hipSetDevice(t->device);
    if (t->stream) (void)hipStreamSynchronize(t->stream);
    if (t->own_entries && t->d_entries) (void)hipFree(t->d_entries);
    if (t->d_tags) (void)hipFree(t->d_tags);
    if (t->d_bidx) (void)hipFree(t->d_bidx);
    if (t->d_hbits) (void)hipFree(t->d_hbits);
    if (t->d_cold) (void)hipFree(t->d_cold);
    if (t->d_calls_cold) (void)hipFree(t->d_calls_cold);
    t->cache.release_all();
    t->pins.release_all();
    if (t->h_pin) (void)hipHostFree(t->h_pin);
    for (auto &e : t->ev)
        if (e) (void)hipEventDestroy(e);
    for (auto &e : t->pev)
        if (e) (void)hipEventDestroy(e);
    if (t->stream2) { (void)hipStreamSynchronize(t->stream2); (void)hipStreamDestroy(t->stream2); }
    if (t->stream3) { (void)hipStreamSynchronize(t->stream3); (void)hipStreamDestroy(t->stream3); }
    for (auto &os : t->ostream) if (os) { (void)hipStreamSynchronize(os); (void)hipStreamDestroy(os); }
    if (t->stream) (void)hipStreamDestroy(t->stream);
    delete t;
}

int64_t kg_table_live_device_bytes(kg_table *t)
{
    return t ? (int64_t)t->cache.live_bytes() : 0;
}

const void *kg_table_device_entries(const kg_table *t) { return t ? t->d_entries : nullptr; }
int64_t kg_table_records(const kg_table *t) { return t ? (int64_t)t->limit : 0; }

int kg_table_save(kg_table *t, const char *path)
{
    if (!t || !path) return fail(KG_ERR_ARG, "null argument");
    CallScope cs(t, "a kg_scan* is in flight on this kg_table");
    if (cs.rc) return cs.rc;
    const size_t plen = strlen(path);
    const bool gz = plen >= 3 && strcmp(path + plen - 3, ".gz") == 0;
    std::string tmp = std::string(path) + ".tmpXXXXXX";
    const int fd = mkstemp(&tmp[0]);
    if (fd < 0) return fail(KG_ERR_IO, std::string("cannot create a file next to ") + path + ": " + strerror(errno));
    const mode_t um = umask(0);
    umask(um);
    (void)fchmod(fd, 0666 & ~um);
    gzFile g = nullptr;
    bool ok = true;
    std::string why;
    if (gz) {
        g = gzdopen(fd, "wb1");
        if (!g) { ok = false; why = "gzdopen failed"; }
    }
    uint8_t hdr[24];
    const int64_t h3[3] = {t->num_sigs, t->entry_size, t->version};
    for (int f = 0; f < 3; f++)
        for (int b = 0; b < 8; b++) hdr[f * 8 + b] = (uint8_t)((uint64_t)h3[f] >> (8 * b));
    if (ok && !write_all(fd, g, hdr, 24)) { ok = false; why = strerror(errno); }
    const size_t bytes = (size_t)t->limit * KG_TABLE_ENTRY_SIZE, CH = 32u << 20;
    const size_t n_pieces = (bytes + CH - 1) / CH;
    void *pin[2] = {nullptr, nullptr};
    hipEvent_t done[2] = {nullptr, nullptr};
    if (ok && n_pieces) {
        ok = t->pins.get(&pin[0], CH) == hipSuccess && t->pins.get(&pin[1], CH) == hipSuccess &&
             hipEventCreateWithFlags(&done[0], hipEventDisableTiming) == hipSuccess &&
             hipEventCreateWithFlags(&done[1], hipEventDisableTiming) == hipSuccess;
        if (!ok) why = "pinned staging allocation failed";
    }
    auto issue = [&](size_t k) {
        const size_t at = k * CH, n = std::min(CH, bytes - at);
        return hipMemcpyAsync(pin[k & 1], t->d_entries + at, n, hipMemcpyDeviceToHost, t->stream) == hipSuccess &&
               hipEventRecord(done[k & 1], t->stream) == hipSuccess;
    };
    if (ok && n_pieces && !issue(0)) { ok = false; why = "device-to-host copy failed"; }
    for (size_t k = 0; ok && k < n_pieces; k++) {
        if (k + 1 < n_pieces && !issue(k + 1)) { ok = false; why = "device-to-host copy failed"; break; }
        if (hipEventSynchronize(done[k & 1]) != hipSuccess) { ok = false; why = "device-to-host copy failed"; break; }
        if (!write_all(fd, g, (const uint8_t *)pin[k & 1], std::min(CH, bytes - k * CH))) { ok = false; why = strerror(errno); }
    }
    (void)hipStreamSynchronize(t->stream);
    for (int i = 0; i < 2; i++) {
        if (pin[i]) t->pins.put(pin[i]);
        if (done[i]) (void)hipEventDestroy(done[i]);
    }
    if (g) {
        if (gzclose(g) != Z_OK && ok) { ok = false; why = "gzip stream could not be completed"; }
    } else if (close(fd) != 0 && ok) {
        ok = false;
        why = strerror(errno);
    }
    if (ok && rename(tmp.c_str(), path) != 0) { ok = false; why = std::string("rename: ") + strerror(errno); }
    if (!ok) {
        (void)unlink(tmp.c_str());
        return fail(KG_ERR_IO, std::string("writing ") + path + " failed" + (why.empty() ? std::string() : ": " + why));
    }
    return KG_OK;
}

}
```

Baseline: 132.5 billion residues/s.

## Run CALL aggregation per chunk on a side stream and vectorize voter kernels

Splits the aggregation stage into begin, slice and finish steps so that container starts, piece starts and call walking can run on each partition chunk as soon as its hits are placed. That work goes on a low-priority side stream, or on the order streams, overlapping the remaining scan. The early path sits behind a KG_AGG_EARLY environment flag that defaults to off, so by default a single full-range slice runs as before. The voter count and scatter kernels are also rewritten to read votes 16 bytes per lane over 1024-hit tiles with grid-stride waves, aiming to cut per-byte loads and launch width; this adds extra shuffles and more complex range and piece indexing.

```diff
diff --git a/kmergutsjava_amd/csrc/kg_aggregate.hpp b/kmergutsjava_amd/csrc/kg_aggregate.hpp
--- a/kmergutsjava_amd/csrc/kg_aggregate.hpp
+++ b/kmergutsjava_amd/csrc/kg_aggregate.hpp
@@ -128,16 +128,21 @@
 constexpr uint32_t kPairMaxContainer = 39000;
 
 __global__ __launch_bounds__(256) void piece_starts_kernel(const kg_hit *__restrict__ hits, const int64_t *__restrict__ chs,
-                                                           uint32_t n_hits, uint32_t pshift, int32_t max_gap,
+                                                           const uint64_t *__restrict__ range, uint32_t lo_h, uint32_t hi_h, uint32_t last,
+                                                           uint32_t pshift, int32_t max_gap,
                                                            uint32_t *__restrict__ piece_start, uint8_t *__restrict__ piece_pair ,
                                                            uint32_t n_blocks, uint32_t pairs_ok)
 {
     const int lane = threadIdx.x & 63;
-    const uint32_t u = (uint32_t)uni((int32_t)(blockIdx.x * 4 + (threadIdx.x >> 6)));
-    if (u >= n_blocks) return;
+    const uint32_t k = (uint32_t)uni((int32_t)(blockIdx.x * 4 + (threadIdx.x >> 6)));
+    const uint32_t lo = range ? (uint32_t)range[0] : lo_h, n_hits = range ? (uint32_t)range[1] : hi_h;
+    if (k >= n_blocks || n_hits <= lo) return;
+    const uint32_t u = (lo >> pshift) + k;
+    if (u > (n_hits - 1u) >> pshift) return;
     uint32_t found = kNoPiece;
     const uint32_t blk = 1u << pshift, i0 = u << pshift;
-    if (u > 0 && i0 < n_hits) {
+    const bool whole = i0 >= lo && ((uint64_t)i0 + blk <= n_hits || last);
+    if (whole && u > 0 && i0 < n_hits) {
         const uint32_t c0 = hits[i0].container;
         const uint32_t lo0 = (uint32_t)chs[c0], hi0 = (uint32_t)chs[c0 + 1];
         const bool long_enough = hi0 - lo0 >= 2u * blk || hi0 < i0 + blk;
@@ -158,7 +163,7 @@
         if (found - lo < blk / 2 || hi - found < blk / 2) found = kNoPiece;
     }
     uint32_t pair = 0;
-    if (found == kNoPiece && pairs_ok && u > 0 && i0 < n_hits) {
+    if (found == kNoPiece && pairs_ok && whole && u > 0 && i0 < n_hits) {
         const uint32_t c0 = hits[i0].container;
         const uint32_t lo0 = (uint32_t)chs[c0], hi0 = (uint32_t)chs[c0 + 1];
         if (hi0 - lo0 >= 2u * blk && hi0 - lo0 < kPairMaxContainer) {
@@ -219,6 +224,9 @@
     uint32_t *call_cnt, *first_cnt, *piece_cnt;
     uint8_t *before_ev;
     const uint8_t *piece_pair;
+    const uint64_t *range;
+    uint64_t own_range[2];
+    uint32_t c_lo;
 };
 
 __device__ __forceinline__ uint32_t walk_unit(const kg_hit *__restrict__ hits, const AggParams &p, uint8_t *acc, uint8_t *vote,
@@ -411,8 +419,11 @@
     const int lane = threadIdx.x & 63;
     const uint32_t w = (uint32_t)uni((int32_t)(blockIdx.x * 4 + (threadIdx.x >> 6)));
     if (w >= n_cwaves) {
-        const uint32_t u = w - n_cwaves;
-        if (u >= n_pblocks) return;
+        if (w - n_cwaves >= n_pblocks) return;
+        const uint64_t *range = cold->range;
+        const uint32_t lo = (uint32_t)range[0], hi = (uint32_t)range[1];
+        const uint32_t u = (uint32_t)uni((int32_t)((lo >> pshift) + (w - n_cwaves)));
+        if (hi <= lo || u > (hi - 1u) >> pshift) return;
         const uint32_t begin = piece_start[u];
         if (begin == kNoPiece) return;
         const uint32_t c = hits[begin].container;
@@ -422,13 +433,13 @@
         const uint32_t ncalls = walk_unit(hits, p, acc, vote, begin, end, c, cold->staged + begin / (uint32_t)p.min_hits, piece_start, pshift,
                                           cold, &tail, &reached_end);
         if (lane == 0) {
-            cold->piece_cnt[u] = ncalls;
+            cold->piece_cnt[begin >> pshift] = ncalls;
             if (ncalls) atomicAdd(&cold->call_cnt[c], ncalls);
             if (reached_end) cold->tail_ev[c] = (uint8_t)tail;
         }
         return;
     }
-    const uint32_t c_first = w * per_wave;
+    const uint32_t c_first = cold->c_lo + w * per_wave;
     uint32_t my_begin = 0, my_end = 0;
     const bool mine = (uint32_t)lane < per_wave && c_first + (uint32_t)lane < n_cont;
     if (mine) { my_begin = (uint32_t)chs[c_first + lane]; my_end = (uint32_t)chs[c_first + lane + 1]; }
@@ -512,22 +523,55 @@
     ccs[c] = c == n_cont ? (int64_t)*total : (int64_t)call_off[c];
 }
 
+constexpr uint32_t kVoteTile = 1024;
+
+__device__ __forceinline__ uint32_t vote_bits16(const uint8_t *__restrict__ vote, uint64_t i0, uint32_t n_hits)
+{
+    if (i0 >= n_hits) return 0u;
+    const uint4 v = *reinterpret_cast<const uint4 *>(vote + i0);
+    auto nibble = [](uint32_t w) {
+        const uint32_t nz = (((w & 0x7F7F7F7Fu) + 0x7F7F7F7Fu) | w) & 0x80808080u;
+        return (((nz >> 7) * 0x00204081u) >> 21) & 0xFu;
+    };
+    uint32_t m = nibble(v.x) | nibble(v.y) << 4 | nibble(v.z) << 8 | nibble(v.w) << 12;
+    const uint64_t left = (uint64_t)n_hits - i0;
+    if (left < 16u) m &= (1u << (uint32_t)left) - 1u;
+    return m;
+}
+
 __global__ __launch_bounds__(256) void voter_count_kernel(const uint8_t *__restrict__ vote, uint32_t n_hits, uint32_t *__restrict__ cnt)
 {
-    const uint32_t i = blockIdx.x * blockDim.x + threadIdx.x;
-    const uint64_t m = __ballot(i < n_hits && vote[i] != 0);
-    if ((threadIdx.x & 63) == 0 && (i & ~63u) < n_hits) cnt[i >> 6] = (uint32_t)__popcll(m);
-    if (i == 0) cnt[(n_hits + 63u) >> 6] = 0;
+    const uint32_t lane = threadIdx.x & 63u;
+    const uint32_t wave = (uint32_t)uni((int32_t)(blockIdx.x * 4 + (threadIdx.x >> 6))), n_waves = gridDim.x * 4;
+    const uint32_t n_tiles = (uint32_t)(((uint64_t)n_hits + kVoteTile - 1) / kVoteTile), n_chunks = (uint32_t)(((uint64_t)n_hits + 63u) >> 6);
+    for (uint32_t tile = wave; tile < n_tiles; tile += n_waves) {
+        uint32_t c = (uint32_t)__popc(vote_bits16(vote, (uint64_t)tile * kVoteTile + lane * 16u, n_hits));
+        c += (uint32_t)__shfl_xor((int)c, 1);
+        c += (uint32_t)__shfl_xor((int)c, 2);
+        const uint32_t chunk = tile * (kVoteTile / 64) + (lane >> 2);
+        if ((lane & 3u) == 0 && chunk < n_chunks) cnt[chunk] = c;
+    }
+    if (blockIdx.x == 0 && threadIdx.x == 0) cnt[n_chunks] = 0;
 }
 
 __global__ __launch_bounds__(256) void voter_scatter_kernel(const kg_hit *__restrict__ hits, const uint8_t *__restrict__ vote,
                                                             uint32_t n_hits, const uint32_t *__restrict__ voff, int32_t *__restrict__ vlist)
 {
-    const uint32_t i = blockIdx.x * blockDim.x + threadIdx.x;
-    const int lane = threadIdx.x & 63;
-    const bool v = i < n_hits && vote[i] != 0;
-    const uint64_t m = __ballot(v);
-    if (v) vlist[voff[i >> 6] + (uint32_t)__popcll(m & ((1ull << lane) - 1ull))] = hits[i].oI;
+    const uint32_t lane = threadIdx.x & 63u;
+    const uint32_t wave = (uint32_t)uni((int32_t)(blockIdx.x * 4 + (threadIdx.x >> 6))), n_waves = gridDim.x * 4;
+    const uint32_t n_tiles = (uint32_t)(((uint64_t)n_hits + kVoteTile - 1) / kVoteTile);
+    for (uint32_t tile = wave; tile < n_tiles; tile += n_waves) {
+        const uint32_t m16 = vote_bits16(vote, (uint64_t)tile * kVoteTile + lane * 16u, n_hits);
+        if (!__ballot(m16 != 0)) continue;
+        for (uint32_t s = 0; s < kVoteTile / 64; s++) {
+            const uint32_t bits = (uint32_t)__shfl((int)m16, (int)(s * 4 + (lane >> 4)));
+            const bool v = ((bits >> (lane & 15u)) & 1u) != 0;
+            const uint64_t m = __ballot(v);
+            if (!m) continue;
+            const uint32_t chunk = tile * (kVoteTile / 64) + s;
+            if (v) vlist[voff[chunk] + (uint32_t)__popcll(m & ((1ull << lane) - 1ull))] = hits[(uint64_t)chunk * 64u + lane].oI;
+        }
+    }
 }
 
 __global__ __launch_bounds__(256) void otu_wave_kernel(const int32_t *__restrict__ vlist, const uint32_t *__restrict__ voff,
diff --git a/kmergutsjava_amd/csrc/kg_device.hpp b/kmergutsjava_amd/csrc/kg_device.hpp
--- a/kmergutsjava_amd/csrc/kg_device.hpp
+++ b/kmergutsjava_amd/csrc/kg_device.hpp
@@ -949,11 +949,11 @@
 }
 
 template <bool AA>
-__global__ void container_starts_kernel(const uint32_t *ibase, uint32_t n_seqs, const uint32_t *offs, uint64_t n_rows,
+__global__ void container_starts_kernel(const uint32_t *ibase, uint32_t seq_lo, uint32_t n_seqs, const uint32_t *offs, uint64_t n_rows,
                                         const uint64_t *total, int64_t *chs)
 {
     constexpr uint32_t PER = AA ? 1 : 6;
-    uint64_t c = (uint64_t)blockIdx.x * blockDim.x + threadIdx.x;
+    uint64_t c = (uint64_t)seq_lo * PER + (uint64_t)blockIdx.x * blockDim.x + threadIdx.x;
     uint64_t n_cont = (uint64_t)n_seqs * PER;
     if (c > n_cont) return;
     if (c == n_cont) { chs[c] = (int64_t)*total; return; }
diff --git a/kmergutsjava_amd/csrc/kg_host.hpp b/kmergutsjava_amd/csrc/kg_host.hpp
--- a/kmergutsjava_amd/csrc/kg_host.hpp
+++ b/kmergutsjava_amd/csrc/kg_host.hpp
@@ -171,10 +171,13 @@
     kPevVerified = 20,
     kPevBase = 32,
     kPevOrdered = 40,
-    kPevCount = 48
+    kPevPlaced = 48,
+    kPevSliced = 56,
+    kPevCount = 57
 };
 static_assert(kPevChunk + 2 * kMaxChunks <= kPevFork && kPevVerified + kMaxChunks <= kPevBase && kPevBase + kMaxChunks <= kPevOrdered &&
-              kPevOrdered + kMaxOrderStreams <= kPevCount, "event slots overlap");
+              kPevOrdered + kMaxOrderStreams <= kPevPlaced && kPevPlaced + kMaxChunks <= kPevSliced && kPevSliced < kPevCount,
+              "event slots overlap");
 enum : int { kEvBegin = 0, kEvScanBegin = 1, kEvScanEnd = 2, kEvOrderEnd = 3, kEvAggEnd = 4, kEvScattered = 5 , kEvSpare = 6,
              kEvJoined = 7 , kEvCount = 8, kEvStageBegin = kEvBegin, kEvStageEnd = kEvScanBegin };
 enum : int { kTotHits = 0, kTotCursor = 1 , kTotValid = 2, kTotSlots = 3 ,
@@ -200,6 +203,7 @@
     hipStream_t stream2 = nullptr;
     hipStream_t stream3 = nullptr;
     hipStream_t ostream[kMaxOrderStreams] = {};
+    hipStream_t sstream = nullptr;
     hipEvent_t pev[kPevCount] = {};
     bool own_entries = false;
     uint8_t *d_entries = nullptr;
@@ -218,7 +222,7 @@
     kg::ScatterCold *d_cold = nullptr;
     kg::ScatterCold h_cold[kMaxChunks] = {};
     kg::CallsCold *d_calls_cold = nullptr;
-    kg::CallsCold h_calls_cold = {};
+    kg::CallsCold h_calls_cold[kMaxChunks] = {};
     size_t hist_lds = 48 * 1024;
     size_t place_lds[2] = {48 * 1024, 48 * 1024};
     hipEvent_t ev[kEvCount] = {};
@@ -370,6 +374,7 @@
         if (t->stream2) (void)hipStreamSynchronize(t->stream2);
         if (t->stream3) (void)hipStreamSynchronize(t->stream3);
         for (auto &os : t->ostream) if (os) (void)hipStreamSynchronize(os);
+        if (t->sstream) (void)hipStreamSynchronize(t->sstream);
         for (void *p : ptrs) dfree(t, p);
     }
     void adopt(void *p) { ptrs.push_back(p); }
diff --git a/kmergutsjava_amd/csrc/kg_host_aggregate.hpp b/kmergutsjava_amd/csrc/kg_host_aggregate.hpp
--- a/kmergutsjava_amd/csrc/kg_host_aggregate.hpp
+++ b/kmergutsjava_amd/csrc/kg_host_aggregate.hpp
@@ -2,61 +2,109 @@
 
 namespace {
 
-int aggregate_stage(kg_table *t, const kg_params *p, kg_result *res, Scratch &sc, int64_t n_seqs, uint64_t n_cont, uint64_t n_hits,
-                    uint32_t PER, uint64_t *d_partial, uint64_t *d_totals, const kg_otu *d_otu_init, bool allow_pieces, const AggPlan &ag)
-{
-    int rc;
-    kg::AggParams ap;
-    ap.min_hits = p->min_hits; ap.min_weighted_hits = p->min_weighted_hits;
-    ap.max_gap = p->max_gap; ap.order_constraint = p->order_constraint ? 1 : 0;
-    uint32_t *d_ccnt = nullptr, *d_coff = nullptr, *d_first = nullptr;
+struct AggRun {
+    bool begun = false, pieces = false;
+    kg::AggParams ap = {};
+    AggPlan ag = {};
+    uint64_t n_cont = 0, cap = 0;
+    uint32_t cpw = 1;
+    uint32_t n_slices = 0;
+    uint32_t *d_ccnt = nullptr, *d_coff = nullptr, *d_first = nullptr, *d_pstart = nullptr, *d_pcnt = nullptr;
     kg_call *d_staged = nullptr;
-    uint8_t *d_vote = nullptr;
-    if ((rc = dalloc(t, (void **)&res->d_ev, n_hits))) return rc;
+    uint8_t *d_vote = nullptr, *d_before = nullptr, *d_ppair = nullptr;
+};
+
+int agg_begin(kg_table *t, const kg_params *p, kg_result *res, Scratch &sc, AggRun &ar, uint64_t n_cont, uint64_t cap, bool allow_pieces,
+              const AggPlan &ag)
+{
+    int rc;
+    ar = AggRun();
+    ar.ap.min_hits = p->min_hits; ar.ap.min_weighted_hits = p->min_weighted_hits;
+    ar.ap.max_gap = p->max_gap; ar.ap.order_constraint = p->order_constraint ? 1 : 0;
+    ar.ag = ag; ar.n_cont = n_cont; ar.cap = cap;
+    if ((rc = dalloc(t, (void **)&res->d_ev, cap))) return rc;
     if ((rc = dalloc(t, (void **)&res->d_tail_ev, n_cont))) return rc;
-    uint8_t *d_acc = res->d_ev;
-    if ((rc = sc.get(&d_ccnt, n_cont))) return rc;
-    if ((rc = sc.get(&d_first, n_cont))) return rc;
-    if ((rc = sc.get(&d_coff, n_cont))) return rc;
-    if ((rc = sc.get(&d_vote, n_hits))) return rc;
-    if ((rc = sc.get(&d_staged, (size_t)(n_hits / (uint64_t)p->min_hits + 1)))) return rc;
+    if ((rc = sc.get(&ar.d_ccnt, n_cont))) return rc;
+    if ((rc = sc.get(&ar.d_first, n_cont))) return rc;
+    if ((rc = sc.get(&ar.d_coff, n_cont))) return rc;
+    if ((rc = sc.get(&ar.d_vote, cap + 16))) return rc;
+    if ((rc = sc.get(&ar.d_staged, (size_t)(cap / (uint64_t)p->min_hits + 1)))) return rc;
+    ar.pieces = allow_pieces && !p->order_constraint && p->max_gap >= 0 && p->max_gap < (1 << 30) && n_cont &&
+                cap > (2ull << ag.pshift) && ag.pieces_on;
+    const uint32_t n_pblocks = ar.pieces ? (uint32_t)((cap + (1ull << ag.pshift) - 1) >> ag.pshift) : 0u;
+    t->h_pin[kPinCalls] = 0;
+    t->h_pin[kPinPieces] = 0;
+    if (ar.pieces) {
+        if ((rc = sc.get(&ar.d_pstart, (size_t)n_pblocks + 1))) return rc;
+        if ((rc = sc.get(&ar.d_pcnt, (size_t)n_pblocks + 1))) return rc;
+        if ((rc = sc.get(&ar.d_before, ((size_t)n_pblocks + 4) & ~(size_t)3))) return rc;
+        if ((rc = sc.get(&ar.d_ppair, ((size_t)n_pblocks + 4) & ~(size_t)3))) return rc;
+    }
+    ar.cpw = (uint32_t)std::min<uint64_t>(16, std::max<uint64_t>(1, n_cont / (1u << 17)));
+    if ((rc = clear_words(t->stream, [](uint64_t most) { return (uint32_t)std::min<uint64_t>(1024, most / 1024 + 1); },
+                          {{ar.d_ccnt, n_cont}, {ar.d_pcnt, ar.pieces ? (uint64_t)n_pblocks + 1 : 0},
+                           {ar.d_before, ar.pieces ? ((uint64_t)n_pblocks + 4) / 4 : 0}})))
+        return rc;
+    ar.begun = true;
+    return KG_OK;
+}
+
+void agg_drop(kg_table *t, kg_result *res, AggRun &ar)
+{
+    if (!ar.begun) return;
+    dfree(t, res->d_ev); dfree(t, res->d_tail_ev);
+    res->d_ev = nullptr; res->d_tail_ev = nullptr;
+    ar = AggRun();
+}
+
+int agg_slice(kg_table *t, kg_result *res, AggRun &ar, hipStream_t stream, uint64_t c_lo, uint64_t c_hi, const uint64_t *d_range,
+              uint64_t lo, uint64_t hi, bool last, uint64_t max_records)
+{
+    if (c_hi <= c_lo) return KG_OK;
+    if (ar.n_slices >= kMaxChunks) return fail(KG_ERR_DEVICE, "more CALL slices than chunks (internal error)");
+    const uint32_t k = ar.n_slices++;
+    const uint32_t pshift = ar.ag.pshift;
+    const uint32_t n_pblocks = ar.pieces && max_records ? (uint32_t)(((max_records - 1) >> pshift) + 2) : 0u;
+    if (n_pblocks)
+        hipLaunchKernelGGL(kg::piece_starts_kernel, dim3((n_pblocks + 3) / 4), dim3(256), 0, stream, res->d_hits, res->d_chs, d_range,
+                           (uint32_t)lo, (uint32_t)hi, last ? 1u : 0u, pshift, ar.ap.max_gap, ar.d_pstart, ar.d_ppair, n_pblocks, ar.ag.agg_pairs);
+    const uint32_t n_cwaves = (uint32_t)((c_hi - c_lo + ar.cpw - 1) / ar.cpw);
+    kg::CallsCold cold;
+    memset(&cold, 0, sizeof cold);
+    cold.staged = ar.d_staged; cold.tail_ev = res->d_tail_ev; cold.call_cnt = ar.d_ccnt; cold.first_cnt = ar.d_first;
+    cold.piece_cnt = ar.d_pcnt; cold.before_ev = ar.d_before; cold.piece_pair = ar.d_ppair;
+    if (!t->d_calls_cold) {
+        HIP_TRY(hipMalloc((void **)&t->d_calls_cold, sizeof t->h_calls_cold));
+        memset(t->h_calls_cold, 0, sizeof t->h_calls_cold);
+    }
+    cold.own_range[0] = lo; cold.own_range[1] = hi; cold.c_lo = (uint32_t)c_lo;
+    cold.range = d_range ? d_range : t->d_calls_cold[k].own_range;
+    if (memcmp(&cold, &t->h_calls_cold[k], sizeof cold)) {
+        t->h_calls_cold[k] = cold;
+        HIP_TRY(hipMemcpyAsync(t->d_calls_cold + k, &t->h_calls_cold[k], sizeof cold, hipMemcpyHostToDevice, stream));
+    }
+    hipLaunchKernelGGL(kg::calls_wave_kernel, dim3((n_cwaves + n_pblocks + 3) / 4), dim3(256), 0, stream, res->d_hits, res->d_chs,
+                       (uint32_t)c_hi, ar.ap, res->d_ev, ar.d_vote, ar.cpw, n_cwaves, ar.d_pstart, pshift, n_pblocks, t->d_calls_cold + k);
+    HIP_TRY(hipGetLastError());
+    return KG_OK;
+}
+
+int agg_finish(kg_table *t, const kg_params *p, kg_result *res, Scratch &sc, AggRun &ar, int64_t n_seqs, uint64_t n_hits, uint32_t PER,
+               uint64_t *d_partial, uint64_t *d_totals, const kg_otu *d_otu_init)
+{
+    int rc;
+    const uint64_t n_cont = ar.n_cont;
+    const AggPlan &ag = ar.ag;
+    uint32_t *d_ccnt = ar.d_ccnt, *d_coff = ar.d_coff, *d_first = ar.d_first, *d_pstart = ar.d_pstart, *d_pcnt = ar.d_pcnt;
+    uint8_t *d_vote = ar.d_vote;
+    const bool pieces = ar.pieces;
+    const uint32_t n_pblocks = pieces ? (uint32_t)((n_hits + (1ull << ag.pshift) - 1) >> ag.pshift) : 0u;
     if ((rc = dalloc(t, (void **)&res->d_ccs, (n_cont + 1) * 8))) return rc;
     if ((rc = dalloc(t, (void **)&res->d_otu, (size_t)(n_seqs ? n_seqs : 1) * sizeof(kg_otu)))) return rc;
-    const bool pieces = allow_pieces && !p->order_constraint && p->max_gap >= 0 && p->max_gap < (1 << 30) && n_cont &&
-                        n_hits > (2ull << ag.pshift) && ag.pieces_on;
-    const uint32_t n_pblocks = pieces ? (uint32_t)((n_hits + (1ull << ag.pshift) - 1) >> ag.pshift) : 0u;
-    uint32_t *d_pstart = nullptr, *d_pcnt = nullptr;
-    uint8_t *d_before = nullptr, *d_ppair = nullptr;
-    t->h_pin[kPinCalls] = 0;
-    t->h_pin[kPinPieces] = 0;
-    if (pieces) {
-        if ((rc = sc.get(&d_pstart, (size_t)n_pblocks + 1))) return rc;
-        if ((rc = sc.get(&d_pcnt, (size_t)n_pblocks + 1))) return rc;
-        if ((rc = sc.get(&d_before, ((size_t)n_pblocks + 4) & ~(size_t)3))) return rc;
-        if ((rc = sc.get(&d_ppair, ((size_t)n_pblocks + 4) & ~(size_t)3))) return rc;
-    }
-    if ((rc = clear_words(t->stream, [](uint64_t most) { return (uint32_t)std::min<uint64_t>(1024, most / 1024 + 1); },
-                          {{d_ccnt, n_cont}, {d_pcnt, pieces ? (uint64_t)n_pblocks + 1 : 0}, {d_before, pieces ? ((uint64_t)n_pblocks + 4) / 4 : 0}})))
-        return rc;
-    if (pieces)
-        hipLaunchKernelGGL(kg::piece_starts_kernel, dim3((n_pblocks + 3) / 4), dim3(256), 0, t->stream, res->d_hits, res->d_chs,
-                           (uint32_t)n_hits, ag.pshift, ap.max_gap, d_pstart, d_ppair, n_pblocks, ag.agg_pairs);
-    const uint32_t cpw = (uint32_t)std::min<uint64_t>(16, std::max<uint64_t>(1, n_cont / (1u << 17)));
-    const uint32_t n_cwaves = (uint32_t)((n_cont + cpw - 1) / cpw);
-    if (n_cont) {
-        const kg::CallsCold cold = {d_staged, res->d_tail_ev, d_ccnt, d_first, d_pcnt, d_before, d_ppair};
-        if (!t->d_calls_cold || memcmp(&cold, &t->h_calls_cold, sizeof cold)) {
-            if (!t->d_calls_cold) HIP_TRY(hipMalloc((void **)&t->d_calls_cold, sizeof cold));
-            t->h_calls_cold = cold;
-            HIP_TRY(hipMemcpyAsync(t->d_calls_cold, &t->h_calls_cold, sizeof cold, hipMemcpyHostToDevice, t->stream));
-        }
-        hipLaunchKernelGGL(kg::calls_wave_kernel, dim3((n_cwaves + n_pblocks + 3) / 4), dim3(256), 0, t->stream, res->d_hits, res->d_chs,
-                           (uint32_t)n_cont, ap, d_acc, d_vote, cpw, n_cwaves, d_pstart, ag.pshift, n_pblocks, t->d_calls_cold);
-        if (pieces)
-            hipLaunchKernelGGL(kg::merge_before_kernel, dim3((n_pblocks + 255) / 256), dim3(256), 0, t->stream, d_pstart, d_ppair, d_before,
-                               n_pblocks, res->d_ev, (unsigned long long *)(d_totals + kTotPieces));
-        HIP_TRY(hipGetLastError());
-    }
+    if (n_cont && n_pblocks)
+        hipLaunchKernelGGL(kg::merge_before_kernel, dim3((n_pblocks + 255) / 256), dim3(256), 0, t->stream, d_pstart, ar.d_ppair, ar.d_before,
+                           n_pblocks, res->d_ev, (unsigned long long *)(d_totals + kTotPieces));
+    HIP_TRY(hipGetLastError());
     if ((rc = prefix_sum(t, d_ccnt, n_cont, d_coff, d_partial, d_totals + kTotCalls))) return rc;
     if (n_cont) HIP_TRY(hipMemcpyAsync(t->h_pin + kPinCalls, d_totals + kTotCalls, 8, hipMemcpyDeviceToHost, t->stream));
     if (pieces) HIP_TRY(hipMemcpyAsync(t->h_pin + kPinPieces, d_totals + kTotPieces, 8, hipMemcpyDeviceToHost, t->stream));
@@ -70,7 +118,7 @@
         if ((rc = sc.get(&d_vlist, (size_t)n_hits + 1))) return rc;
         if ((rc = sc.get(&d_vpartial, (size_t)((n_vchunks + 1) / kg::kScanChunk + 2)))) return rc;
         if (n_hits) {
-            const uint32_t vgrid = (uint32_t)((n_hits + 255) / 256);
+            const uint32_t vgrid = (uint32_t)std::min<uint64_t>(256u * 8u, ((n_hits + kg::kVoteTile - 1) / kg::kVoteTile + 3) / 4);
             hipLaunchKernelGGL(kg::voter_count_kernel, dim3(vgrid), dim3(256), 0, t->stream, d_vote, (uint32_t)n_hits, d_vcnt);
             if ((rc = prefix_sum(t, d_vcnt, (uint64_t)n_vchunks + 1, d_voff, d_vpartial, d_totals + kTotVoters))) return rc;
             hipLaunchKernelGGL(kg::voter_scatter_kernel, dim3(vgrid), dim3(256), 0, t->stream, res->d_hits, d_vote, (uint32_t)n_hits, d_voff,
@@ -88,15 +136,25 @@
     if (n_cont) {
         if (n_cont < (1u << 17))
             hipLaunchKernelGGL((kg::compact_calls_kernel<64>), dim3((uint32_t)((n_cont * 64 + 255) / 256)), dim3(256), 0, t->stream,
-                               d_staged, res->d_chs, d_first, d_coff, (uint32_t)n_cont, (uint32_t)p->min_hits, res->d_calls,
+                               ar.d_staged, res->d_chs, d_first, d_coff, (uint32_t)n_cont, (uint32_t)p->min_hits, res->d_calls,
                                d_pstart, d_pcnt, ag.pshift);
         else
             hipLaunchKernelGGL((kg::compact_calls_kernel<1>), dim3((uint32_t)((n_cont + 255) / 256)), dim3(256), 0, t->stream,
-                               d_staged, res->d_chs, d_first, d_coff, (uint32_t)n_cont, (uint32_t)p->min_hits, res->d_calls,
+                               ar.d_staged, res->d_chs, d_first, d_coff, (uint32_t)n_cont, (uint32_t)p->min_hits, res->d_calls,
                                d_pstart, d_pcnt, ag.pshift);
     }
     HIP_TRY(hipGetLastError());
     return KG_OK;
+}
+
+int aggregate_stage(kg_table *t, const kg_params *p, kg_result *res, Scratch &sc, int64_t n_seqs, uint64_t n_cont, uint64_t n_hits,
+                    uint32_t PER, uint64_t *d_partial, uint64_t *d_totals, const kg_otu *d_otu_init, bool allow_pieces, const AggPlan &ag)
+{
+    int rc;
+    AggRun ar;
+    if ((rc = agg_begin(t, p, res, sc, ar, n_cont, n_hits, allow_pieces, ag))) return rc;
+    if ((rc = agg_slice(t, res, ar, t->stream, 0, n_cont, nullptr, 0, n_hits, true, n_hits))) return rc;
+    return agg_finish(t, p, res, sc, ar, n_seqs, n_hits, PER, d_partial, d_totals, d_otu_init);
 }
 
 int aggregate_records(kg_table *t, const kg_params *p, const kg_hit *hits, const int64_t *container_hit_start, int64_t n_seqs,
diff --git a/kmergutsjava_amd/csrc/kg_host_plan.hpp b/kmergutsjava_amd/csrc/kg_host_plan.hpp
--- a/kmergutsjava_amd/csrc/kg_host_plan.hpp
+++ b/kmergutsjava_amd/csrc/kg_host_plan.hpp
@@ -74,6 +74,7 @@
     uint64_t list_slack = 0, ucap = 0, ccap = 0;
     uint32_t n_os = 0;
     bool early_totals = false, place_staged = false, debug = false;
+    bool agg_early = false;
 };
 
 template <bool AA>
@@ -172,6 +173,7 @@
     pl.probe_grab = env_knob("KG_PROBE_GRAB", pl.cap, grab_unit, 1u << 24, grab_unit);
     pl.n_os = pl.n_chunks < 2 ? 0u : std::min(env_u32("KG_ORDER_STREAMS", 0u), kMaxOrderStreams);
     pl.early_totals = pl.n_os == 0 && env_u32("KG_EARLY_TOTALS", 1u) != 0;
+    pl.agg_early = pl.n_chunks >= 2 && env_u32("KG_AGG_EARLY", 0u) != 0;
     pl.order_grid = env_knob("KG_ORDER_GRID", 256u * 3u, 1u, kMaxGrid);
     pl.place_staged = pl.gshift == 10 && env_u32("KG_PLACE_STAGED", 1u) != 0;
     pl.debug = getenv("KG_DEBUG") != nullptr;
diff --git a/kmergutsjava_amd/csrc/kg_host_scan.hpp b/kmergutsjava_amd/csrc/kg_host_scan.hpp
--- a/kmergutsjava_amd/csrc/kg_host_scan.hpp
+++ b/kmergutsjava_amd/csrc/kg_host_scan.hpp
@@ -19,6 +19,10 @@
     uint32_t *d_counts = nullptr, *d_offs = nullptr, *d_bsb = nullptr;
     uint64_t *d_partial = nullptr, *d_totals = nullptr;
     kg::Progress *d_prog = nullptr;
+    const kg_params *p = nullptr;
+    AggRun *agg = nullptr;
+    uint64_t last_c_lo = 0, slice_cap = 0;
+    const uint64_t *d_last_range = nullptr;
 };
 
 int upload_seq(const ScanCtx &cx, int64_t a, int64_t b)
@@ -301,6 +305,24 @@
                        v.sortB, v.gbase, n_groups, g0, gshift, (uint32_t)row_lo, (uint32_t)row_hi, pb.d_geo, (uint64_t)cx.b.n_rows,
                        pl.place_staged ? 1u : 0u, v.base, res->d_hits, hits_cap, cx.d_offs, res->d_hit_slots);
     HIP_TRY(hipGetLastError());
+    if (pl.agg_early && cx.agg) {
+        HIP_TRY(hipEventRecord(t->pev[kPevPlaced + c], s));
+        if (!last) {
+            hipStream_t ss = s;
+            if (pl.n_os) {
+                for (uint32_t k = 0; k < c; k++)
+                    if (k % pl.n_os != c % pl.n_os) HIP_TRY(hipStreamWaitEvent(s, t->pev[kPevPlaced + k], 0));
+            } else {
+                ss = t->sstream;
+                HIP_TRY(hipStreamWaitEvent(ss, t->pev[kPevPlaced + c], 0));
+            }
+            const uint64_t seq_lo = (uint64_t)pl.cseq[c], seq_hi = (uint64_t)pl.cseq[c + 1];
+            hipLaunchKernelGGL((kg::container_starts_kernel<AA>), dim3((uint32_t)(((seq_hi - seq_lo) * PER + 1 + 255) / 256)), dim3(256), 0, ss,
+                               cx.d_ibase, (uint32_t)seq_lo, (uint32_t)seq_hi, cx.d_offs, row_hi, v.base + 1, res->d_chs);
+            int rc;
+            if ((rc = agg_slice(t, res, *cx.agg, ss, seq_lo * PER, seq_hi * PER, v.base, 0, 0, false, pb.ucap))) return rc;
+        }
+    }
     return KG_OK;
 }
 
@@ -385,9 +407,19 @@
                                {pb.d_ghist, (uint64_t)pl.groups_stride * n_chunks}})))
             return rc;
         if ((rc = upload_scatter_cold(cx, pl, pb))) return rc;
+        const bool early = pl.agg_early && cx.agg;
+        if (early) {
+            if ((rc = agg_begin(t, cx.p, res, cx.sc, *cx.agg, cx.b.n_cont, hits_cap, cx.b.longest < (1ll << 30), plan_aggregate()))) return rc;
+            if (!pl.n_os && !t->sstream) {
+                int pr_least = 0, pr_greatest = 0;
+                HIP_TRY(hipDeviceGetStreamPriorityRange(&pr_least, &pr_greatest));
+                HIP_TRY(hipStreamCreateWithPriority(&t->sstream, hipStreamNonBlocking, pr_least));
+            }
+        }
         HIP_TRY(hipEventRecord(t->pev[kPevFork], t->stream));
         HIP_TRY(hipStreamWaitEvent(t->stream2, t->pev[kPevFork], 0));
         HIP_TRY(hipStreamWaitEvent(t->stream3, t->pev[kPevFork], 0));
+        if (early && !pl.n_os) HIP_TRY(hipStreamWaitEvent(t->sstream, t->pev[kPevFork], 0));
         hipLaunchKernelGGL((kg::row_geo_kernel<AA>), dim3((uint32_t)((nblocks * PER + 255) / 256)), dim3(256), 0, t->stream3, cx.d_blocks,
                            (uint32_t)nblocks, pb.d_geo);
         for (uint32_t c = 0; c < n_chunks; c++) {
@@ -408,6 +440,10 @@
         for (uint32_t k = 0; k < pl.n_os; k++) {
             HIP_TRY(hipEventRecord(t->pev[kPevOrdered + k], t->ostream[k]));
             HIP_TRY(hipStreamWaitEvent(t->stream, t->pev[kPevOrdered + k], 0));
+        }
+        if (early && !pl.n_os) {
+            HIP_TRY(hipEventRecord(t->pev[kPevSliced], t->sstream));
+            HIP_TRY(hipStreamWaitEvent(t->stream, t->pev[kPevSliced], 0));
         }
         HIP_TRY(hipEventRecord(t->pev[kPevJoin2], t->stream2));
         HIP_TRY(hipStreamWaitEvent(t->stream, t->pev[kPevJoin2], 0));
@@ -445,6 +481,7 @@
             st.fallback = guard ? 2 : 1;
             lists.release();
             drop_hits(t, res);
+            if (early) agg_drop(t, res, *cx.agg);
             return KG_OK;
         }
         if (!redo) {
@@ -452,11 +489,17 @@
             st.partitioned = 1;
             st.part_chunks = (int32_t)n_chunks; st.part_buckets = (int32_t)pl.buckets; st.part_shift = (int32_t)pl.shift;
             st.part_levels = pl.use_bidx ? 4 : 1;
+            if (early) {
+                cx.last_c_lo = (uint64_t)pl.cseq[n_chunks - 1] * PER;
+                cx.d_last_range = pb.d_pc + kPcBase + (n_chunks - 1);
+                cx.slice_cap = ucap;
+            }
             done = true;
             return KG_OK;
         }
         lists.release();
         drop_hits(t, res);
+        if (early) agg_drop(t, res, *cx.agg);
         if (attempt == 2) break;
         if (need_c > ccap) { pb.ccap = (need_c + pl.list_slack + kg::kUChunk - 1) / kg::kUChunk * kg::kUChunk; pb.ucap = std::max(ucap, pb.ccap); }
         else pb.ucap = (need_u + pl.list_slack + kg::kUChunk - 1) / kg::kUChunk * kg::kUChunk;
@@ -545,6 +588,9 @@
 
     Scratch sc(t);
     ScanCtx cx{t, res, sc, b, d_seq, h_seq, offsets, n_seqs, progress, counters_req || progress, h_seq == nullptr};
+    AggRun agg;
+    cx.p = p;
+    if (aggregate) cx.agg = &agg;
     if ((rc = sc.get(&cx.d_off, (size_t)n_seqs + 1))) return rc;
     if ((rc = sc.get(&cx.d_ibase, (size_t)n_seqs + 1))) return rc;
     HIP_TRY(hipMemcpyAsync(cx.d_off, offsets, ((size_t)n_seqs + 1) * 8, hipMemcpyHostToDevice, t->stream));
@@ -574,13 +620,19 @@
 
     if (progress && (rc = progress_finish(cx, part_done && part.prog_index))) return rc;
     hipLaunchKernelGGL((kg::container_starts_kernel<AA>), dim3((uint32_t)((n_cont + 1 + 255) / 256)), dim3(256), 0, t->stream,
-                       cx.d_ibase, (uint32_t)n_seqs, cx.d_offs, n_rows, cx.d_totals, res->d_chs);
+                       cx.d_ibase, 0u, (uint32_t)n_seqs, cx.d_offs, n_rows, cx.d_totals, res->d_chs);
     HIP_TRY(hipGetLastError());
     HIP_TRY(hipEventRecord(t->ev[kEvOrderEnd], t->stream));
 
-    if (aggregate && (rc = aggregate_stage(t, p, res, sc, n_seqs, n_cont, cx.n_hits, PER, cx.d_partial, cx.d_totals, nullptr, b.longest < (1ll << 30),
-                                         plan_aggregate())))
-        return rc;
+    if (aggregate) {
+        if (!agg.begun) {
+            if ((rc = agg_begin(t, p, res, sc, agg, n_cont, cx.n_hits, b.longest < (1ll << 30), plan_aggregate()))) return rc;
+            if ((rc = agg_slice(t, res, agg, t->stream, 0, n_cont, nullptr, 0, cx.n_hits, true, cx.n_hits))) return rc;
+        } else if ((rc = agg_slice(t, res, agg, t->stream, cx.last_c_lo, n_cont, cx.d_last_range, 0, 0, true, cx.slice_cap))) {
+            return rc;
+        }
+        if ((rc = agg_finish(t, p, res, sc, agg, n_seqs, cx.n_hits, PER, cx.d_partial, cx.d_totals, nullptr))) return rc;
+    }
     HIP_TRY(hipEventRecord(t->ev[kEvAggEnd], t->stream));
     HIP_TRY(hipStreamSynchronize(t->stream));
     st.n_calls = aggregate ? (int64_t)t->h_pin[kPinCalls] : 0;
diff --git a/kmergutsjava_amd/csrc/kg_host_table.hpp b/kmergutsjava_amd/csrc/kg_host_table.hpp
--- a/kmergutsjava_amd/csrc/kg_host_table.hpp
+++ b/kmergutsjava_amd/csrc/kg_host_table.hpp
@@ -330,6 +330,7 @@
     if (t->stream2) { (void)hipStreamSynchronize(t->stream2); (void)hipStreamDestroy(t->stream2); }
     if (t->stream3) { (void)hipStreamSynchronize(t->stream3); (void)hipStreamDestroy(t->stream3); }
     for (auto &os : t->ostream) if (os) { (void)hipStreamSynchronize(os); (void)hipStreamDestroy(os); }
+    if (t->sstream) { (void)hipStreamSynchronize(t->sstream); (void)hipStreamDestroy(t->sstream); }
     if (t->stream) (void)hipStreamDestroy(t->stream);
     delete t;
 }
```

Measured after the change: 133.3 billion residues/s (median of 6 runs). Within noise of the previous version (+0.6%).
